# IuvenisSapiens/Qwen3-TTS-Rust

Hardware: AMD Instinct MI355X
Metric: audio-seconds generated per second (aggregate over GPUs) = concurrent real-time streams; RTF and first-chunk latency from the single-utterance leg (higher is better)
Workload: dtype i8

## Files before the change

include/q3tts.h:

```cpp
#ifndef Q3TTS_H
#define Q3TTS_H
#include <stdint.h>
#include <stddef.h>
#ifdef __cplusplus
extern "C" {
#endif

#define Q3TTS_OK 0
#define Q3TTS_ERR -1

const char* q3tts_last_error(void);
int q3tts_version(void);
int q3tts_device_count(void);

typedef struct q3tts_sampler_config {
    float temperature;
    int32_t top_k;
    float top_p;
    int32_t has_seed;
    uint64_t seed;
} q3tts_sampler_config;
void q3tts_sampler_config_default(q3tts_sampler_config* c);

typedef struct q3tts_gen_options {
    float repetition_penalty;
    float predictor_temperature;
    int32_t predictor_top_k;
    float predictor_top_p;
} q3tts_gen_options;
void q3tts_gen_options_default(q3tts_gen_options* o);

typedef struct q3tts_engine q3tts_engine;
typedef struct q3tts_engine_params {
    const char* model_dir;
    const char* quant;
    int32_t device;
    int32_t max_batch;
    int32_t max_prompt;
    int32_t max_steps;
    int32_t load_codec;
    int32_t use_graph;
} q3tts_engine_params;
void q3tts_engine_params_default(q3tts_engine_params* p);
int q3tts_engine_create(const q3tts_engine_params* p, q3tts_engine** out);
void q3tts_engine_destroy(q3tts_engine* e);

typedef struct q3tts_request {
    const float* prompt;
    int32_t n_prompt;
    q3tts_sampler_config sampler;
    int32_t max_steps;
    int32_t mask_eos;
    int32_t* codes_out;
    float* pcm_out;
    int64_t pcm_capacity;
    int32_t n_frames;
    int64_t n_pcm;
    double prefill_ms, first_chunk_ms, total_ms;
} q3tts_request;
int q3tts_generate_batch(q3tts_engine* e, q3tts_request* reqs, int32_t n_reqs, int32_t want_pcm);
int q3tts_generate_batch_ex(q3tts_engine* e, q3tts_request* reqs, int32_t n_reqs, int32_t want_pcm, const q3tts_gen_options* opts);
int q3tts_generate_batch_trailing(q3tts_engine* e, q3tts_request* reqs, int32_t n_reqs, int32_t want_pcm, const q3tts_gen_options* opts,
                                  const int32_t* const* trail_ids, const int32_t* n_trail);

typedef struct q3tts_stats {
    double frame_loop_ms; int64_t frames; double prefill_ms;
    double gemv_ms; int64_t gemv_launches; double gemv_bytes;
    double codec_ms; int64_t codec_calls;
    double talker_weight_bytes, predictor_weight_bytes, kv_bytes_per_token;
    double gu_ms; int64_t gu_launches; double gu_bytes;
    int64_t sched_steps; double slot_frames;
    int64_t graph_frames;
} q3tts_stats;
int q3tts_engine_stats(q3tts_engine* e, q3tts_stats* out);
void q3tts_engine_reset_stats(q3tts_engine* e);
void q3tts_engine_set_instrument(q3tts_engine* e, int32_t on);
double q3tts_engine_bytes_per_step(q3tts_engine* e, int32_t batch, double mean_ctx);

#define Q3TTS_REQ_QUEUED 0
#define Q3TTS_REQ_RUNNING 1
#define Q3TTS_REQ_DRAINING 2
#define Q3TTS_REQ_DONE 3
#define Q3TTS_REQ_CANCELLED 4
#define Q3TTS_REQ_FAILED (-1)
typedef struct q3tts_req_status {
    int32_t state; int32_t n_frames; int64_t n_pcm;
    double queue_ms, prefill_ms, first_chunk_ms, total_ms;
} q3tts_req_status;
int q3tts_submit(q3tts_engine* e, const q3tts_request* r, int32_t want_pcm, int64_t* req_id);
int q3tts_submit_ex(q3tts_engine* e, const q3tts_request* r, int32_t want_pcm, const q3tts_gen_options* opts ,
                    int64_t* req_id);
int q3tts_submit_trailing(q3tts_engine* e, const q3tts_request* r, int32_t want_pcm, const q3tts_gen_options* opts ,
                          const int32_t* trail_ids, int32_t n_trail, int64_t* req_id);
int q3tts_submit_trailing_open(q3tts_engine* e, const q3tts_request* r, int32_t want_pcm, const q3tts_gen_options* opts,
                               const int32_t* trail_ids, int32_t n_trail, int64_t* req_id);
int q3tts_trail_append(q3tts_engine* e, int64_t req_id, const int32_t* ids, int32_t n, int32_t close);
int q3tts_trail_progress(q3tts_engine* e, int64_t req_id, int32_t* n_appended, int32_t* n_consumed, int32_t* closed);
int q3tts_poll(q3tts_engine* e, int64_t req_id, q3tts_req_status* out);
int q3tts_fetch(q3tts_engine* e, int64_t req_id, int32_t* codes_out, int32_t frame_off, int32_t max_frames, float* pcm_out,
                int64_t pcm_off, int64_t pcm_cap, int32_t* got_frames, int64_t* got_pcm);
int q3tts_wait(q3tts_engine* e, int64_t req_id, double timeout_ms );
int q3tts_release(q3tts_engine* e, int64_t req_id);
int q3tts_cancel(q3tts_engine* e, int64_t req_id);
int q3tts_submit_resume(q3tts_engine* e, const q3tts_request* r, int32_t want_pcm, const q3tts_gen_options* opts,
                        const int32_t* trail_ids, int32_t n_trail, int32_t open,
                        const int32_t* prefix_codes, int32_t n_prefix, int64_t* req_id);
#define Q3TTS_LOGPROB_COLS 17
#define Q3TTS_LOGPROB_NONE 1.0f
int q3tts_engine_set_logprobs(q3tts_engine* e, int32_t on);
int q3tts_fetch_logprobs(q3tts_engine* e, int64_t req_id, float* out, int32_t frame_off, int32_t max_frames, int32_t* got_frames);
int32_t q3tts_engine_prefill_width(q3tts_engine* e);
int q3tts_sched_start(q3tts_engine* e);
int q3tts_sched_stop(q3tts_engine* e);
int q3tts_sched_step(q3tts_engine* e, int32_t* busy);
int q3tts_voice_register(q3tts_engine* e, const float* spk_emb2048, const int32_t* ref_codes, int32_t n_ref_codes,
                         const int32_t* ref_text_ids, int32_t n_ref_text, int32_t* voice_id);
int q3tts_submit_text(q3tts_engine* e, int32_t voice_id, const int32_t* text_ids, int32_t n_text, int32_t lang_id,
                      const int32_t* instr_ids, int32_t n_instr, const q3tts_sampler_config* sampler, int32_t max_steps,
                      int32_t mask_eos, int32_t want_pcm, int64_t* req_id);
int q3tts_submit_text_ex(q3tts_engine* e, int32_t voice_id, const int32_t* text_ids, int32_t n_text, int32_t lang_id,
                         const int32_t* instr_ids, int32_t n_instr, const q3tts_sampler_config* sampler, int32_t max_steps,
                         int32_t mask_eos, int32_t want_pcm, const q3tts_gen_options* opts, int64_t* req_id);
int q3tts_submit_text_streaming(q3tts_engine* e, int32_t voice_id, const int32_t* text_ids, int32_t n_text, int32_t lang_id,
                                const int32_t* instr_ids, int32_t n_instr, const q3tts_sampler_config* sampler, int32_t max_steps,
                                int32_t mask_eos, int32_t want_pcm, const q3tts_gen_options* opts, int64_t* req_id);
int q3tts_submit_text_streaming_open(q3tts_engine* e, int32_t voice_id, const int32_t* text_ids, int32_t n_text, int32_t lang_id,
                                     const int32_t* instr_ids, int32_t n_instr, const q3tts_sampler_config* sampler, int32_t max_steps,
                                     int32_t mask_eos, int32_t want_pcm, const q3tts_gen_options* opts, int64_t* req_id);
int q3tts_text_append(q3tts_engine* e, int64_t req_id, const int32_t* text_ids, int32_t n, int32_t is_last);

// ... 173 lines not shown
enum { Q3TTS_GEMM_AUTO = 0, Q3TTS_GEMM_SKINNY4 = 1, Q3TTS_GEMM_SKINNY8 = 2, Q3TTS_GEMM_SKINNY16 = 3,
       Q3TTS_GEMM_F32_1 = 4, Q3TTS_GEMM_F32_2 = 5,
       Q3TTS_GEMM_H1 = 6, Q3TTS_GEMM_H1_EPL = 7, Q3TTS_GEMM_H2 = 8, Q3TTS_GEMM_H2_EPL = 9,
       Q3TTS_GEMM_H3 = 10, Q3TTS_GEMM_H3_EPL = 11 };
enum { Q3TTS_EPI_NONE = 0, Q3TTS_EPI_GELU = 1, Q3TTS_EPI_RES_SCALE = 2 , Q3TTS_EPI_RES = 3 ,
       Q3TTS_EPI_SNAKE = 4  };
typedef struct q3tts_codec_gemm_desc {
    int32_t M, N, cin, taps, dil;
    const float* A; int64_t a_rows; int32_t lda, a_segT, a_skip;
    int32_t a_split, o_split;
    const float* W; const float* bias;
    int32_t epi; const float* res; int64_t res_floats; int32_t ldr, r_segT; int64_t r_skip;
    const float* scale; const float* snake_ea; const float* snake_ib;
    float* out; int64_t out_floats, out_off; int32_t ldo, o_segT; int64_t o_skip;
    int64_t ws_floats;
    int32_t form, ksplit, reducer;
    int32_t form_ran, ksplit_ran, reducer_ran;
} q3tts_codec_gemm_desc;
int q3tts_op_codec_gemm(q3tts_codec_gemm_desc* d);
int q3tts_codec_gemm_plan(q3tts_codec_gemm_desc* d);

enum { Q3TTS_CK_RVQ_SUM = 0, Q3TTS_CK_RMSNORM_ROWS = 1, Q3TTS_CK_LAYERNORM_ROWS = 2, Q3TTS_CK_ROPE_APPEND = 3, Q3TTS_CK_WINDOW_ATTN = 4,
       Q3TTS_CK_SWIGLU_ROWS = 5, Q3TTS_CK_DWCONV7 = 6, Q3TTS_CK_SNAKE = 7, Q3TTS_CK_SNAKE_SPLIT = 8, Q3TTS_CK_CONV_OUT_WAVE = 9,
       Q3TTS_CK_CONV_OUT_WIN = 10, Q3TTS_CK_HIST_LOAD = 11, Q3TTS_CK_HIST_SAVE = 12, Q3TTS_CK_HIST_ZERO = 13 };
typedef struct q3tts_codec_kernel_desc {
    int32_t kernel;
    int32_t G, T, C, H;
    int32_t n_heads, head_dim, window; float rope_base, eps, bias;
    const int64_t* meta;
    const int64_t* codes; int32_t n_q, cb_size;
    int32_t n_streams, stream;
    const float* in[3]; int64_t in_floats[3];
    const float* p0; const float* p1; int64_t p0_floats, p1_floats;
    float* out[3]; int64_t out_floats[3];
} q3tts_codec_kernel_desc;
int q3tts_op_codec_kernel(q3tts_codec_kernel_desc* d);

enum { Q3TTS_ATTN_AUTO = 0, Q3TTS_ATTN_UNFUSED = 1 , Q3TTS_ATTN_FUSED = 2 ,
       Q3TTS_ATTN_SHORT1 = 3, Q3TTS_ATTN_SHORT2 = 4 , Q3TTS_ATTN_GGML = 5  };
typedef struct q3tts_attention_desc {
    int32_t n_head, n_kv, n_layer, layer, ntok;
    const float* qkv; int32_t qkv_stride;
    const float* q_norm; const float* k_norm;
    float eps, rope_base; int32_t n_ctx; int32_t mrope_sec[4];
    const int32_t* seq; const int32_t* slot; const int32_t* pos; int32_t uniform_pos;
    const int32_t* page_table; int32_t n_seq, max_pages;
    uint16_t* k_cache; uint16_t* v_cache; int32_t n_pages;
    int32_t fused, fused_max_tok, same_seq, short_attn_min, hpw1_max, float_mode, ggml_mode;
    int32_t form;
    float* att; int8_t* aq; uint16_t* ad;
    int32_t form_ran;
} q3tts_attention_desc;
int q3tts_op_attention(q3tts_attention_desc* d);
int q3tts_attention_plan(q3tts_attention_desc* d);

enum { Q3TTS_LOP_GEMV = 0, Q3TTS_LOP_GATEUP = 1, Q3TTS_LOP_NORM = 2, Q3TTS_LOP_NORM_GEMV = 3, Q3TTS_LOP_NORM_ARGMAX = 4, Q3TTS_LOP_NORM_GATEUP = 5,
       Q3TTS_LOP_F_GEMV = 6, Q3TTS_LOP_F_GATEUP = 7 };
enum { Q3TTS_LIN_AUTO = 0, Q3TTS_LIN_GEMV_Q8 = 1, Q3TTS_LIN_GEMM_Q8_TOK = 2, Q3TTS_LIN_GEMM_Q8_MFMA = 3, Q3TTS_LIN_GEMM_Q8_TILE1 = 4,
       Q3TTS_LIN_GEMV_KQ = 5, Q3TTS_LIN_GEMM_KQ_MFMA = 6, Q3TTS_LIN_GU_Q8_TILE1 = 7, Q3TTS_LIN_GU_Q8_MFMA = 8, Q3TTS_LIN_GU_KQ_MFMA = 9,
       Q3TTS_LIN_GU_UNFUSED = 10, Q3TTS_LIN_NORM = 11, Q3TTS_LIN_NORM_WG = 12, Q3TTS_LIN_GEMV_NORM = 13, Q3TTS_LIN_GEMV_NORM_ARGMAX = 14,
       Q3TTS_LIN_GU_SWIGLU_NORM = 15, Q3TTS_LIN_F_GEMV = 16, Q3TTS_LIN_F_MFMA16 = 17, Q3TTS_LIN_F_MFMA = 18, Q3TTS_LIN_F_GU_MFMA16 = 19,
       Q3TTS_LIN_F_GU_UNFUSED = 20 };
typedef struct q3tts_linear_desc {
    int32_t op, form;
    int32_t nw; const void* raw[3]; int32_t type[3]; int32_t rows[3]; int32_t kq_layout;
    int32_t K, row0, nrows, nrows_valid, ntok, ff;
    int32_t lpr, mt, ztiles;
    int32_t fused;
    const int8_t* xq; const uint16_t* xd; int32_t a_rows;
    const float* x; int64_t x_floats; int32_t x_off, x_stride;
    const float* h_in; int64_t h_floats; int32_t h_stride;
    const uint64_t* idx_keys; const int32_t* idx; int32_t idx_stride;
    const float* parts; int64_t parts_floats; int32_t nparts, parts_stride; int64_t parts_slab;
    const float* g; float eps;
    float* h_out; float* xn_out;
    int8_t* xq_out; uint16_t* xd_out;
    uint64_t* keys; int64_t n_keys; int32_t key_stride; const int32_t* mask_per_tok; int32_t idx_add;
    float* out; int64_t out_floats, out_off; int32_t out_stride;
    int8_t* aq; uint16_t* ad;
    int32_t form_ran, lpr_ran, mt_ran, z_ran;
} q3tts_linear_desc;
int q3tts_op_linear(q3tts_linear_desc* d);
int q3tts_linear_plan(q3tts_linear_desc* d);
uint64_t q3tts_argmax_key(float v, int32_t idx);

#ifdef __cplusplus
}
#endif
#endif
```

qwen3-tts-rust_amd/csrc/capi.cpp:

```cpp
#include "../../include/q3tts.h"
#include "engine.h"
#include "tfctx.h"
#include <algorithm>

using namespace q3;

struct q3tts_assets { std::unique_ptr<HostAssets> owned; const HostAssets* a = nullptr; };
struct q3tts_engine { std::unique_ptr<Engine> e; q3tts_assets assets_view; };
struct q3tts_sampler { Sampler s; };
struct q3tts_chunker { std::unique_ptr<Chunker> c; };
struct q3tts_decoder { std::unique_ptr<CodecDecoder> d; hipStream_t st = nullptr; float* pinned = nullptr; size_t pinned_cap = 0; };
struct q3tts_tf { std::unique_ptr<TfContext> c; };

#define Q3_API_BEGIN try {
#define Q3_API_END(failval) } catch (const std::exception& ex) { set_last_error(ex.what()); return failval; } catch (...) { set_last_error("unknown error"); return failval; }

static void require_gpu() {
    int n = 0;
    if (hipGetDeviceCount(&n) != hipSuccess || n <= 0) throw Error("no HIP device available: the HIP path is the only compute path (no CPU fallback)");
}

extern "C" {

const char* q3tts_last_error(void) { return last_error(); }
// ... 214 lines not shown
    return submit_text(e, voice_id, text_ids, n_text, lang_id, instr_ids, n_instr, sampler, max_steps, mask_eos, want_pcm, opts, true, req_id);
}
int q3tts_submit_text_streaming_open(q3tts_engine* e, int32_t voice_id, const int32_t* text_ids, int32_t n_text, int32_t lang_id,
                                     const int32_t* instr_ids, int32_t n_instr, const q3tts_sampler_config* sampler, int32_t max_steps,
                                     int32_t mask_eos, int32_t want_pcm, const q3tts_gen_options* opts, int64_t* req_id) {
    return submit_text(e, voice_id, text_ids, n_text, lang_id, instr_ids, n_instr, sampler, max_steps, mask_eos, want_pcm, opts, true, req_id,
                       true);
}
static int submit_text(q3tts_engine* e, int32_t voice_id, const int32_t* text_ids, int32_t n_text, int32_t lang_id, const int32_t* instr_ids,
                       int32_t n_instr, const q3tts_sampler_config* sampler, int32_t max_steps, int32_t mask_eos, int32_t want_pcm,
                       const q3tts_gen_options* opts, bool streaming, int64_t* req_id, bool open) {
    Q3_API_BEGIN
    Q3_CHECK(e && text_ids && n_text >= 0 && req_id, "bad arguments");
    Q3_CHECK(!streaming || n_text >= 1, "the streaming-text layout needs n_text >= 1");
    const Voice& v = e->e->voice(voice_id);
    std::vector<int32_t> t(text_ids, text_ids + n_text), ins;
    if (instr_ids) ins.assign(instr_ids, instr_ids + n_instr);
    int lang = lang_id;
    std::vector<int32_t> trail;
    std::vector<int32_t>* tr = streaming ? &trail : nullptr;
    PromptData pd = !v.ref_codes.empty()
        ? PromptBuilder::build_clone_prompt(e->e->assets(), t, v.ref_codes, v.ref_text_ids, v.spk_emb.data(), lang_id, instr_ids ? &ins : nullptr, tr)
        : PromptBuilder::build_core(e->e->assets(), t, lang_id >= 0 ? &lang : nullptr, nullptr, v.spk_emb.data(), instr_ids ? &ins : nullptr, nullptr, tr);
    GenRequest g;
    g.prompt = pd.embd.data(); g.n_prompt = pd.n_rows; g.max_steps = max_steps; g.mask_eos = mask_eos != 0;
    if (sampler) {
        g.sampler.temperature = sampler->temperature; g.sampler.top_k = sampler->top_k; g.sampler.top_p = sampler->top_p;
        g.sampler.has_seed = sampler->has_seed != 0; g.sampler.seed = sampler->seed;
    }
    g.opts = to_opts(opts);
    if (open) trail.pop_back();
    g.trail = trail.data(); g.n_trail = (int)trail.size(); g.open = open;
    *req_id = e->e->submit(g, want_pcm != 0, true);
    return Q3TTS_OK;
    Q3_API_END(Q3TTS_ERR)
}

int q3tts_engine_stats(q3tts_engine* e, q3tts_stats* o) {
    Q3_API_BEGIN
    const EngineStats& s = e->e->stats;
    o->frame_loop_ms = s.frame_loop_ms; o->frames = s.frames; o->prefill_ms = s.prefill_ms; o->gemv_ms = s.gemv_ms;
    o->gemv_launches = s.gemv_launches; o->gemv_bytes = s.gemv_bytes; o->codec_ms = s.codec_ms; o->codec_calls = s.codec_calls;
    o->gu_ms = s.gu_ms; o->gu_launches = s.gu_launches; o->gu_bytes = s.gu_bytes;
    o->sched_steps = s.steps; o->slot_frames = s.slot_frames; o->graph_frames = s.graph_frames;
    o->talker_weight_bytes = (double)e->e->talker().weight_bytes(); o->predictor_weight_bytes = (double)e->e->predictor().weight_bytes();
    const auto& hp = e->e->talker().hp();
    o->kv_bytes_per_token = (double)hp.n_layer * 2 * hp.n_kv * 128 * 2;
    return Q3TTS_OK;
    Q3_API_END(Q3TTS_ERR)
}
void q3tts_engine_reset_stats(q3tts_engine* e) { if (e) e->e->reset_stats(); }
void q3tts_engine_set_instrument(q3tts_engine* e, int32_t on) { if (e) e->e->set_instrument(on != 0); }
double q3tts_engine_bytes_per_step(q3tts_engine* e, int32_t batch, double mean_ctx) { return e ? (double)e->e->bytes_per_frame_step(batch, mean_ctx) : 0.0; }

int q3tts_assets_open(const char* path, q3tts_assets** out) {
    Q3_API_BEGIN
    Q3_CHECK(path && out, "null argument");
    auto* h = new q3tts_assets();
    try { h->owned.reset(new HostAssets(path)); } catch (...) { delete h; throw; }
    h->a = h->owned.get();
    *out = h;
    return Q3TTS_OK;
    Q3_API_END(Q3TTS_ERR)
}
void q3tts_assets_close(q3tts_assets* a) { delete a; }
const q3tts_assets* q3tts_engine_assets(q3tts_engine* e) { return e ? &e->assets_view : nullptr; }
int q3tts_assets_codec_embedding(const q3tts_assets* a, int32_t q, int32_t code, float* out) { Q3_API_BEGIN a->a->codec_embedding(q, code, out); return Q3TTS_OK; Q3_API_END(Q3TTS_ERR) }
int q3tts_assets_text_embedding(const q3tts_assets* a, int64_t tok, float* out) { Q3_API_BEGIN a->a->text_embedding(tok, out); return Q3TTS_OK; Q3_API_END(Q3TTS_ERR) }
int q3tts_assets_tts_pad(const q3tts_assets* a, float* out) { Q3_API_BEGIN std::copy(a->a->tts_pad(), a->a->tts_pad() + 2048, out); return Q3TTS_OK; Q3_API_END(Q3TTS_ERR) }

int q3tts_op_feedback_rows(const q3tts_assets* a, const int32_t* codes, int32_t n, const int32_t* trail_ids, int32_t n_trail, float* rows) {
    Q3_API_BEGIN
    Q3_CHECK(a && a->a && codes && rows && n >= 1, "bad arguments");
    Q3_CHECK(n_trail >= 0 && (n_trail == 0 || trail_ids), "trailing ids missing");
    require_gpu();
    const HostAssets& h = *a->a;
    Q3_CHECK(h.n_codec == 16, "need 16 codec embedding tables");
    std::vector<DevBuf<float>> tab(16);
    std::vector<const float*> ptrs(16); std::vector<int64_t> nrows(16);
    for (int q = 0; q < 16; q++) {
        const size_t sz = (size_t)h.codec_rows[q] * Q3_EMBD;
        tab[q].alloc(sz); tab[q].upload(h.codec[q], sz);
        ptrs[q] = tab[q].p; nrows[q] = h.codec_rows[q];
    }
    DevBuf<const float*> d_ptrs(16); DevBuf<int64_t> d_nrows(16); DevBuf<float> d_pad(Q3_EMBD), d_text, d_rows((size_t)(n + 2) * Q3_EMBD);
    DevBuf<int32_t> d_codes((size_t)n * 16), d_ids;
    d_ptrs.upload(ptrs.data(), 16); d_nrows.upload(nrows.data(), 16); d_pad.upload(h.tts_pad(), Q3_EMBD); d_codes.upload(codes, (size_t)n * 16);
    FeedbackIds fi;
    const int nt = std::min(n_trail, n);
    if (nt > 0) {
        const int64_t tr = h.text_table ? h.text_rows : 0;
        d_text.alloc((size_t)std::max<int64_t>(tr, 1) * Q3_EMBD);
        if (tr > 0) d_text.upload(h.text_table, (size_t)tr * Q3_EMBD);
        d_ids.alloc(nt); d_ids.upload(trail_ids, nt);
        fi.ids = d_ids.p; fi.n_ids = nt; fi.table = d_text.p; fi.rows = tr;
    }
    std::vector<float> all((size_t)(n + 2) * Q3_EMBD, -12345.0f);
    d_rows.upload(all.data(), all.size());
    launch_feedback_codes(0, d_ptrs.p, d_nrows.p, d_codes.p, d_pad.p, d_rows.p + Q3_EMBD, n, &fi);
    Q3_HIP(hipDeviceSynchronize());
    d_rows.download(all.data(), all.size());
    for (int i = 0; i < Q3_EMBD; i++)
        Q3_CHECK(all[i] == -12345.0f && all[(size_t)(n + 1) * Q3_EMBD + i] == -12345.0f, "k_feedback_codes wrote outside its rows");
    std::copy(all.begin() + Q3_EMBD, all.begin() + (size_t)(n + 1) * Q3_EMBD, rows);
    return Q3TTS_OK;
    Q3_API_END(Q3TTS_ERR)
// ... 166 lines not shown
```

qwen3-tts-rust_amd/csrc/capi_ops.cpp:

```cpp
#include "../../include/q3tts.h"
#include "transformer.h"
#include "host_logic.h"
#include "kdev.h"
#include "codec.h"

using namespace q3;
#define Q3_API_BEGIN try {
#define Q3_API_END(failval) } catch (const std::exception& ex) { set_last_error(ex.what()); return failval; } catch (...) { set_last_error("unknown error"); return failval; }
static void require_gpu() {
    int n = 0;
    if (hipGetDeviceCount(&n) != hipSuccess || n <= 0) throw Error("no HIP device available: the HIP path is the only compute path (no CPU fallback)");
}

static int attention_op_plan(const q3tts_attention_desc& d) {
    AttnPlanIn a;
    a.ntok = d.ntok; a.fused = d.fused != 0; a.fused_max_tok = d.fused_max_tok; a.same_seq = d.same_seq != 0; a.short_attn_min = d.short_attn_min;
    a.n_head = d.n_head; a.n_kv = d.n_kv; a.hpw1_max = d.hpw1_max > 0 ? d.hpw1_max : short_attn_hpw1_max();
    a.float_mode = d.float_mode != 0; a.ggml_mode = d.ggml_mode != 0;
    return plan_attention(a);
}

static void attention_op_check(const q3tts_attention_desc& d, int form) {
    Q3_CHECK(form >= ATTN_UNFUSED && form <= ATTN_GGML, "unknown attention form");
    Q3_CHECK(d.n_head >= 1 && d.n_kv >= 1 && d.n_head % d.n_kv == 0, "n_head must be a multiple of n_kv");
    Q3_CHECK(d.n_layer >= 1 && d.layer >= 0 && d.layer < d.n_layer && d.ntok >= 1 && d.ntok <= 65535, "bad layer / token count");
    Q3_CHECK(d.qkv && d.q_norm && d.k_norm && d.k_cache && d.v_cache && d.qkv_stride >= (d.n_head + 2 * d.n_kv) * 128, "bad qkv / norm / cache buffers");
    Q3_CHECK(d.n_ctx >= 1 && d.n_pages >= 1, "bad n_ctx / n_pages");
    if (form != ATTN_GGML) Q3_CHECK(d.aq && d.ad, "aq / ad are required");
    else Q3_CHECK(d.att, "the ggml form produces att only");
    if (d.uniform_pos < 0) Q3_CHECK(d.seq && d.slot && d.pos, "per-token seq / slot / pos are required without uniform_pos");
    if (d.page_table) {
        Q3_CHECK(d.n_seq >= 1 && d.max_pages >= 1, "bad page table shape");
        for (int64_t i = 0; i < (int64_t)d.n_seq * d.max_pages; i++)
            Q3_CHECK(d.page_table[i] >= 0 && d.page_table[i] < d.n_pages, "page table entry out of range");
    }
    const bool short_form = form == ATTN_SHORT1 || form == ATTN_SHORT2;
    if (short_form) Q3_CHECK(d.n_head == 2 * d.n_kv, "the short forms need n_head == 2 * n_kv");
    std::map<std::pair<int, int>, int> seen;
    std::map<int, int> per_seq;
    for (int t = 0; t < d.ntok; t++) {
        const int seq = d.uniform_pos >= 0 ? t : d.seq[t], slot = d.uniform_pos >= 0 ? d.uniform_pos : d.slot[t];
        Q3_CHECK(slot >= 0 && slot < d.n_ctx, "slot out of [0, n_ctx)");
        if (d.page_table) Q3_CHECK(seq >= 0 && seq < d.n_seq && slot < d.max_pages * 64, "sequence or slot beyond the page table");
        else Q3_CHECK(seq >= 0 && seq < d.n_pages && slot < 64, "identity paging: sequence beyond the cache or slot beyond its one page");
        if (short_form) Q3_CHECK(slot < 64, "the short forms read page 0 only: slot must be < 64");
        Q3_CHECK(seen[std::make_pair(seq, slot)]++ == 0, "two tokens write the same (sequence, slot)");
        if (++per_seq[seq] > 1) Q3_CHECK(form == ATTN_UNFUSED || form == ATTN_GGML, "the fused and short forms need one token per sequence");
    }
}

static void attention_op_run(q3tts_attention_desc* dp) {
    Q3_CHECK(dp, "null attention descriptor");
    q3tts_attention_desc& d = *dp;
    Q3_CHECK(d.ntok >= 1 && d.n_head >= 1 && d.n_kv >= 1, "bad attention shape");
    const int form = d.form == Q3TTS_ATTN_AUTO ? attention_op_plan(d) : d.form;
    attention_op_check(d, form);
    const int nt = d.ntok, dq = d.n_head * 128, qs = d.qkv_stride;
    DevBuf<float> qkv((size_t)nt * qs); qkv.upload(d.qkv, qkv.n);
    DevBuf<float> qn(128), kn(128); qn.upload(d.q_norm, 128); kn.upload(d.k_norm, 128);
    std::vector<float> hc, hs;
    build_rope_tables(d.rope_base, d.n_ctx, hc, hs);
    DevBuf<float> rc(hc.size()), rs(hs.size()); rc.upload(hc.data(), hc.size()); rs.upload(hs.data(), hs.size());
    DevBuf<int32_t> sec(4); sec.upload(d.mrope_sec, 4);
    DevBuf<int32_t> dseq, dslot, dpos, dtab;
    TokMeta tm{nullptr, nullptr, nullptr};
    if (d.uniform_pos >= 0) tm.uniform_pos = d.uniform_pos;
    else {
        dseq.alloc(nt); dseq.upload(d.seq, nt); dslot.alloc(nt); dslot.upload(d.slot, nt); dpos.alloc((size_t)nt * 4); dpos.upload(d.pos, (size_t)nt * 4);
        tm.seq = dseq.p; tm.slot = dslot.p; tm.pos = dpos.p;
    }
    const size_t cache_halfs = (size_t)d.n_pages * d.n_layer * d.n_kv * 8192;
    DevBuf<uint16_t> kc(cache_halfs), vc(cache_halfs);
    kc.upload(d.k_cache, cache_halfs); vc.upload(d.v_cache, cache_halfs);
    KvCache kv;
    kv.k = kc.p; kv.v = vc.p; kv.page_table = nullptr; kv.max_pages = d.page_table ? d.max_pages : 1; kv.n_layer = d.n_layer; kv.n_kv = d.n_kv;
    if (d.page_table) { dtab.alloc((size_t)d.n_seq * d.max_pages); dtab.upload(d.page_table, dtab.n); kv.page_table = dtab.p; }
    DevBuf<float> att((size_t)nt * dq), qrot, scores;
    DevBuf<int8_t> aq((size_t)nt * dq); DevBuf<uint16_t> ad((size_t)nt * (dq / 32));
    switch (form) {
    case ATTN_UNFUSED:
        qrot.alloc((size_t)nt * dq);
        launch_qk_rope_append(0, qkv.p, qs, nullptr, d.n_head, d.n_kv, qn.p, kn.p, d.eps, rc.p, rs.p, d.n_ctx, sec.p, tm, kv, d.layer, qrot.p, nt);
        launch_attention(0, qrot.p, d.n_head, d.n_kv, tm, kv, d.layer, att.p, aq.p, ad.p, nt);
        break;
    case ATTN_FUSED:
        launch_attention_fused(0, qkv.p, qs, d.n_head, d.n_kv, qn.p, kn.p, d.eps, rc.p, rs.p, d.n_ctx, sec.p, tm, kv, d.layer, aq.p, ad.p, nt);
        break;
    case ATTN_SHORT1: case ATTN_SHORT2:
        launch_attention_short(0, form == ATTN_SHORT1 ? 1 : 2, qkv.p, qs, d.n_head, d.n_kv, qn.p, kn.p, d.eps, rc.p, rs.p, d.n_ctx, sec.p, tm, kv,
                               d.layer, aq.p, ad.p, nt, att.p);
        break;
    default:
        scores.alloc((size_t)nt * d.n_head * d.n_ctx);
        gg_qk_rope_append(0, qkv.p, qs, d.n_head, d.n_kv, qn.p, kn.p, d.eps, rc.p, rs.p, d.n_ctx, sec.p, tm, kv, d.layer, nt);
        gg_attention(0, qkv.p, qs, d.n_head, d.n_kv, tm, kv, d.layer, att.p, scores.p, d.n_ctx, nt);
        break;
    }
    Q3_LAUNCH_CHECK();
    Q3_HIP(hipDeviceSynchronize());
    kc.download(d.k_cache, cache_halfs); vc.download(d.v_cache, cache_halfs);
    if (d.att && form != ATTN_FUSED) att.download(d.att, att.n);
    if (form != ATTN_GGML) { aq.download(d.aq, aq.n); ad.download(d.ad, ad.n); }
    d.form_ran = form;
}

static bool lin_quant(const q3tts_linear_desc& d) { return d.op <= LOP_NORM_GATEUP && d.op != LOP_NORM; }
static bool lin_kq(const q3tts_linear_desc& d) {
    if (d.kq_layout || d.nw > 1) return true;
    return d.type[0] != Q3_T_Q8_0;
}
static int lin_rows(const q3tts_linear_desc& d) { int n = 0; for (int i = 0; i < d.nw; i++) n += d.rows[i]; return n; }
static int lin_wts(const q3tts_linear_desc& d) {
    if (d.op >= LOP_F_GEMV) return d.type[0];
    if (!lin_kq(d)) return 0;
    int n = 0, last = -1;
    for (int i = 0; i < d.nw; i++) if (d.type[i] != last) { n++; last = d.type[i]; }
    return n == 1 ? d.type[0] : -1;
}
static LinearPlanIn lin_plan_in(const q3tts_linear_desc& d) {
    LinearPlanIn in;
    in.op = d.op; in.K = d.K; in.row0 = d.row0; in.nrows = d.nrows; in.ntok = d.ntok; in.ff = d.ff;
    in.kq = lin_quant(d) && lin_kq(d); in.wts = lin_wts(d); in.has_wt = true;
    if (in.kq) { int n = 0, last = -1; for (int i = 0; i < d.nw; i++) if (d.type[i] != last) { n++; last = d.type[i]; } in.kq_parts = n; }
    in.out_stride = d.out_stride; in.out_addr = (uintptr_t)d.out_off * 4 + (d.out ? (uintptr_t)d.out : 0);
    in.x_stride = d.x_stride; in.x_addr = (uintptr_t)d.x_off * 4 + (d.x ? (uintptr_t)d.x : 0);
    in.aq_addr = 0; in.fused = d.fused != 0;
    return in;
}
static LinearPlan lin_plan(const q3tts_linear_desc& d) {
    Q3_CHECK(d.op >= LOP_GEMV && d.op <= LOP_F_GATEUP, "unknown linear op");
    Q3_CHECK(d.K >= 256 && d.K % 256 == 0 && d.ntok >= 1 && d.ntok <= 65535 && d.nrows >= 1 && d.row0 >= 0, "bad linear shape");
    return plan_linear(lin_plan_in(d));
}
static bool in_set(int v, std::initializer_list<int> s) { for (int x : s) if (v == x) return true; return false; }
static int op_of_form(int f) {
    if (f <= LIN_GEMM_KQ_MFMA) return LOP_GEMV;
    if (f <= LIN_GU_UNFUSED) return LOP_GATEUP;
    if (f <= LIN_NORM_WG) return LOP_NORM;
    if (f == LIN_GEMV_NORM) return LOP_NORM_GEMV;
    if (f == LIN_GEMV_NORM_ARGMAX) return LOP_NORM_ARGMAX;
    if (f == LIN_GU_SWIGLU_NORM) return LOP_NORM_GATEUP;
    if (f <= LIN_F_MFMA) return LOP_F_GEMV;
    return LOP_F_GATEUP;
}
static void lin_check(const q3tts_linear_desc& d, const LinearPlan& p) {
    const int f = p.form, K = d.K, nt = d.ntok, ntiles = (nt + 31) / 32;
    Q3_CHECK(f >= LIN_GEMV_Q8 && f <= LIN_F_GU_UNFUSED && op_of_form(f) == d.op, "the form does not compute this op");
    const bool quant = lin_quant(d), kq = quant && lin_kq(d), norm = d.op >= LOP_NORM && d.op <= LOP_NORM_GATEUP;
    if (d.op != LOP_NORM) {
        Q3_CHECK(d.nw >= 1 && d.nw <= 3, "1 to 3 weight tensors");
        for (int i = 0; i < d.nw; i++) Q3_CHECK(d.raw[i] && d.rows[i] >= 1, "missing weight tensor");
        if (d.op >= LOP_F_GEMV) Q3_CHECK(d.nw == 1 && (d.type[0] == Q3_T_F32 || d.type[0] == Q3_T_F16 || d.type[0] == Q3_T_BF16), "float ops take one f32 / f16 / bf16 tensor");
        else if (kq) for (int i = 0; i < d.nw; i++) Q3_CHECK(in_set(d.type[i], {Q3_T_Q8_0, Q3_T_Q5_K, Q3_T_Q6_K}) && d.rows[i] % 32 == 0, "K-quant layout: Q8_0 / Q5_K / Q6_K tensors of 32-row multiples");
        Q3_CHECK(d.row0 + d.nrows <= lin_rows(d), "rows past the matrix");
    }
// ... 134 lines not shown
        dxq_out.alloc((size_t)nt * K); dxq_out.upload(d.xq_out, dxq_out.n); dxd_out.alloc((size_t)nt * (K / 32)); dxd_out.upload(d.xd_out, dxd_out.n);
        launch_rmsnorm_quant_wg(0, a, K, dxq_out.p, dxd_out.p, nt);
        break;
    case LIN_GEMV_NORM: case LIN_GEMV_NORM_ARGMAX: {
        ArgmaxEpi am{};
        if (p.form == LIN_GEMV_NORM_ARGMAX) {
            dkeys.alloc((size_t)d.n_keys); dkeys.upload((const q3_u64*)d.keys, dkeys.n);
            if (d.mask_per_tok) { dmask.alloc(nt); dmask.upload(d.mask_per_tok, nt); }
            am.keys = dkeys.p; am.key_stride = d.key_stride; am.mask_per_tok = dmask.p; am.idx_add = d.idx_add;
            run_gemv_q8_norm(0, p, m, d.row0, d.nrows_valid, a, nullptr, 0, nt, &am);
        } else run_gemv_q8_norm(0, p, m, d.row0, d.nrows, a, out, d.out_stride, nt, nullptr);
        break;
    }
    case LIN_GU_SWIGLU_NORM: run_gateup_swiglu(0, p, m, ff, a, daq.p, dad.p, nt); break;
    case LIN_F_GEMV: case LIN_F_MFMA16: case LIN_F_MFMA:
        run_gemv_float(0, p, fm, d.row0, d.nrows, dx.p + d.x_off, d.x_stride, out, d.out_stride, nt);
        break;
    case LIN_F_GU_MFMA16:
        dgu.alloc((size_t)nt * ff);
        run_gateup_float(0, p, fm, ff, dx.p + d.x_off, d.x_stride, dgu.p, nt);
        break;
    case LIN_F_GU_UNFUSED: {
        dgu.alloc((size_t)nt * 2 * ff);
        LinearPlanIn gi = lin_plan_in(d); gi.op = LOP_F_GEMV;
        const LinearPlan gp = plan_linear(gi);
        run_gemv_float(0, gp, fm, 0, 2 * ff, dx.p + d.x_off, d.x_stride, dgu.p, 2 * ff, nt);
        DevBuf<float> act((size_t)nt * ff);
        launch_swiglu_f32(0, dgu.p, ff, act.p, nt);
        Q3_HIP(hipMemcpy2D(out, (size_t)d.out_stride * 4, act.p, (size_t)ff * 4, (size_t)ff * 4, nt, hipMemcpyDeviceToDevice));
        Q3_HIP(hipDeviceSynchronize());
        p.lpr = gp.lpr; p.mt = gp.mt; p.z = gp.z;
        break;
    }
    default: throw Error("unhandled linear form");
    }
    Q3_LAUNCH_CHECK();
    if (p.form == LIN_F_GU_MFMA16) Q3_HIP(hipMemcpy2D(out, (size_t)d.out_stride * 4, dgu.p, (size_t)ff * 4, (size_t)ff * 4, nt, hipMemcpyDeviceToDevice));
    Q3_HIP(hipDeviceSynchronize());
    if (d.out) dout.download(d.out, dout.n);
    if (d.aq) { daq.download(d.aq, daq.n); dad.download(d.ad, dad.n); }
    if (d.h_out) dhout.download(d.h_out, dhout.n);
    if (d.xn_out) dxn.download(d.xn_out, dxn.n);
    if (dxq_out.p) { dxq_out.download(d.xq_out, dxq_out.n); dxd_out.download(d.xd_out, dxd_out.n); }
    if (dkeys.p) dkeys.download((q3_u64*)d.keys, dkeys.n);
    d.form_ran = p.form; d.lpr_ran = p.lpr; d.mt_ran = p.mt; d.z_ran = p.z;
}

extern "C" {

int q3tts_op_attention(q3tts_attention_desc* d) {
    Q3_API_BEGIN
    require_gpu();
    attention_op_run(d);
    return Q3TTS_OK;
    Q3_API_END(Q3TTS_ERR)
}

int q3tts_attention_plan(q3tts_attention_desc* d) {
    Q3_API_BEGIN
    Q3_CHECK(d && d->ntok >= 1 && d->n_kv >= 1 && d->n_head >= 1, "bad attention shape");
    d->form_ran = attention_op_plan(*d);
    return Q3TTS_OK;
    Q3_API_END(Q3TTS_ERR)
}

int q3tts_op_linear(q3tts_linear_desc* d) {
    Q3_API_BEGIN
    require_gpu();
    lin_run(d);
    return Q3TTS_OK;
    Q3_API_END(Q3TTS_ERR)
}

int q3tts_linear_plan(q3tts_linear_desc* d) {
    Q3_API_BEGIN
    Q3_CHECK(d, "null linear descriptor");
    const LinearPlan p = lin_plan(*d);
    d->form_ran = p.form; d->lpr_ran = p.lpr; d->mt_ran = p.mt; d->z_ran = p.z;
    return Q3TTS_OK;
    Q3_API_END(Q3TTS_ERR)
}

uint64_t q3tts_argmax_key(float v, int32_t idx) { return pack_key(v, idx); }

int q3tts_op_gemv_q8(const void* w, int32_t n, int32_t k, const int8_t* xq, const uint16_t* xd, int32_t ntok, float* y, int32_t lpr) {
    Q3_API_BEGIN
    require_gpu();
    DevBuf<uint8_t> storage;
    Q8Mat m = q8mat_from_host(w, n, k, storage);
    DevBuf<int8_t> dxq((size_t)ntok * k); dxq.upload(xq, dxq.n);
    DevBuf<uint16_t> dxd((size_t)ntok * (k / 32)); dxd.upload(xd, dxd.n);
    const int nsseg = ((k >> 8) + 7) / 8;
    DevBuf<float> parts((size_t)nsseg * ntok * n);
    launch_gemv_q8(0, m, 0, n, dxq.p, dxd.p, parts.p, n, ntok, lpr);
    Q3_HIP(hipDeviceSynchronize());
    std::vector<float> hp(parts.n);
    parts.download(hp.data(), hp.size());
    for (int t = 0; t < ntok; t++)
        for (int r = 0; r < n; r++) {
            float v = hp[((size_t)0 * ntok + t) * n + r];
            for (int s = 1; s < nsseg; s++) v = v + hp[((size_t)s * ntok + t) * n + r];
            y[(size_t)t * n + r] = v;
        }
    return Q3TTS_OK;
    Q3_API_END(Q3TTS_ERR)
}
// ... 483 lines not shown
```

qwen3-tts-rust_amd/csrc/engine.cpp:

```cpp
#include "engine.h"
#include "../../include/q3tts.h"
#include <algorithm>
#include <cmath>
#include <chrono>
#include "kdev.h"
#include <functional>

namespace q3 {

static std::string quant_dir(const std::string& q) {
    if (q == "q5_k_m") return "gguf_q5_k_m";
    if (q == "q8_0") return "gguf_q8_0";
    if (q == "bf16") return "gguf_bf16";
    if (q == "f16") return "gguf_f16";
    return "gguf";
}
static double now_ms() {
    return std::chrono::duration<double, std::milli>(std::chrono::steady_clock::now().time_since_epoch()).count();
}

Engine::Engine(const EngineParams& p) : p_(p) {
    Q3_CHECK(p.max_batch >= 1 && p.max_batch <= 512, "max_batch out of range");
    Q3_HIP(hipGetDevice(&dev_));
    Q3_HIP(hipStreamCreateWithFlags(&st_, hipStreamNonBlocking));
    const std::string dir = p.model_dir + "/" + quant_dir(p.quant);
    assets_.reset(new HostAssets(dir + "/qwen3_assets.gguf"));
    const int B = p.max_batch;
    B_ = B;
    talker_.reset(new Transformer(dir + "/qwen3_tts_talker.gguf", Q3_TALKER_NCTX, std::max(256, B)));
    predictor_.reset(new Transformer(dir + "/qwen3_tts_predictor.gguf", Q3_PRED_NCTX, 2 * B));
    if (const char* e = std::getenv("Q3_PRED_FUSED_MAX")) predictor_->set_fused_max_tokens(atoi(e));
    {
        int min_tok = 8;
        if (const char* e = std::getenv("Q3_SHORT_ATTN_MIN")) min_tok = atoi(e);
        predictor_->set_short_attention(min_tok, 17);
    }
    Q3_CHECK(talker_->hp().n_embd == Q3_EMBD, "talker n_embd must be 2048 (reference hard-codes 2048-wide rows)");
    dP_ = predictor_->hp().n_embd;
    Q3_CHECK(assets_->proj_out == dP_ && assets_->proj_in == Q3_EMBD, "proj shape does not match predictor n_embd");
    Q3_CHECK(assets_->n_codec == 16, "need 16 codec embedding tables");
    Q3_CHECK(predictor_->hp().n_vocab >= 15 * Q3_CODEBOOK_SIZE, "predictor vocab < 15*2048");
    std::vector<float> wt((size_t)Q3_EMBD * dP_);
    for (int o = 0; o < dP_; o++)
        for (int i = 0; i < Q3_EMBD; i++) wt[(size_t)i * dP_ + o] = assets_->proj_w[(size_t)o * Q3_EMBD + i];
    d_proj_wt_.alloc(wt.size()); d_proj_wt_.upload(wt.data(), wt.size());
    Q3_CHECK(dP_ % 16 == 0, "projection width must be a multiple of 16");
    {
        std::vector<float> wb((size_t)Q3_EMBD * dP_);
        for (int o = 0; o < dP_; o++)
            for (int i = 0; i < Q3_EMBD; i++) wb[((size_t)(o / 16) * Q3_EMBD + i) * 16 + (o % 16)] = assets_->proj_w[(size_t)o * Q3_EMBD + i];
        d_proj_wblk_.alloc(wb.size()); d_proj_wblk_.upload(wb.data(), wb.size());
    }
    d_proj_b_.alloc(dP_); d_proj_b_.upload(assets_->proj_b, dP_);
    d_tts_pad_.alloc(Q3_EMBD); d_tts_pad_.upload(assets_->tts_pad(), Q3_EMBD);
    std::vector<const float*> ptrs(16);
    std::vector<int64_t> rows(16);
    for (int q = 0; q < 16; q++) {
        const size_t n = (size_t)assets_->codec_rows[q] * Q3_EMBD;
        d_codec_tab_[q].alloc(n); d_codec_tab_[q].upload(assets_->codec[q], n);
        d_proj_tab_[q].alloc((size_t)assets_->codec_rows[q] * dP_);
        launch_project_table(st_, d_codec_tab_[q].p, assets_->codec_rows[q], d_proj_wt_.p, d_proj_b_.p, Q3_EMBD, dP_, d_proj_tab_[q].p);
        ptrs[q] = d_codec_tab_[q].p; rows[q] = assets_->codec_rows[q];
    }
    d_tab_ptrs_.alloc(16); d_tab_ptrs_.upload(ptrs.data(), 16);
    d_tab_rows_.alloc(16); d_tab_rows_.upload(rows.data(), 16);
    const int pages_per_seq = (p.max_prompt + p.max_steps + 1 + 63) / 64;
    kv_rows_ = (int64_t)pages_per_seq * 64;
    kv_t_.reset(new KvPool(talker_->hp().n_layer, talker_->hp().n_kv, B * pages_per_seq + 1, B + 1, pages_per_seq));
    kv_p_.reset(new KvPool(predictor_->hp().n_layer, predictor_->hp().n_kv, B, B, 1));
    for (int b = 0; b < B; b++) kv_p_->ensure(b, 16);
    pred_identity_pages_ = true;
    for (int b = 0; b < B; b++) if (kv_p_->page(b, 0) != b) pred_identity_pages_ = false;
    if (const char* e = std::getenv("Q3_UNIFORM_META")) if (e[0] == '0') pred_identity_pages_ = false;
    kv_t_->ensure(B, 1);
    {
        const char* e = std::getenv("Q3_ASYNC_PREFILL");
        async_pf_ = B > 1 && !(e && e[0] == '0');
    }
    if (async_pf_) {
        talker_pf_.reset(new Transformer(*talker_, 256));
        Q3_HIP(hipStreamCreateWithFlags(&st_pf_, hipStreamNonBlocking));
        Q3_HIP(hipEventCreate(&pf_done_)); Q3_HIP(hipEventCreate(&pf_e0_));
        arena_pf_cap_ = (size_t)4096 * (Q3_EMBD * 4 + 24 + 68) + ((size_t)1 << 16);
        Q3_HIP(hipHostMalloc((void**)&arena_pf_, arena_pf_cap_));
        d_prompt_pf_.alloc((size_t)256 * Q3_EMBD); d_pfa_seq_.alloc(256); d_pfa_slot_.alloc(256); d_pfa_pos_.alloc(4 * 256);
        d_pfa_codes_.alloc((size_t)256 * 16); d_pfa_ids_.alloc(256);
    }
    hist_stride_ = p.max_steps * 16;
    tl_stride_ = (Q3_SAMPLE_END + 31) & ~31;
    slots_ = SlotTable(B); d_slots_.alloc(slots_.host.size()); slots_.dev = d_slots_.p;
    d_keys_.alloc(16 * B); d_next_key0_.alloc(B); d_hist_.alloc((size_t)B * hist_stride_);
    d_rngkey_.alloc((size_t)8 * B); d_draws_.alloc(B); d_prngkey_.alloc((size_t)8 * B); d_pdraws_.alloc(B);
    d_rngkey_.zero(); d_draws_.zero(); d_prngkey_.zero(); d_pdraws_.zero(); d_plogits_.alloc((size_t)B * Q3_CODEBOOK_SIZE);
    d_tlogits_.alloc((size_t)B * tl_stride_); d_thidden_.alloc((size_t)B * Q3_EMBD); d_pin_.alloc((size_t)2 * B * dP_);
    d_fb_.alloc((size_t)B * Q3_EMBD);
    d_prompt_.alloc((size_t)talker_->max_tok() * Q3_EMBD);
    d_pf_seq_.alloc(talker_->max_tok()); d_pf_slot_.alloc(talker_->max_tok()); d_pf_pos_.alloc(4 * (size_t)talker_->max_tok());
    d_pf_codes_.alloc((size_t)talker_->max_tok() * 16); d_pf_ids_.alloc(talker_->max_tok());
    d_hist_.zero(); d_tlogits_.zero(); d_thidden_.zero();
    std::vector<int32_t> seq(B), slot((size_t)16 * B), pos((size_t)16 * B * 4);
    for (int b = 0; b < B; b++) {
        seq[b] = b;
        for (int i = 0; i < 16; i++) { slot[(size_t)i * B + b] = i; for (int s = 0; s < 4; s++) pos[((size_t)i * B + b) * 4 + s] = i; }
    }
    d_pseq_.alloc(B); d_pseq_.upload(seq.data(), B);
    d_pslot_.alloc(slot.size()); d_pslot_.upload(slot.data(), slot.size());
    d_ppos_.alloc(pos.size()); d_ppos_.upload(pos.data(), pos.size());
    h_pend_.assign(B, std::vector<int32_t>()); h_pend_off_.assign(B, 0);
    slot_req_.assign(B, nullptr);
    if (async_pf_) { d_pf_logits_.alloc((size_t)B * tl_stride_); d_pf_hidden_.alloc((size_t)B * Q3_EMBD); }
    {
        std::vector<q3_u64> k0((size_t)16 * B, pack_key(-INFINITY, 0)), n0(B, pack_key(-INFINITY, 0));
        d_keys_.upload(k0.data(), k0.size()); d_next_key0_.upload(n0.data(), n0.size());
    }
    arena_cap_ = (size_t)talker_->max_tok() * Q3_EMBD * 4 + (size_t)B * 4096 + ((size_t)1 << 20);
    Q3_HIP(hipHostMalloc((void**)&arena_, arena_cap_));
    Q3_HIP(hipDeviceSynchronize());
    upload_slot_state();
// ... 32 lines not shown
void* Engine::d2h_begin(const void* src, size_t bytes) {
    void* p = stage_alloc(bytes);
    Q3_HIP(hipMemcpyAsync(p, src, bytes, hipMemcpyDeviceToHost, st_));
    return p;
}

struct Engine::Req {
    int64_t id = 0;
    GenRequest r; std::vector<float> prompt_own; std::vector<int32_t> trail_own; bool want_pcm = false;
    std::vector<int32_t> prefix_own;
    bool closed = false;
    bool cancel = false;
    int state = REQ_QUEUED; int slot = -1, cs = -1; int fed = 0;
    std::vector<int32_t> codes; std::vector<float> pcm;
    std::vector<float> lp;
    size_t pcm_enq = 0;
    size_t pcm_ready = 0;
    std::unique_ptr<Chunker> chunker;
    uint64_t seed = 0;
    hipEvent_t ev_admit = nullptr; bool first_seen = false;
    double t_submit = 0, t_admit = 0, t_done = 0, prefill_ms = 0, first_chunk_ms = 0;
    std::string error;
};

Engine::~Engine() {
    (void)hipSetDevice(dev_);
    try { stop_driver(); } catch (...) {}
    if (dec_started_) {
        { std::lock_guard<std::mutex> lk(dmu_); dec_stop_ = true; }
        dcv_.notify_all();
        dec_thread_.join();
    }
    for (auto& c : comp_) (void)hipEventDestroy(c.ev);
    for (auto& kv : reqs_) if (kv.second->ev_admit) (void)hipEventDestroy(kv.second->ev_admit);
    for (auto& g : graphs_) {
        if (g.second->exec) (void)hipGraphExecDestroy(g.second->exec);
        if (g.second->graph) (void)hipGraphDestroy(g.second->graph);
    }
    if (pcm_pinned_) (void)hipHostFree(pcm_pinned_);
    if (arena_) (void)hipHostFree(arena_);
    if (arena_pf_) (void)hipHostFree(arena_pf_);
    if (pf_done_) (void)hipEventDestroy(pf_done_);
    if (pf_e0_) (void)hipEventDestroy(pf_e0_);
    if (st_pf_) (void)hipStreamDestroy(st_pf_);
    for (auto s2 : st2_) (void)hipStreamDestroy(s2);
    if (st_) (void)hipStreamDestroy(st_);
}

size_t Engine::bytes_per_frame_step(int batch, double mean_ctx) const {
    const auto& t = talker_->hp();
    const size_t head_t = (size_t)tl_stride_ * talker_->head_bytes_per_row();
    const size_t head_p = (size_t)15 * Q3_CODEBOOK_SIZE * predictor_->head_bytes_per_row();
    const size_t kv_per_tok = (size_t)t.n_layer * 2 * t.n_kv * 128 * 2;
    return talker_->weight_bytes() + head_t + predictor_->weight_bytes() + head_p +
           (size_t)((double)batch * mean_ctx * (double)kv_per_tok) + (size_t)batch * 17 * 8192;
}

void Engine::record_frame(FrameGraph& fg, FrameVariant v) {
    const int B = fg.width;
    const KvCache kvt = kv_t_->view(), kvp = kv_p_->view();
    AdvanceKeysArgs a{B, di(SF_FINISHED), di(SF_NFRAMES), di(SF_MAXFRAMES), d_keys_.p, d_next_key0_.p, d_hist_.p, hist_stride_, di(SF_TSLOT), di(SF_TPOS)};
    StallArgs sg;
    if (v.gate) {
        sg.open = di(SF_OPEN); sg.n_trail = di(SF_NTRAIL); sg.hidden = d_thidden_.p; sg.draws = d_draws_.p; sg.pdraws = d_pdraws_.p;
        sg.save_hidden = d_stall_hidden_.p; sg.save_draws = d_stall_draws_.p;
        launch_stall_save(st_, a, sg);
    }
    launch_project_blk(st_, d_thidden_.p, Q3_EMBD, d_proj_wblk_.p, d_proj_b_.p, Q3_EMBD, dP_, d_pin_.p, dP_, B);
    launch_gather_rows_keys(st_, d_proj_tab_[0].p, assets_->codec_rows[0], d_keys_.p, 16, dP_, d_pin_.p + (size_t)B * dP_, B);
    {
        TokMeta tm{fg.seqA.p, fg.slotA.p, fg.posA.p};
        Transformer::Input in; in.x = d_pin_.p; in.x_stride = dP_;
        predictor_->set_same_seq_tokens(true);
        predictor_->forward(st_, in, 2 * B, tm, kvp, nullptr);
        if (v.pred || v.lp) {
            float* pl = v.lp ? d_plp_.p : d_plogits_.p;
            predictor_->head(st_, B, B, 0, Q3_CODEBOOK_SIZE, pl, Q3_CODEBOOK_SIZE);
            SampleArgs sa{pl, Q3_CODEBOOK_SIZE, Q3_CODEBOOK_SIZE, df(SF_PTEMP), di(SF_PTOPK), df(SF_PTOPP), nullptr, d_prngkey_.p, d_pdraws_.p, d_keys_.p + 1, 16};
            launch_sample_pred(st_, sa, B);
        } else {
            ArgmaxEpi am{d_keys_.p + 1, 16, nullptr, 0};
            predictor_->head(st_, B, B, 0, Q3_CODEBOOK_SIZE, nullptr, 0, &am);
        }
    }
    predictor_->set_same_seq_tokens(false);
    for (int q = 1; q < 15; q++) {
        TokMeta tm{d_pseq_.p, d_pslot_.p + (size_t)(q + 1) * B_, d_ppos_.p + (size_t)(q + 1) * B_ * 4};
        KvCache kvq = kvp;
        if (pred_identity_pages_) { tm.uniform_pos = q + 1; kvq.page_table = nullptr; }
        Transformer::Input in; in.x = d_proj_tab_[q].p; in.x_stride = dP_; in.idx_keys = d_keys_.p + q; in.idx_stride = 16;
        predictor_->forward(st_, in, B, tm, kvq, nullptr);
        if (v.pred || v.lp) {
            float* pl = v.lp ? d_plp_.p + (size_t)q * B_ * Q3_CODEBOOK_SIZE : d_plogits_.p;
            predictor_->head(st_, 0, B, q * Q3_CODEBOOK_SIZE, Q3_CODEBOOK_SIZE, pl, Q3_CODEBOOK_SIZE);
            SampleArgs sa{pl, Q3_CODEBOOK_SIZE, Q3_CODEBOOK_SIZE, df(SF_PTEMP), di(SF_PTOPK), df(SF_PTOPP), nullptr, d_prngkey_.p, d_pdraws_.p, d_keys_.p + q + 1, 16};
            launch_sample_pred(st_, sa, B);
        } else {
            ArgmaxEpi am{d_keys_.p + q + 1, 16, nullptr, 0};
            predictor_->head(st_, 0, B, q * Q3_CODEBOOK_SIZE, Q3_CODEBOOK_SIZE, nullptr, 0, &am);
        }
    }
    if (v.trail) {
        TextTrail tt; tt.n_frames = di(SF_NFRAMES); tt.n_trail = di(SF_NTRAIL); tt.ids = d_trail_.p; tt.ids_stride = p_.max_prompt;
        tt.table = d_text_.p; tt.rows = text_rows_;
        launch_feedback_keys(st_, d_tab_ptrs_.p, d_tab_rows_.p, d_keys_.p, 16, d_tts_pad_.p, d_fb_.p, B, &tt);
    } else {
        launch_feedback_keys(st_, d_tab_ptrs_.p, d_tab_rows_.p, d_keys_.p, 16, d_tts_pad_.p, d_fb_.p, B);
    }
    {
        TokMeta tm{di(SF_TSEQ), di(SF_TSLOT), di(SF_TPOS)};
        Transformer::Input in; in.x = d_fb_.p; in.x_stride = Q3_EMBD;
        talker_->set_same_seq_tokens(false);
        talker_->forward(st_, in, B, tm, kvt, nullptr);
        if (v.sampled || v.pen || v.lp) {
            talker_->head(st_, 0, B, 0, tl_stride_, d_tlogits_.p, tl_stride_, nullptr, -1, d_thidden_.p);
            SampleArgs sa{d_tlogits_.p, tl_stride_, Q3_SAMPLE_END, df(SF_TEMP), di(SF_TOPK), df(SF_TOPP), di(SF_MASKEOS), d_rngkey_.p, d_draws_.p, d_next_key0_.p, 1};
            if (v.pen) { sa.penalty = df(SF_PEN); sa.hist = d_hist_.p; sa.hist_stride = hist_stride_; sa.hist_len = di(SF_NFRAMES); sa.cur_key = d_keys_.p; sa.cur_stride = 16; }
            launch_sample(st_, sa, B);
            if (v.lp) {
                LogprobArgs la;
                la.p.logits = d_plp_.p; la.p.stride = Q3_CODEBOOK_SIZE; la.p.head_stride = (size_t)B_ * Q3_CODEBOOK_SIZE; la.p.n = Q3_CODEBOOK_SIZE;
                la.p.key = d_keys_.p + 1; la.p.key_stride = 16; la.p.col = 1; la.n_first = 15;
                la.t.logits = d_tlogits_.p; la.t.stride = tl_stride_; la.t.n = Q3_SAMPLE_END; la.t.key = d_next_key0_.p; la.t.key_stride = 1;
                la.t.extra_idx = Q3_CODEC_EOS; la.t.col = 0; la.t.col_extra = Q3_LOGPROB_COLS - 1; la.t.row_ahead = 1;
                la.out = d_lp_.p; la.out_stride = Q3_LOGPROB_COLS; la.out_rows = lp_rows_;
                la.n_frames = di(SF_NFRAMES); la.finished = di(SF_FINISHED); la.max_frames = di(SF_MAXFRAMES); la.open = di(SF_OPEN);
                la.n_trail = di(SF_NTRAIL); la.record = d_lp_rec_.p;
                launch_logprob_rows(st_, la, B);
            }
        } else {
            ArgmaxEpi am{d_next_key0_.p, 1, di(SF_MASKEOS), 0};
            talker_->head(st_, 0, B, 0, tl_stride_, nullptr, 0, &am, Q3_SAMPLE_END, d_thidden_.p);
        }
    }
    if (v.gate) launch_advance_keys_gated(st_, a, sg);
    else launch_advance_keys(st_, a);
    Q3_LAUNCH_CHECK();
}

std::mutex& capture_mutex() { static std::mutex mu; return mu; }

Engine::FrameGraph& Engine::frame_graph(int width, FrameVariant v, bool capture) {
    std::unique_ptr<FrameGraph>& slot = graphs_[v.key(width)];
// ... 879 lines not shown
```

qwen3-tts-rust_amd/csrc/engine.h:

```cpp
#pragma once
#include "transformer.h"
#include "host_logic.h"
#include "sched_logic.h"
#include "codec.h"
#include <atomic>
#include <condition_variable>
#include <deque>
#include <map>
#include <memory>
#include <mutex>
#include <thread>

namespace q3 {

struct EngineParams {
    std::string model_dir;
    std::string quant = "q8_0";
    int max_batch = 1;
    int max_prompt = 1024;
    int max_steps = Q3_DEFAULT_MAX_STEPS;
    bool load_codec = true;
    bool use_graph = true;
};

// ... 4 lines not shown
};

struct EngineStats {
    double frame_loop_ms = 0; long frames = 0;
    double gemv_ms = 0; long gemv_launches = 0; double gemv_bytes = 0;
    double gu_ms = 0; long gu_launches = 0; double gu_bytes = 0;
    double codec_ms = 0; long codec_calls = 0;
    double prefill_ms = 0;
    long steps = 0; double slot_frames = 0;
    long graph_frames = 0;
};

struct ReqStatus {
    int state = REQ_QUEUED; int n_frames = 0; int64_t n_pcm = 0;
    double queue_ms = 0, prefill_ms = 0, first_chunk_ms = 0, total_ms = 0;
    std::string error;
};

struct Voice {
    std::vector<float> spk_emb; std::vector<int32_t> ref_codes, ref_text_ids;
};


class Engine {
public:
    explicit Engine(const EngineParams& p);
    ~Engine();
    void generate_batch(const std::vector<GenRequest>& reqs, std::vector<GenResult>& out, bool want_pcm);

    int64_t submit(const GenRequest& r, bool want_pcm, bool copy_prompt = true, bool may_record = true);
    void set_logprobs(bool on);
    void fetch_logprobs(int64_t id, float* out, int frame_off, int max_frames, int* got_frames);
    int append_trail(int64_t id, const int32_t* ids, int n, bool close);
    void trail_progress(int64_t id, int* n_appended, int* n_consumed, bool* closed);
    int cancel(int64_t id);
    bool step();
    ReqStatus poll(int64_t id);
    void fetch(int64_t id, int32_t* codes, int frame_off, int max_frames, float* pcm, int64_t pcm_off, int64_t pcm_cap,
               int* got_frames, int64_t* got_pcm);
    bool wait(int64_t id, double timeout_ms);
    void release(int64_t id);
    void start_driver();
    void stop_driver();
    int register_voice(const Voice& v);
    const Voice& voice(int id) const;

    const HostAssets& assets() const { return *assets_; }
    Transformer& talker() { return *talker_; }
    Transformer& predictor() { return *predictor_; }
    CodecDecoder* codec() { return codec_.get(); }
    EngineStats stats; void reset_stats() { stats = EngineStats(); }
    void set_instrument(bool on) { instrument_ = on; }
    size_t bytes_per_frame_step(int batch, double mean_ctx) const;
    hipStream_t stream() const { return st_; }
    int max_batch() const { return B_; }
    int device() const { return dev_; }

private:
    struct Req;
    struct FrameGraph {
        int width = 0; hipGraph_t graph = nullptr; hipGraphExec_t exec = nullptr;
        DevBuf<int32_t> seqA, slotA, posA;
    };
    void record_frame(FrameGraph& fg, FrameVariant v);
    FrameGraph& frame_graph(int width, FrameVariant v, bool capture);
    void validate(const GenRequest& g) const;
    void ensure_text_stream();
    void prefill(const std::vector<Req*>& batch, bool sampled);
    void feedback_rows(hipStream_t st, const std::vector<Req*>& batch, const std::vector<FbRun>& fb, int32_t* hc, int32_t* d_codes, int32_t* d_ids, float* d_rows);
    void head_history(SampleArgs& sa, int b) const;
    static bool resumed_penalised(const GenRequest& g) { return g.n_prefix > 0 && g.opts.penalised(); }
    void first_head_logprobs(hipStream_t st, const float* logits_row, int b, int row);
    void prefill_async(const std::vector<Req*>& batch);
    void activate();
    void admit(bool stalled);
    void run_group();
    void collect_appends();
    void collect_cancels();
    void harvest(bool block);
    void purge_chunks(Req* r);
    void retire(Req* r, bool flush_tail);
    void decoder_main();
    void upload_slot_state();
    void* stage_alloc(size_t bytes);
    void h2d(void* dst, const void* src, size_t bytes);
    void* d2h_begin(const void* src, size_t bytes);
    unsigned char* arena_ = nullptr; size_t arena_cap_ = 0, arena_used_ = 0;

    EngineParams p_;
    hipStream_t st_ = nullptr; int dev_ = 0;
    std::vector<hipStream_t> st2_;
    float* pcm_pinned_ = nullptr; size_t slot_cap_ = 0;
    std::unique_ptr<HostAssets> assets_;
    std::unique_ptr<Transformer> talker_, predictor_, talker_pf_;
    hipStream_t st_pf_ = nullptr; unsigned char* arena_pf_ = nullptr; size_t arena_pf_cap_ = 0;
    DevBuf<float> d_prompt_pf_, d_pf_logits_, d_pf_hidden_; DevBuf<int32_t> d_pfa_seq_, d_pfa_slot_, d_pfa_pos_;
    std::vector<Req*> pf_batch_; hipEvent_t pf_done_ = nullptr, pf_e0_ = nullptr; bool async_pf_ = false; int n_prefilling_ = 0;
    std::unique_ptr<KvPool> kv_t_, kv_p_;
    std::unique_ptr<CodecDecoder> codec_;
    DevBuf<float> d_codec_tab_[16]; DevBuf<float> d_proj_tab_[16];
    DevBuf<float> d_proj_wt_, d_proj_wblk_, d_proj_b_, d_tts_pad_;
    DevBuf<const float*> d_tab_ptrs_; DevBuf<int64_t> d_tab_rows_;
    int dP_ = 0;
    int B_ = 0; SlotTable slots_; DevBuf<uint32_t> d_slots_; bool slot_dirty_ = false;
    int32_t* di(SlotField f) const { return slots_.di(f); } float* df(SlotField f) const { return slots_.df(f); }
    DevBuf<int32_t> d_hist_; DevBuf<q3_u64> d_keys_, d_next_key0_;
    DevBuf<uint32_t> d_rngkey_, d_draws_, d_prngkey_, d_pdraws_; DevBuf<float> d_plogits_;
    DevBuf<int32_t> d_pseq_, d_pslot_, d_ppos_;
    DevBuf<float> d_tlogits_, d_thidden_, d_pin_, d_fb_, d_prompt_;
    DevBuf<int32_t> d_pf_seq_, d_pf_slot_, d_pf_pos_;
    DevBuf<int32_t> d_pf_codes_, d_pf_ids_, d_pfa_codes_, d_pfa_ids_;
    int64_t kv_rows_ = 0;
    int hist_stride_ = 0, tl_stride_ = 0;
    DevBuf<float> d_text_; DevBuf<int32_t> d_trail_; int64_t text_rows_ = 0;
    std::mutex text_mu_; bool text_ready_ = false;
    DevBuf<float> d_stall_hidden_; DevBuf<uint32_t> d_stall_draws_;
    DevBuf<float> d_lp_, d_plp_; DevBuf<int32_t> d_lp_rec_; int lp_rows_ = 0;
    std::mutex lp_mu_; std::atomic<bool> lp_on_{false}, lp_ready_{false};
    std::map<int, std::unique_ptr<FrameGraph>> graphs_;
    bool instrument_ = false; bool pred_identity_pages_ = false;
    std::vector<std::vector<int32_t>> h_pend_; std::vector<int> h_pend_off_;
    std::mutex mu_; std::condition_variable cv_;
    std::mutex step_mu_;
    std::map<int64_t, std::unique_ptr<Req>> reqs_;
    std::deque<Req*> pending_;
    std::vector<Req*> slot_req_;
    std::vector<int> cs_free_;
    int64_t next_id_ = 1;
    int n_active_ = 0, n_draining_ = 0;
    bool trail_dirty_ = false;
    std::vector<int64_t> cancel_ids_;
    uint64_t wake_ = 0;
    bool stalled_idle_ = false;
    std::vector<Voice> voices_;
    std::thread driver_; bool driver_on_ = false, driver_stop_ = false;
    struct DecTask { Req* r; std::vector<int64_t> codes; bool is_final; bool fence; bool reset; };
    struct Completion { Req* r; hipEvent_t ev; size_t pcm_after; bool fence; };
    std::thread dec_thread_; bool dec_started_ = false, dec_stop_ = false;
    std::mutex dmu_; std::condition_variable dcv_;
    std::deque<DecTask> dq_; std::deque<Completion> comp_;
    int dec_pending_ = 0;
    std::string derr_;
    LaunchTimer timer_, timer_gu_;
};

}
```

qwen3-tts-rust_amd/csrc/kernels.h:

```cpp
#pragma once
#include <hip/hip_runtime.h>
#include <cstdint>
#include "wlayout.h"

namespace q3 {

struct Q8Mat {
    const uint8_t* qs = nullptr;
    const uint16_t* sc = nullptr;
    int N = 0;
    int Npad = 0;
    int K = 0;
    const uint8_t* rg_type = nullptr;
    const uint32_t* rg_off = nullptr;
    const uint8_t* meta = nullptr;
    size_t qbytes = 0;
    int nparts = 0; int p1_rg0 = 0x7fffffff, p2_rg0 = 0x7fffffff; int p0_type = 0, p1_type = 0, p2_type = 0; uint32_t p0_off = 0, p1_off = 0, p2_off = 0;
    size_t bytes() const { return (qbytes ? qbytes : (size_t)Npad * K) + (size_t)Npad * (K / 32) * 2 + (meta ? (size_t)Npad * (K / 256) * 16 : 0); }
};

struct TokMeta {
    const int32_t* seq;
    const int32_t* slot;
    const int32_t* pos;
    int uniform_pos = -1;
    __device__ __forceinline__ int seq_of(int tok) const { return uniform_pos >= 0 ? tok : seq[tok]; }
    __device__ __forceinline__ int slot_of(int tok) const { return uniform_pos >= 0 ? uniform_pos : slot[tok]; }
    __device__ __forceinline__ int pos_of(int tok, int stream) const { return uniform_pos >= 0 ? uniform_pos : pos[(size_t)tok * 4 + stream]; }
};

struct KvCache {
    uint16_t* k;
    uint16_t* v;
    const int32_t* page_table;
    int max_pages;
    int n_layer, n_kv;
    __host__ __device__ size_t page_stride() const { return (size_t)n_layer * n_kv * 8192; }
    __host__ __device__ size_t layer_stride() const { return (size_t)n_kv * 8192; }
    __device__ __forceinline__ int page_of(int seq, int logical) const { return page_table ? page_table[(size_t)seq * max_pages + logical] : seq; }
};

bool launch_gateup_mfma(hipStream_t st, const Q8Mat& wgu, int ff, const int8_t* xq, const uint16_t* xd, int8_t* aq, uint16_t* ad, int ntok);
void launch_gemv_q8(hipStream_t st, const Q8Mat& w, int row0, int nrows, const int8_t* xq, const uint16_t* xd,
                    float* out, int out_stride, int ntok, int lpr_hint = 0);

struct NormArgs {
    const float* h_in; int h_stride;
    const int32_t* idx; int idx_stride;
    const unsigned long long* idx_keys;
    const float* parts; int nparts; int parts_stride;
    float* h_out;
    const float* g; float eps; int d;
    int8_t* xq; uint16_t* xd;
    float* xn_out;
};
void launch_rmsnorm_quant(hipStream_t st, const NormArgs& a, int ntok);

void launch_qk_rope_append(hipStream_t st, const float* qkv, int qkv_stride, const float* parts_unused, int n_head, int n_kv,
                           const float* q_norm_w, const float* k_norm_w, float eps, const float* rope_cos,
                           const float* rope_sin, int n_ctx, const int32_t* mrope_sec , const TokMeta& tm,
                           const KvCache& kv, int layer, float* qrot, int ntok);

void launch_attention(hipStream_t st, const float* qrot, int n_head, int n_kv, const TokMeta& tm, const KvCache& kv,
                      int layer, float* att , int8_t* aq, uint16_t* ad, int ntok);

void launch_swiglu_quant(hipStream_t st, const float* gu, int ff, int8_t* aq, uint16_t* ad, int ntok);

void launch_argmax(hipStream_t st, const float* logits, int stride, int start, int end, const int32_t* mask_per_tok,
                   int32_t* out, int out_stride, int add, int ntok);

void launch_project(hipStream_t st, const float* x, int x_stride, const float* Wt, const float* b, int n_in, int n_out,
                    float* out, int out_stride, int ntok);
void launch_project_table(hipStream_t st, const float* table, int64_t rows, const float* Wt, const float* b, int n_in,
                          int n_out, float* out);

void launch_argmax_keys(hipStream_t st, const float* logits, int stride, int n, const int32_t* mask_per_tok, unsigned long long* keys,
                        int key_stride, int ntok);


void launch_copy_f32(hipStream_t st, const float* src, float* dst, size_t n);
void init_kernel_attributes();

struct FMat { const void* w = nullptr; const void* wt = nullptr; int type = 0; int N = 0, K = 0; size_t bytes() const { return (size_t)N * K * (type == 0 ? 4 : 2); } };
void launch_gemv_float(hipStream_t st, const FMat& w, int row0, int nrows, const float* x, int x_stride, float* out, int out_stride, int ntok);
bool launch_gateup_float(hipStream_t st, const FMat& wgu, int ff, const float* x, int x_stride, float* act, int ntok);
void launch_tile_float(hipStream_t st, const void* w, void* wt, int type, int N, int K);
void launch_swiglu_f32(hipStream_t st, const float* gu, int ff, float* out, int ntok);

typedef unsigned long long q3_u64;
struct NormPro {
    const float* h_in; int h_stride;
    const q3_u64* idx_keys; int idx_stride;
    const float* parts; int nparts; int parts_stride; size_t parts_slab;
    float* h_out;
    const float* g; float eps;
    float* xn_out;
};
struct ArgmaxEpi {
    q3_u64* keys; int key_stride;
    const int32_t* mask_per_tok;
    int idx_add;
};
void launch_gemv_q8_norm(hipStream_t st, const Q8Mat& w, int row0, int nrows, const NormPro& a, float* out, int out_stride,
                         int ntok, const ArgmaxEpi* am);
void launch_rmsnorm_quant_wg(hipStream_t st, const NormPro& a, int d, int8_t* xq, uint16_t* xd, int ntok);
inline NormArgs norm_args(const NormPro& p, int d, int8_t* xq, uint16_t* xd, const int32_t* idx = nullptr) {
    return NormArgs{p.h_in, p.h_stride, idx, p.idx_stride, p.idx_keys, p.parts, p.nparts, p.parts_stride, p.h_out, p.g, p.eps, d, xq, xd, p.xn_out};
}
void launch_gateup_swiglu(hipStream_t st, const Q8Mat& wgu, int ff, const NormPro& a, int8_t* aq, uint16_t* ad, int ntok);
void launch_attention_fused(hipStream_t st, const float* qkv, int qkv_stride, int n_head, int n_kv, const float* q_norm_w,
                            const float* k_norm_w, float eps, const float* rope_cos, const float* rope_sin, int n_ctx,
                            const int32_t* mrope_sec, const TokMeta& tm, const KvCache& kv, int layer, int8_t* aq, uint16_t* ad,
                            int ntok);
void launch_attention_short(hipStream_t st, int hpw, const float* qkv, int qkv_stride, int n_head, int n_kv, const float* q_norm_w,
                            const float* k_norm_w, float eps, const float* rope_cos, const float* rope_sin, int n_ctx,
                            const int32_t* mrope_sec, const TokMeta& tm, const KvCache& kv, int layer, int8_t* aq, uint16_t* ad, int ntok,
                            float* att = nullptr );
int short_attn_hpw1_max();
void launch_project_blk(hipStream_t st, const float* x, int x_stride, const float* Wblk , const float* b,
                        int n_in, int n_out, float* out, int out_stride, int ntok);
enum LinearOp { LOP_GEMV = 0, LOP_GATEUP = 1, LOP_NORM = 2, LOP_NORM_GEMV = 3, LOP_NORM_ARGMAX = 4, LOP_NORM_GATEUP = 5, LOP_F_GEMV = 6,
                LOP_F_GATEUP = 7 };
enum LinearForm { LIN_AUTO = 0, LIN_GEMV_Q8 = 1, LIN_GEMM_Q8_TOK = 2, LIN_GEMM_Q8_MFMA = 3, LIN_GEMM_Q8_TILE1 = 4, LIN_GEMV_KQ = 5,
                  LIN_GEMM_KQ_MFMA = 6, LIN_GU_Q8_TILE1 = 7, LIN_GU_Q8_MFMA = 8, LIN_GU_KQ_MFMA = 9, LIN_GU_UNFUSED = 10, LIN_NORM = 11,
                  LIN_NORM_WG = 12, LIN_GEMV_NORM = 13, LIN_GEMV_NORM_ARGMAX = 14, LIN_GU_SWIGLU_NORM = 15, LIN_F_GEMV = 16, LIN_F_MFMA16 = 17,
                  LIN_F_MFMA = 18, LIN_F_GU_MFMA16 = 19, LIN_F_GU_UNFUSED = 20 };
struct LinearPlanIn {
    int op = LOP_GEMV;
    int K = 0, row0 = 0, nrows = 0, ntok = 0, ff = 0;
    int wts = 0;
    bool kq = false;
    int kq_parts = 0;
    bool has_wt = false;
    int out_stride = 0; uintptr_t out_addr = 0;
    int x_stride = 0; uintptr_t x_addr = 0;
    uintptr_t aq_addr = 0;
    int lpr_hint = 0;
    bool fused = true;
};
struct LinearPlan { int form = LIN_AUTO, lpr = 0, mt = 0, z = 0, nseg = 0; };
LinearPlan plan_linear(const LinearPlanIn& in);
void run_gemv_q8(hipStream_t st, const LinearPlan& p, const Q8Mat& w, int row0, int nrows, const int8_t* xq, const uint16_t* xd, float* out,
                 int out_stride, int ntok);
void run_gateup_q8(hipStream_t st, const LinearPlan& p, const Q8Mat& wgu, int ff, const int8_t* xq, const uint16_t* xd, int8_t* aq, uint16_t* ad,
                   int ntok);
void run_gemv_q8_norm(hipStream_t st, const LinearPlan& p, const Q8Mat& w, int row0, int nrows, const NormPro& a, float* out, int out_stride,
                      int ntok, const ArgmaxEpi* am);
void run_gateup_swiglu(hipStream_t st, const LinearPlan& p, const Q8Mat& wgu, int ff, const NormPro& a, int8_t* aq, uint16_t* ad, int ntok);
void run_gemv_float(hipStream_t st, const LinearPlan& p, const FMat& w, int row0, int nrows, const float* x, int x_stride, float* out,
                    int out_stride, int ntok);
void run_gateup_float(hipStream_t st, const LinearPlan& p, const FMat& wgu, int ff, const float* x, int x_stride, float* act, int ntok);
LinearPlanIn linear_plan_in(int op, const Q8Mat& w, int row0, int nrows, int ntok);
struct TextTrail {
    const int32_t* n_frames = nullptr; const int32_t* n_trail = nullptr; const int32_t* ids = nullptr; int ids_stride = 0;
    const float* table = nullptr; int64_t rows = 0;
};
void launch_feedback_keys(hipStream_t st, const float* const* tables, const int64_t* table_rows, const q3_u64* keys, int key_stride,
                          const float* tts_pad, float* out, int ntok, const TextTrail* trail = nullptr);
struct FeedbackIds { const int32_t* ids = nullptr; int n_ids = 0; const float* table = nullptr; int64_t rows = 0; };
void launch_feedback_codes(hipStream_t st, const float* const* tables, const int64_t* table_rows, const int32_t* codes, const float* tts_pad,
                           float* out, int n, const FeedbackIds* ids = nullptr);
void launch_gather_rows_keys(hipStream_t st, const float* table, int64_t rows, const q3_u64* keys, int key_stride, int row_len,
                             float* dst, int ntok);
struct AdvanceKeysArgs {
    int B; int32_t *finished, *n_frames; const int32_t* max_frames; q3_u64* keys; q3_u64* next_key0; int32_t* hist; int hist_stride;
    int32_t *t_slot, *t_pos;
};
// ... 37 lines not shown
```

qwen3-tts-rust_amd/csrc/kernels.hip:

```cpp
#include "kernels.h"
#include <cstdlib>
#include "q3_common.h"
#include "../../include/q3tts_spec.h"
#include "kdev.h"
#include "wslice.h"

namespace q3 {

Q3_STAMP_SETTER(set_stamp_buffer)

template <int LPR, int MT>
__global__ void __launch_bounds__(512) k_gemv_q8(Q8Mat w, int row0, int nrows, const int8_t* __restrict__ xq,
                                                 const uint16_t* __restrict__ xd, float* __restrict__ out,
                                                 int out_stride, int ntok) {
    constexpr int R = 64 / LPR, BPL = LPR / 2, NLD = 8 / BPL;
    __shared__ float red[8][R * MT];
    const int lane = threadIdx.x & 63, wave = threadIdx.x >> 6;
    const int r = lane % R, q = lane / R, half = q & 1, bil = q >> 1;
    const int nseg = w.K >> 8, nb = w.K >> 5;
    const int sseg = blockIdx.y, seg = sseg * 8 + wave;
    const int tok0 = blockIdx.z * MT;
    const bool active = seg < nseg;
    float acc[MT];
#pragma unroll
// ... 758 lines not shown
__global__ void __launch_bounds__(64) k_rmsnorm_quant(NormArgs a) {
    const int tok = blockIdx.x, lane = threadIdx.x;
    const int nch = a.d >> 8;
    const float* hin = a.h_in;
    if (a.idx_keys) hin += (size_t)key_code(a.idx_keys[(size_t)tok * a.idx_stride]) * a.h_stride;
    else if (a.idx) hin += (size_t)a.idx[(size_t)tok * a.idx_stride] * a.h_stride;
    else hin += (size_t)tok * a.h_stride;
    float4 x[8];
    float p = 0.0f;
#pragma unroll
    for (int c = 0; c < 8; c++) {
        if (c < nch) {
            float4 v = *reinterpret_cast<const float4*>(hin + 256 * c + 4 * lane);
            if (a.nparts > 0) {
                const float* pp = a.parts + (size_t)tok * a.parts_stride + 256 * c + 4 * lane;
                float4 y = *reinterpret_cast<const float4*>(pp);
                for (int s = 1; s < a.nparts; s++) {
                    const float4 z = *reinterpret_cast<const float4*>(pp + (size_t)s * gridDim.x * a.parts_stride);
                    y.x = y.x + z.x; y.y = y.y + z.y; y.z = y.z + z.z; y.w = y.w + z.w;
                }
                v.x = v.x + y.x; v.y = v.y + y.y; v.z = v.z + y.z; v.w = v.w + y.w;
            }
            if (a.h_out) *reinterpret_cast<float4*>(a.h_out + (size_t)tok * a.d + 256 * c + 4 * lane) = v;
            x[c] = v;
            p = q3_fmaf(v.x, v.x, p); p = q3_fmaf(v.y, v.y, p); p = q3_fmaf(v.z, v.z, p); p = q3_fmaf(v.w, v.w, p);
        }
    }
    const float ss = wave_sum_bfly(p);
    const float mean = ss / (float)a.d;
    const float scale = 1.0f / q3_sqrtf(mean + a.eps);
#pragma unroll
    for (int c = 0; c < 8; c++) {
        if (c < nch) {
            const float4 g = *reinterpret_cast<const float4*>(a.g + 256 * c + 4 * lane);
            float4 y;
            y.x = (x[c].x * scale) * g.x; y.y = (x[c].y * scale) * g.y;
            y.z = (x[c].z * scale) * g.z; y.w = (x[c].w * scale) * g.w;
            if (a.xn_out) *reinterpret_cast<float4*>(a.xn_out + (size_t)tok * a.d + 256 * c + 4 * lane) = y;
            float amax = fmaxf(fmaxf(q3_fabsf(y.x), q3_fabsf(y.y)), fmaxf(q3_fabsf(y.z), q3_fabsf(y.w)));
            amax = fmaxf(amax, xor_lane<1>(amax)); amax = fmaxf(amax, xor_lane<2>(amax)); amax = fmaxf(amax, xor_lane<4>(amax));
            const float dd = amax / 127.0f;
            const float id = (dd != 0.0f) ? (1.0f / dd) : 0.0f;
            const int q0 = (int)q3_rintf(y.x * id), q1 = (int)q3_rintf(y.y * id), q2 = (int)q3_rintf(y.z * id), q3v = (int)q3_rintf(y.w * id);
            const uint32_t pk = (uint32_t)(q0 & 0xFF) | ((uint32_t)(q1 & 0xFF) << 8) | ((uint32_t)(q2 & 0xFF) << 16) | ((uint32_t)(q3v & 0xFF) << 24);
            *reinterpret_cast<uint32_t*>(a.xq + (size_t)tok * a.d + 256 * c + 4 * lane) = pk;
            if ((lane & 7) == 0) a.xd[(size_t)tok * (a.d >> 5) + 8 * c + (lane >> 3)] = f2h(dd);
        }
    }
}
void launch_rmsnorm_quant(hipStream_t st, const NormArgs& a, int ntok) {
    hipLaunchKernelGGL(k_rmsnorm_quant, dim3(ntok), dim3(64), 0, st, a);
}

__global__ void __launch_bounds__(64) k_qk_rope_append(const float* __restrict__ qkv, int qkv_stride, int n_head, int n_kv,
                                                       const float* __restrict__ q_norm_w, const float* __restrict__ k_norm_w,
                                                       float eps, const float* __restrict__ rope_cos,
                                                       const float* __restrict__ rope_sin, int n_ctx,
                                                       const int32_t* __restrict__ mrope_sec, TokMeta tm, KvCache kv,
                                                       int layer, float* __restrict__ qrot) {
    const int hv = blockIdx.x, tok = blockIdx.y, lane = threadIdx.x;
    const float* vec = qkv + (size_t)tok * qkv_stride + (size_t)hv * 128;
    float x1 = vec[lane], x2 = vec[lane + 64];
    const int seq = tm.seq_of(tok), slot = tm.slot_of(tok);
    const int page = kv.page_of(seq, slot >> 6);
    const int ps = slot & 63;
    if (hv < n_head + n_kv) {
        const float* w = hv < n_head ? q_norm_w : k_norm_w;
        float p = x1 * x1;
        p = q3_fmaf(x2, x2, p);
        const float ss = wave_sum_bfly(p);
        const float mean = ss / 128.0f;
        const float scale = 1.0f / q3_sqrtf(mean + eps);
        const float y1 = (x1 * scale) * w[lane], y2 = (x2 * scale) * w[lane + 64];
        int32_t sec[4] = { mrope_sec[0], mrope_sec[1], mrope_sec[2], mrope_sec[3] };
        int pp = tm.pos_of(tok, q3_mrope_stream(lane, sec));
        if (pp < 0) pp = 0;
        if (pp > n_ctx - 1) pp = n_ctx - 1;
        float o1, o2;
        q3_rope_pair(y1, y2, rope_cos[(size_t)pp * 64 + lane], rope_sin[(size_t)pp * 64 + lane], &o1, &o2);
        if (hv < n_head) {
            float* dst = qrot + ((size_t)tok * n_head + hv) * 128;
            dst[lane] = o1; dst[lane + 64] = o2;
        } else {
            const int kh = hv - n_head;
            uint16_t* Kb = kv.k + (size_t)page * kv.page_stride() + (size_t)layer * kv.layer_stride() + (size_t)kh * 8192;
            Kb[((lane >> 3) * 64 + ps) * 8 + (lane & 7)] = f2h(o1);
            Kb[(((lane + 64) >> 3) * 64 + ps) * 8 + (lane & 7)] = f2h(o2);
        }
    } else {
        const int vh = hv - n_head - n_kv;
        uint16_t* Vb = kv.v + (size_t)page * kv.page_stride() + (size_t)layer * kv.layer_stride() + (size_t)vh * 8192;
        Vb[ps * 128 + lane] = f2h(x1);
        Vb[ps * 128 + lane + 64] = f2h(x2);
    }
}
void launch_qk_rope_append(hipStream_t st, const float* qkv, int qkv_stride, const float*, int n_head, int n_kv,
                           const float* q_norm_w, const float* k_norm_w, float eps, const float* rope_cos,
                           const float* rope_sin, int n_ctx, const int32_t* mrope_sec, const TokMeta& tm,
                           const KvCache& kv, int layer, float* qrot, int ntok) {
    hipLaunchKernelGGL(k_qk_rope_append, dim3(n_head + 2 * n_kv, ntok), dim3(64), 0, st, qkv, qkv_stride, n_head, n_kv,
                       q_norm_w, k_norm_w, eps, rope_cos, rope_sin, n_ctx, mrope_sec, tm, kv, layer, qrot);
}

__global__ void __launch_bounds__(256) k_attention(const float* __restrict__ qrot, int n_head, int n_kv, TokMeta tm,
                                                   KvCache kv, int layer, float* __restrict__ att,
                                                   int8_t* __restrict__ aq, uint16_t* __restrict__ ad) {
    __shared__ float q_s[128];
    __shared__ float p_s[256];
    __shared__ float red_s[4][128];
    __shared__ float wmax_s[4];
    const int h = blockIdx.x, tok = blockIdx.y, tid = threadIdx.x, lane = tid & 63, wave = tid >> 6;
    const int seq = tm.seq_of(tok), n = tm.slot_of(tok) + 1;
    const int kvh = h / (n_head / n_kv);
    const size_t head_off = (size_t)layer * kv.layer_stride() + (size_t)kvh * 8192;
    if (tid < 128) q_s[tid] = qrot[((size_t)tok * n_head + h) * 128 + tid];
    __syncthreads();
    const float scale = 0.08838834764831845f;
    const int jj = lane >> 4, dc = lane & 15;
    float M = 0.0f, L = 0.0f, O[8];
#pragma unroll
    for (int i = 0; i < 8; i++) O[i] = 0.0f;
    for (int c0 = 0; c0 < n; c0 += 256) {
        const int jbase = c0 + wave * 64;
        const bool valid = (jbase + lane) < n;
        float s = -INFINITY;
        if (jbase < n) {
            const int page = kv.page_of(seq, jbase >> 6);
            const uint16_t* Kb = kv.k + (size_t)page * kv.page_stride() + head_off;
            float acc = 0.0f;
#pragma unroll
            for (int d8 = 0; d8 < 16; d8++) {
                const uint4 kk = *reinterpret_cast<const uint4*>(Kb + (d8 * 64 + lane) * 8);
                const float4 qa = *reinterpret_cast<const float4*>(&q_s[8 * d8]);
                const float4 qb = *reinterpret_cast<const float4*>(&q_s[8 * d8 + 4]);
                acc = q3_fmaf(qa.x, h2f(kk.x & 0xFFFFu), acc); acc = q3_fmaf(qa.y, h2f(kk.x >> 16), acc);
                acc = q3_fmaf(qa.z, h2f(kk.y & 0xFFFFu), acc); acc = q3_fmaf(qa.w, h2f(kk.y >> 16), acc);
                acc = q3_fmaf(qb.x, h2f(kk.z & 0xFFFFu), acc); acc = q3_fmaf(qb.y, h2f(kk.z >> 16), acc);
                acc = q3_fmaf(qb.z, h2f(kk.w & 0xFFFFu), acc); acc = q3_fmaf(qb.w, h2f(kk.w >> 16), acc);
            }
            if (valid) s = acc * scale;
        }
        const float wm = wave_max_bfly(s);
        if (lane == 0) wmax_s[wave] = wm;
        __syncthreads();
        const float mc = fmaxf(fmaxf(wmax_s[0], wmax_s[1]), fmaxf(wmax_s[2], wmax_s[3]));
        const float p = valid ? q3_expf(s - mc) : 0.0f;
        p_s[wave * 64 + lane] = p;
        __syncthreads();
        float S[8];
#pragma unroll
        for (int i = 0; i < 8; i++) S[i] = 0.0f;
        const int cn = (n - c0) < 256 ? (n - c0) : 256;
#pragma unroll 4
// ... 631 lines not shown
```

qwen3-tts-rust_amd/csrc/kernels_fused.hip:

```cpp
#include "kernels.h"
#include "kdev.h"
#include "wslice.h"
#include <cstdlib>
#include "q3_common.h"

namespace q3 {
Q3_STAMP_SETTER(set_stamp_buffer_fused)

__device__ __forceinline__ void norm_quant_token(const NormPro& a, int d, int tok, int ntok, int lane, int8_t* xq_dst,
                                                 uint16_t* xd_dst, bool write_global) {
    const int nch = d >> 8;
    const float* hin = a.h_in;
    if (a.idx_keys) hin += (size_t)key_code(a.idx_keys[(size_t)tok * a.idx_stride]) * a.h_stride;
    else hin += (size_t)tok * a.h_stride;
    float4 x[8];
    float p = 0.0f;
#pragma unroll
    for (int c = 0; c < 8; c++) {
        if (c < nch) {
            float4 v = *reinterpret_cast<const float4*>(hin + 256 * c + 4 * lane);
            if (a.nparts > 0) {
                const float* pp = a.parts + (size_t)tok * a.parts_stride + 256 * c + 4 * lane;
                float4 y = *reinterpret_cast<const float4*>(pp);
                for (int s = 1; s < a.nparts; s++) {
// ... 252 lines not shown
                    const float dx = h2f(half_of(dxv, i));
                    ag = q3_fmaf((float)ig, h2f(half_of(wsg.dwv, i)) * dx, ag);
                    au = q3_fmaf((float)iu, h2f(half_of(wsu.dwv, i)) * dx, au);
                }
            } else {
                ag = wsg.chain(0.0f, &xq_s[mm][seg * 256], dxv, r, half, 0);
                au = wsu.chain(0.0f, &xq_s[mm][seg * 256], dxv, r, half, 0);
            }
            if (half == 0) { red[wave][0][m * 32 + r] = ag; red[wave][1][m * 32 + r] = au; }
        }
    });
    wg_barrier_lds();
    for (int t = threadIdx.x; t < 32 * MT; t += blockDim.x) {
        const int m = t >> 5, rr = t & 31, tok = tok0 + m;
        float vg[8], vu[8];
#pragma unroll
        for (int s = 0; s < 8; s++) { vg[s] = red[s][0][t]; vu[s] = red[s][1][t]; }
        float G = vg[0], U = vu[0];
#pragma unroll
        for (int s = 1; s < 8; s++) { G = (s < nseg) ? G + vg[s] : G; U = (s < nseg) ? U + vu[s] : U; }
        const float y = q3_swiglu(G, U);
        float amax = q3_fabsf(y);
        amax = fmaxf(amax, xor_lane<16>(amax)); amax = fmaxf(amax, xor_lane<8>(amax)); amax = fmaxf(amax, xor_lane<4>(amax));
        amax = fmaxf(amax, xor_lane<2>(amax)); amax = fmaxf(amax, xor_lane<1>(amax));
        const float dd = amax / 127.0f;
        const float id = (dd != 0.0f) ? (1.0f / dd) : 0.0f;
        if (tok < ntok) {
            aq[(size_t)tok * ff + blockIdx.x * 32 + rr] = (int8_t)(int)q3_rintf(y * id);
            if (rr == 0) ad[(size_t)tok * (ff >> 5) + blockIdx.x] = f2h(dd);
        }
    }
}
void run_gateup_swiglu(hipStream_t st, const LinearPlan& p, const Q8Mat& w, int ff, const NormPro& a, int8_t* aq, uint16_t* ad, int ntok) {
    if (p.form != LIN_GU_SWIGLU_NORM) throw Error("run_gateup_swiglu: not the fused norm gate/up form");
    const int nseg = w.K >> 8;
    const int mt = p.mt;
    dim3 grid(ff / 32, 1, (ntok + mt - 1) / mt);
#define Q3_GU(MTV, NS) Q3_TS_SWITCH(w, hipLaunchKernelGGL((k_gateup_swiglu<MTV, NS, TS>), grid, dim3(64 * NS), 0, st, w, ff, a, aq, ad, ntok))
#define Q3_GU_NS(NS) do { if (mt == 1) Q3_GU(1, NS); else if (mt == 2) Q3_GU(2, NS); else Q3_GU(4, NS); } while (0)
    switch (nseg) {
        case 1: Q3_GU_NS(1); break; case 2: Q3_GU_NS(2); break; case 3: Q3_GU_NS(3); break; case 4: Q3_GU_NS(4); break;
        case 5: Q3_GU_NS(5); break; case 6: Q3_GU_NS(6); break; case 7: Q3_GU_NS(7); break; case 8: Q3_GU_NS(8); break;
        default: throw Error("k_gateup_swiglu: K must be at most 2048");
    }
#undef Q3_GU_NS
#undef Q3_GU
}
void launch_gateup_swiglu(hipStream_t st, const Q8Mat& w, int ff, const NormPro& a, int8_t* aq, uint16_t* ad, int ntok) {
    LinearPlanIn in = linear_plan_in(LOP_NORM_GATEUP, w, 0, 2 * ff, ntok);
    in.ff = ff;
    run_gateup_swiglu(st, plan_linear(in), w, ff, a, aq, ad, ntok);
}

__global__ void __launch_bounds__(256) k_attention_fused(const float* __restrict__ qkv, int qkv_stride, int n_head, int n_kv,
                                                         const float* __restrict__ q_norm_w, const float* __restrict__ k_norm_w,
                                                         float eps, const float* __restrict__ rope_cos,
                                                         const float* __restrict__ rope_sin, int n_ctx,
                                                         const int32_t* __restrict__ mrope_sec, TokMeta tm, KvCache kv, int layer,
                                                         int8_t* __restrict__ aq, uint16_t* __restrict__ ad) {
    __shared__ __attribute__((aligned(16))) float q_s[128];
    __shared__ __attribute__((aligned(16))) uint16_t kcur_s[128];
    __shared__ __attribute__((aligned(16))) uint16_t vcur_s[128];
    __shared__ float p_s[256];
    __shared__ float red_s[4][128];
    __shared__ float wmax_s[4];
    const int h = blockIdx.x, tok = blockIdx.y, tid = threadIdx.x, lane = tid & 63, wave = tid >> 6;
    const int seq = tm.seq_of(tok), slot = tm.slot_of(tok), n = slot + 1;
    const int grp = n_head / n_kv, kvh = h / grp;
    const size_t head_off = (size_t)layer * kv.layer_stride() + (size_t)kvh * 8192;
    const int jj = lane >> 4, dc = lane & 15;
    uint4 kreg[16], vreg[16];
    {
        const int jbase = wave * 64;
        if (jbase < n) {
            const int page = kv.page_of(seq, jbase >> 6);
            const uint16_t* Kb = kv.k + (size_t)page * kv.page_stride() + head_off;
#pragma unroll
            for (int d8 = 0; d8 < 16; d8++) kreg[d8] = *reinterpret_cast<const uint4*>(Kb + (d8 * 64 + lane) * 8);
        }
#pragma unroll
        for (int u = 0; u < 16; u++) {
            const int jg = 16 * u + 4 * wave + jj;
            vreg[u] = make_uint4(0, 0, 0, 0);
            if (jg < n && jg != slot) {
                const int page = kv.page_of(seq, jg >> 6);
                vreg[u] = *reinterpret_cast<const uint4*>(kv.v + (size_t)page * kv.page_stride() + head_off + (jg & 63) * 128 + dc * 8);
            }
        }
    }
    if (wave < 3) {
        const float* vec = qkv + (size_t)tok * qkv_stride + (wave == 0 ? (size_t)h * 128 : wave == 1 ? (size_t)(n_head + kvh) * 128 : (size_t)(n_head + n_kv + kvh) * 128);
        const float x1 = vec[lane], x2 = vec[lane + 64];
        const int page = kv.page_of(seq, slot >> 6), ps = slot & 63;
        if (wave < 2) {
            const float* wn = wave == 0 ? q_norm_w : k_norm_w;
            const float w1 = wn[lane], w2 = wn[lane + 64];
            int32_t sec[4] = { mrope_sec[0], mrope_sec[1], mrope_sec[2], mrope_sec[3] };
            int pp = tm.pos_of(tok, q3_mrope_stream(lane, sec));
            if (pp < 0) pp = 0;
            if (pp > n_ctx - 1) pp = n_ctx - 1;
            const float cs = rope_cos[(size_t)pp * 64 + lane], sn = rope_sin[(size_t)pp * 64 + lane];
            float p = x1 * x1;
            p = q3_fmaf(x2, x2, p);
            const float ss = wave_sum_bfly(p);
            const float mean = ss / 128.0f;
            const float scale = 1.0f / q3_sqrtf(mean + eps);
            const float y1 = (x1 * scale) * w1, y2 = (x2 * scale) * w2;
            float o1, o2;
            q3_rope_pair(y1, y2, cs, sn, &o1, &o2);
            if (wave == 0) { q_s[lane] = o1; q_s[lane + 64] = o2; }
            else {
                const uint16_t k1 = f2h(o1), k2 = f2h(o2);
                kcur_s[lane] = k1; kcur_s[lane + 64] = k2;
                if (h % grp == 0) {
                    uint16_t* Kb = kv.k + (size_t)page * kv.page_stride() + head_off;
                    Kb[((lane >> 3) * 64 + ps) * 8 + (lane & 7)] = k1;
                    Kb[(((lane + 64) >> 3) * 64 + ps) * 8 + (lane & 7)] = k2;
                }
            }
        } else {
            const uint16_t v1 = f2h(x1), v2 = f2h(x2);
            vcur_s[lane] = v1; vcur_s[lane + 64] = v2;
            if (h % grp == 0) {
                uint16_t* Vb = kv.v + (size_t)page * kv.page_stride() + head_off;
                Vb[ps * 128 + lane] = v1; Vb[ps * 128 + lane + 64] = v2;
            }
        }
    }
    wg_barrier_lds();
    const float scale = 0.08838834764831845f;
    float M = 0.0f, L = 0.0f, O[8];
#pragma unroll
    for (int i = 0; i < 8; i++) O[i] = 0.0f;
    for (int c0 = 0; c0 < n; c0 += 256) {
        const int jbase = c0 + wave * 64;
        const int jme = jbase + lane;
        const bool valid = jme < n;
        if (c0 > 0) {
            if (jbase < n) {
                const int page = kv.page_of(seq, jbase >> 6);
                const uint16_t* Kb = kv.k + (size_t)page * kv.page_stride() + head_off;
#pragma unroll
                for (int d8 = 0; d8 < 16; d8++) kreg[d8] = *reinterpret_cast<const uint4*>(Kb + (d8 * 64 + lane) * 8);
            }
// ... 51 lines not shown
        }
#pragma unroll
        for (int i = 0; i < 8; i++) {
            const float a2 = S[i] + xor_lane<16>(S[i]);
            const float T = a2 + xor_lane<32>(a2);
            if (jj == 0) red_s[wave][dc * 8 + i] = T;
        }
        wg_barrier_lds();
        if (wave == 0) {
            float a2 = p_s[lane];
            a2 = a2 + p_s[lane + 64]; a2 = a2 + p_s[lane + 128]; a2 = a2 + p_s[lane + 192];
            const float lc = wave_sum_bfly(a2);
            float oc[8];
#pragma unroll
            for (int i = 0; i < 8; i++) oc[i] = (red_s[0][dc * 8 + i] + red_s[1][dc * 8 + i]) + (red_s[2][dc * 8 + i] + red_s[3][dc * 8 + i]);
            if (c0 == 0) {
                M = mc; L = lc;
#pragma unroll
                for (int i = 0; i < 8; i++) O[i] = oc[i];
            } else {
                const float mn = fmaxf(M, mc);
                const float ea = q3_expf(M - mn), eb = q3_expf(mc - mn);
                const float t2 = lc * eb;
                L = q3_fmaf(L, ea, t2);
#pragma unroll
                for (int i = 0; i < 8; i++) { const float u2 = oc[i] * eb; O[i] = q3_fmaf(O[i], ea, u2); }
                M = mn;
            }
        }
        wg_barrier_lds();
    }
    if (wave == 0) {
        float y[8];
        float amax = 0.0f;
#pragma unroll
        for (int i = 0; i < 8; i++) { y[i] = O[i] / L; amax = fmaxf(amax, q3_fabsf(y[i])); }
        amax = fmaxf(amax, xor_lane<1>(amax));
        amax = fmaxf(amax, xor_lane<2>(amax));
        const float dd = amax / 127.0f;
        const float id = (dd != 0.0f) ? (1.0f / dd) : 0.0f;
        if (jj == 0) {
            const size_t o = ((size_t)tok * n_head + h) * 128 + dc * 8;
            uint32_t lo = 0, hi = 0;
#pragma unroll
            for (int i = 0; i < 4; i++) {
                lo |= (uint32_t)((int)q3_rintf(y[i] * id) & 0xFF) << (8 * i);
                hi |= (uint32_t)((int)q3_rintf(y[i + 4] * id) & 0xFF) << (8 * i);
            }
            *reinterpret_cast<uint2*>(aq + o) = make_uint2(lo, hi);
            if ((dc & 3) == 0) ad[o >> 5] = f2h(dd);
        }
    }
}
void launch_attention_fused(hipStream_t st, const float* qkv, int qkv_stride, int n_head, int n_kv, const float* q_norm_w,
                            const float* k_norm_w, float eps, const float* rope_cos, const float* rope_sin, int n_ctx,
                            const int32_t* mrope_sec, const TokMeta& tm, const KvCache& kv, int layer, int8_t* aq, uint16_t* ad,
                            int ntok) {
    hipLaunchKernelGGL(k_attention_fused, dim3(n_head, ntok), dim3(256), 0, st, qkv, qkv_stride, n_head, n_kv, q_norm_w, k_norm_w,
                       eps, rope_cos, rope_sin, n_ctx, mrope_sec, tm, kv, layer, aq, ad);
}

template <int HPW>
__global__ void __launch_bounds__(64) k_attention_short(const float* __restrict__ qkv, int qkv_stride, int n_head, int n_kv,
                                                        const float* __restrict__ q_norm_w, const float* __restrict__ k_norm_w, float eps,
                                                        const float* __restrict__ rope_cos, const float* __restrict__ rope_sin, int n_ctx,
                                                        const int32_t* __restrict__ mrope_sec, TokMeta tm, KvCache kv, int layer,
                                                        int8_t* __restrict__ aq, uint16_t* __restrict__ ad, float* __restrict__ att) {
    __shared__ __attribute__((aligned(16))) float q_s[HPW][128];
    __shared__ __attribute__((aligned(16))) uint16_t kcur_s[128];
    __shared__ __attribute__((aligned(16))) uint16_t vcur_s[128];
    __shared__ float p_s[HPW][64];
    const int kvh = HPW == 2 ? blockIdx.x : blockIdx.x >> 1, h0 = HPW == 2 ? 2 * blockIdx.x : blockIdx.x;
    Q3_STAMP_DECL;
    Q3_STAMP(0);
    const bool writer = HPW == 2 || (blockIdx.x & 1) == 0;
    const int tok = blockIdx.y, lane = threadIdx.x;
    const float scale = 0.08838834764831845f;
    const int jj = lane >> 4, dc = lane & 15;
    const int seq = tm.seq_of(tok), slot = tm.slot_of(tok), n = slot + 1;
    const size_t head_off = (size_t)layer * kv.layer_stride() + (size_t)kvh * 8192;
    const int page = kv.page_of(seq, 0);
    const uint16_t* Kb = kv.k + (size_t)page * kv.page_stride() + head_off;
    const uint16_t* Vb = kv.v + (size_t)page * kv.page_stride() + head_off;
    uint4 kreg[16], vreg[4][4];
#pragma unroll
    for (int d8 = 0; d8 < 16; d8++) kreg[d8] = (lane < slot) ? *reinterpret_cast<const uint4*>(Kb + (d8 * 64 + lane) * 8) : make_uint4(0, 0, 0, 0);
#pragma unroll
    for (int ww = 0; ww < 4; ww++)
#pragma unroll
        for (int u = 0; u < 4; u++) {
            const int jl = 16 * u + 4 * ww + jj;
            vreg[ww][u] = (jl < slot) ? *reinterpret_cast<const uint4*>(Vb + jl * 128 + dc * 8) : make_uint4(0, 0, 0, 0);
        }
    int32_t sec[4] = { mrope_sec[0], mrope_sec[1], mrope_sec[2], mrope_sec[3] };
    int pp = tm.pos_of(tok, q3_mrope_stream(lane, sec));
    if (pp < 0) pp = 0;
    if (pp > n_ctx - 1) pp = n_ctx - 1;
    const float cs = rope_cos[(size_t)pp * 64 + lane], sn = rope_sin[(size_t)pp * 64 + lane];
    const float* tv = qkv + (size_t)tok * qkv_stride;
#pragma unroll
    for (int which = 0; which < HPW + 1; which++) {
        const float* vec = tv + (which < HPW ? (size_t)(h0 + which) * 128 : (size_t)(n_head + kvh) * 128);
        const float* wn = which < HPW ? q_norm_w : k_norm_w;
        const float x1 = vec[lane], x2 = vec[lane + 64];
        float p = x1 * x1;
        p = q3_fmaf(x2, x2, p);
        const float ss = wave_sum_bfly(p);
        const float mean = ss / 128.0f;
        const float sc2 = 1.0f / q3_sqrtf(mean + eps);
        const float y1 = (x1 * sc2) * wn[lane], y2 = (x2 * sc2) * wn[lane + 64];
        float o1, o2;
        q3_rope_pair(y1, y2, cs, sn, &o1, &o2);
        if (which < HPW) { q_s[which][lane] = o1; q_s[which][lane + 64] = o2; }
        else {
            const uint16_t k1 = f2h(o1), k2 = f2h(o2);
            kcur_s[lane] = k1; kcur_s[lane + 64] = k2;
            if (writer) {
                uint16_t* Kw = kv.k + (size_t)page * kv.page_stride() + head_off;
                Kw[((lane >> 3) * 64 + slot) * 8 + (lane & 7)] = k1;
                Kw[(((lane + 64) >> 3) * 64 + slot) * 8 + (lane & 7)] = k2;
            }
        }
    }
    {
        const float* vec = tv + (size_t)(n_head + n_kv + kvh) * 128;
        const uint16_t v1 = f2h(vec[lane]), v2 = f2h(vec[lane + 64]);
        vcur_s[lane] = v1; vcur_s[lane + 64] = v2;
        if (writer) {
            uint16_t* Vw = kv.v + (size_t)page * kv.page_stride() + head_off;
            Vw[slot * 128 + lane] = v1; Vw[slot * 128 + lane + 64] = v2;
        }
    }
    wg_barrier_lds();
    Q3_STAMP(1);
    const bool valid = lane < n, cur = lane == slot;
    float a[HPW];
#pragma unroll
    for (int hh = 0; hh < HPW; hh++) a[hh] = 0.0f;
#pragma unroll
    for (int d8 = 0; d8 < 16; d8++) {
        uint4 kk = kreg[d8];
        if (cur) kk = *reinterpret_cast<const uint4*>(&kcur_s[8 * d8]);
        const float kf[8] = { h2f(kk.x & 0xFFFFu), h2f(kk.x >> 16), h2f(kk.y & 0xFFFFu), h2f(kk.y >> 16),
                              h2f(kk.z & 0xFFFFu), h2f(kk.z >> 16), h2f(kk.w & 0xFFFFu), h2f(kk.w >> 16) };
#pragma unroll
        for (int e = 0; e < 8; e++)
#pragma unroll
            for (int hh = 0; hh < HPW; hh++) a[hh] = q3_fmaf(q_s[hh][8 * d8 + e], kf[e], a[hh]);
    }
    Q3_STAMP_AFTER(2, a[0]);
    float L[HPW];
#pragma unroll
// ... 18 lines not shown
#pragma unroll
            for (int u = 0; u < 4; u++) {
                if (16 * u < n) {
                    const int jl = 16 * u + 4 * ww + jj;
                    const float pj = p_s[hh][jl];
                    uint4 vv = vreg[ww][u];
                    if (jl == slot) vv = *reinterpret_cast<const uint4*>(&vcur_s[dc * 8]);
                    S[0] = q3_fmaf(pj, h2f(vv.x & 0xFFFFu), S[0]); S[1] = q3_fmaf(pj, h2f(vv.x >> 16), S[1]);
                    S[2] = q3_fmaf(pj, h2f(vv.y & 0xFFFFu), S[2]); S[3] = q3_fmaf(pj, h2f(vv.y >> 16), S[3]);
                    S[4] = q3_fmaf(pj, h2f(vv.z & 0xFFFFu), S[4]); S[5] = q3_fmaf(pj, h2f(vv.z >> 16), S[5]);
                    S[6] = q3_fmaf(pj, h2f(vv.w & 0xFFFFu), S[6]); S[7] = q3_fmaf(pj, h2f(vv.w >> 16), S[7]);
                }
            }
#pragma unroll
            for (int i = 0; i < 8; i++) {
                const float a2 = S[i] + xor_lane<16>(S[i]);
                const float T = a2 + xor_lane<32>(a2);
                if (ww == 0) s01[i] = T; else if (ww == 1) s01[i] = s01[i] + T; else if (ww == 2) s23[i] = T; else s23[i] = s23[i] + T;
            }
        }
#pragma unroll
        for (int i = 0; i < 8; i++) y[i] = (s01[i] + s23[i]) / L[hh];
        const int hq = h0 + hh;
        if (att && jj == 0) {
            float* o = att + (size_t)tok * dq + (size_t)hq * 128 + dc * 8;
            *reinterpret_cast<float4*>(o) = make_float4(y[0], y[1], y[2], y[3]);
            *reinterpret_cast<float4*>(o + 4) = make_float4(y[4], y[5], y[6], y[7]);
        }
        float amax = 0.0f;
#pragma unroll
        for (int i = 0; i < 8; i++) amax = fmaxf(amax, q3_fabsf(y[i]));
        amax = fmaxf(amax, xor_lane<1>(amax));
        amax = fmaxf(amax, xor_lane<2>(amax));
        const float dd = amax / 127.0f;
        const float id = (dd != 0.0f) ? (1.0f / dd) : 0.0f;
        if (jj == 0) {
            uint32_t lo = 0, hi = 0;
#pragma unroll
            for (int i = 0; i < 4; i++) {
                lo |= (uint32_t)((int)q3_rintf(y[i] * id) & 0xFF) << (8 * i);
                hi |= (uint32_t)((int)q3_rintf(y[i + 4] * id) & 0xFF) << (8 * i);
            }
            *reinterpret_cast<uint2*>(aq + (size_t)tok * dq + (size_t)hq * 128 + dc * 8) = make_uint2(lo, hi);
            if ((dc & 3) == 0) ad[(size_t)tok * (dq >> 5) + hq * 4 + (dc >> 2)] = f2h(dd);
        }
    }
    Q3_STAMP(6);
    Q3_STAMP_FLUSH();
}
int short_attn_hpw1_max() {
    static const int v = [] { const char* e = std::getenv("Q3_SHORT_ATTN_HPW1_MAX"); return e ? atoi(e) : 128; }();
    return v;
}
void launch_attention_short(hipStream_t st, int hpw, const float* qkv, int qkv_stride, int n_head, int n_kv, const float* q_norm_w,
                            const float* k_norm_w, float eps, const float* rope_cos, const float* rope_sin, int n_ctx,
                            const int32_t* mrope_sec, const TokMeta& tm, const KvCache& kv, int layer, int8_t* aq, uint16_t* ad, int ntok, float* att) {
    if (hpw == 1)
        hipLaunchKernelGGL(k_attention_short<1>, dim3(n_head, ntok), dim3(64), 0, st, qkv, qkv_stride, n_head, n_kv, q_norm_w, k_norm_w, eps, rope_cos,
                           rope_sin, n_ctx, mrope_sec, tm, kv, layer, aq, ad, att);
    else
        hipLaunchKernelGGL(k_attention_short<2>, dim3(n_kv, ntok), dim3(64), 0, st, qkv, qkv_stride, n_head, n_kv, q_norm_w, k_norm_w, eps, rope_cos,
                           rope_sin, n_ctx, mrope_sec, tm, kv, layer, aq, ad, att);
}

__global__ void __launch_bounds__(256) k_project_mt(const float* __restrict__ x, int x_stride, const float* __restrict__ Wblk,
                                                    const float* __restrict__ b, int n_in, int n_out, float* __restrict__ out,
                                                    int out_stride, int ntok) {
    constexpr int KC = 512, LDP = KC + 4;
    __shared__ __attribute__((aligned(16))) float xs[16][LDP];
    __shared__ __attribute__((aligned(16))) float ws[16][LDP];
    const int ob = blockIdx.x, t0 = blockIdx.y * 16, tid = threadIdx.x;
    const int o16 = tid & 15, tl = tid >> 4;
    const float* wslab = Wblk + (size_t)ob * n_in * 16;
    float4 rx[8], rw[8];
    auto fetch = [&](int k0) {
#pragma unroll
        for (int j = 0; j < 8; j++) {
            const int e = tid + 256 * j;
            const int t = e >> 7, i4 = e & 127;
            rx[j] = (t0 + t < ntok) ? *reinterpret_cast<const float4*>(x + (size_t)(t0 + t) * x_stride + k0 + 4 * i4) : make_float4(0.f, 0.f, 0.f, 0.f);
            rw[j] = *reinterpret_cast<const float4*>(wslab + (size_t)k0 * 16 + 4 * (size_t)e);
        }
    };
    auto stash = [&]() {
#pragma unroll
        for (int j = 0; j < 8; j++) {
            const int e = tid + 256 * j;
            *reinterpret_cast<float4*>(&xs[e >> 7][4 * (e & 127)]) = rx[j];
            const int i = e >> 2, q = (e & 3) * 4;
            ws[q + 0][i] = rw[j].x; ws[q + 1][i] = rw[j].y; ws[q + 2][i] = rw[j].z; ws[q + 3][i] = rw[j].w;
        }
    };
    const int o = ob * 16 + o16;
    float sum = b[o];
    fetch(0);
    for (int k0 = 0; k0 < n_in; k0 += KC) {
        stash();
        __syncthreads();
        if (k0 + KC < n_in) fetch(k0 + KC);
#pragma unroll 8
        for (int i = 0; i < KC; i += 4) {
            const float4 xv = *reinterpret_cast<const float4*>(&xs[tl][i]), wv = *reinterpret_cast<const float4*>(&ws[o16][i]);
            float t = xv.x * wv.x; sum = sum + t;
            t = xv.y * wv.y; sum = sum + t;
            t = xv.z * wv.z; sum = sum + t;
            t = xv.w * wv.w; sum = sum + t;
        }
        __syncthreads();
    }
    if (t0 + tl < ntok) out[(size_t)(t0 + tl) * out_stride + o] = sum;
}
void init_fused_kernel_attributes() {}
void launch_project_blk(hipStream_t st, const float* x, int x_stride, const float* Wblk, const float* b, int n_in, int n_out,
                        float* out, int out_stride, int ntok) {
// ... 164 lines not shown
```

qwen3-tts-rust_amd/csrc/transformer.cpp:

```cpp
#include "transformer.h"
#include <cstdlib>
#include <cmath>

namespace q3 {

__global__ void k_repack_q8(const uint8_t* __restrict__ raw, int n, int K, int row_off, uint8_t* __restrict__ qs,
                            uint16_t* __restrict__ sc, int sc_row_extra) {
    const int nb = K >> 5, nseg = K >> 8;
    const size_t id = (size_t)blockIdx.x * 256 + threadIdx.x;
    if (id >= (size_t)n * nb) return;
    const int r = (int)(id / nb), b = (int)(id % nb);
    const uint8_t* src = raw + id * 34;
    const int row = row_off + r, rg = row >> 5, r32 = row & 31;
    uint16_t d;
    memcpy(&d, src, 2);
    const int srow = row + sc_row_extra;
    sc[(((size_t)(srow >> 5) * nseg + (b >> 3)) * 32 + (srow & 31)) * 8 + (b & 7)] = d;
    uint8_t* dst = qs + ((size_t)rg * nb + b) * 1024 + r32 * 16;
    for (int i = 0; i < 16; i++) { dst[i] = src[2 + i]; dst[512 + i] = src[18 + i]; }
}

__global__ void k_repack_q5k(const uint8_t* __restrict__ raw, int n, int K, int row_off, uint8_t* __restrict__ qs, const uint32_t* __restrict__ rg_off,
                             uint16_t* __restrict__ sc, uint8_t* __restrict__ meta) {
    const int nseg = K >> 8;
    const size_t id = (size_t)blockIdx.x * 256 + threadIdx.x;
    if (id >= (size_t)n * nseg) return;
    const int r = (int)(id / nseg), s = (int)(id % nseg);
    const uint8_t* blk = raw + id * 176;
    const int row = row_off + r, rg = row >> 5, r32 = row & 31;
    const size_t vidx = ((size_t)rg * nseg + s) * 32 + r32;
    uint16_t d, dm;
    memcpy(&d, blk, 2); memcpy(&dm, blk + 2, 2);
    for (int i = 0; i < 8; i++) sc[vidx * 8 + i] = i == 0 ? d : i == 1 ? dm : 0;
    const uint8_t *scales = blk + 4, *qh = blk + 16, *ql = blk + 48;
    uint8_t* base = qs + (size_t)rg_off[rg] * 16 + (size_t)s * 5120;
    for (int j = 0; j < 8; j++) {
        int scv, mv;
        if (j < 4) { scv = scales[j] & 63; mv = scales[j + 4] & 63; }
        else { scv = (scales[j + 4] & 0xF) | ((scales[j - 4] >> 6) << 4); mv = (scales[j + 4] >> 4) | ((scales[j] >> 6) << 4); }
        meta[vidx * 16 + j] = (uint8_t)scv; meta[vidx * 16 + 8 + j] = (uint8_t)mv;
        const int jj = j >> 1, hi = j & 1;
        uint8_t q[32];
        uint32_t H = 0;
        for (int l = 0; l < 32; l++) {
            q[l] = (uint8_t)(hi ? (ql[32 * jj + l] >> 4) : (ql[32 * jj + l] & 0xF));
            H |= (uint32_t)((qh[l] >> (2 * jj + hi)) & 1) << (8 * (l & 3) + (l >> 2));
        }
        for (int h = 0; h < 2; h++)
            for (int w = 0; w < 2; w++)
                for (int bb = 0; bb < 4; bb++) base[j * 512 + h * 256 + r32 * 8 + w * 4 + bb] = (uint8_t)(q[16 * h + 8 * w + bb] | (q[16 * h + 8 * w + 4 + bb] << 4));
        memcpy(base + 4096 + r32 * 32 + j * 4, &H, 4);
    }
}
__global__ void k_repack_q6k(const uint8_t* __restrict__ raw, int n, int K, int row_off, uint8_t* __restrict__ qs, const uint32_t* __restrict__ rg_off,
                             uint16_t* __restrict__ sc, uint8_t* __restrict__ meta) {
// ... 271 lines not shown
    gg_load_rows(st, in.x, in.x_stride, nullptr, in.idx_stride, in.idx_keys, d, h_.p, ntok);
    for (int l = 0; l < hp_.n_layer; l++) {
        const Layer& L = layers_[l];
        const GgLayer& G = gg_layers_[l];
        gg_rmsnorm(st, h_.p, L.attn_norm, d, hp_.eps, gg_xn_.p, ntok);
        gg_quant(st, gg_xn_.p, d, gg_act_, ntok);
        gg_matvec(st, G.wq, 0, dq, gg_act_, qkv_.p, qs, ntok);
        gg_matvec(st, G.wk, 0, dkv, gg_act_, qkv_.p + dq, qs, ntok);
        gg_matvec(st, G.wv, 0, dkv, gg_act_, qkv_.p + dq + dkv, qs, ntok);
        gg_qk_rope_append(st, qkv_.p, qs, hp_.n_head, hp_.n_kv, L.q_norm, L.k_norm, hp_.eps, rope_cos_.p, rope_sin_.p, n_ctx_, d_mrope_.p, tm, kv, l, ntok);
        gg_attention(st, qkv_.p, qs, hp_.n_head, hp_.n_kv, tm, kv, l, gg_att_.p, gg_scores_.p, n_ctx_, ntok);
        gg_linear(st, G.wo, 0, d, gg_att_.p, parts_o_.p, d, ntok);
        gg_add(st, h_.p, parts_o_.p, (size_t)ntok * d);
        gg_rmsnorm(st, h_.p, L.ffn_norm, d, hp_.eps, gg_xn_.p, ntok);
        gg_quant(st, gg_xn_.p, d, gg_act_, ntok);
        gg_matvec(st, G.gate, 0, ff, gg_act_, gu_.p, ff, ntok);
        gg_matvec(st, G.up, 0, ff, gg_act_, gu_.p + (size_t)ntok * ff, ff, ntok);
        gg_swiglu(st, gu_.p, gu_.p + (size_t)ntok * ff, gg_act_f_.p, (size_t)ntok * ff);
        gg_linear(st, G.down, 0, d, gg_act_f_.p, parts_o_.p, d, ntok);
        gg_add(st, h_.p, parts_o_.p, (size_t)ntok * d);
    }
    gg_rmsnorm(st, h_.p, output_norm_, d, hp_.eps, hid_.p, ntok);
    if (hidden_out) launch_copy_f32(st, hid_.p, hidden_out, (size_t)ntok * d);
    Q3_LAUNCH_CHECK();
}


template <class F> static void timed(LaunchTimer* t, hipStream_t st, double bytes, F&& launch) {
    if (t) t->begin(st);
    launch();
    if (t) t->end(st, bytes);
}

void Transformer::gemv(hipStream_t st, const Q8Mat& w, int row0, int nrows, const int8_t* xq, const uint16_t* xd, float* out,
                       int out_stride, int ntok) {
    timed(timer, st, (double)nrows * ((double)w.K + (double)(w.K / 32) * 2.0), [&] { launch_gemv_q8(st, w, row0, nrows, xq, xd, out, out_stride, ntok); });
}

void Transformer::norm(const Pass& s, const NormPro& a) {
    if (s.wgnorm) launch_rmsnorm_quant_wg(s.st, a, hp_.n_embd, xq_.p, xd_.p, s.ntok);
    else launch_rmsnorm_quant(s.st, norm_args(a, hp_.n_embd, xq_.p, xd_.p), s.ntok);
}

void Transformer::linear(const Pass& s, const Q8Mat& w, const FMat& fw, const float* xf, const int8_t* xq, const uint16_t* xd, float* out) {
    if (float_mode_) timed(timer, s.st, (double)fw.bytes(), [&] { launch_gemv_float(s.st, fw, 0, fw.N, xf, fw.K, out, fw.N, s.ntok); });
    else gemv(s.st, w, 0, w.N, xq, xd, out, w.N, s.ntok);
}

void Transformer::qkv(const Pass& s, const Layer& L, const NormPro& a) {
    if (!s.fused) { norm(s, a); linear(s, L.wqkv, L.fqkv, xnf_.p, xq_.p, xd_.p, qkv_.p); return; }
    timed(timer, s.st, (double)L.wqkv.bytes(), [&] { launch_gemv_q8_norm(s.st, L.wqkv, 0, L.wqkv.N, a, qkv_.p, L.wqkv.N, s.ntok, nullptr); });
}

void Transformer::attention(const Pass& s, const Layer& L, int l) {
    const int qs = (hp_.n_head + 2 * hp_.n_kv) * 128;
    float* att = float_mode_ ? attf_.p : nullptr;
    if (s.af == ATTN_SHORT1 || s.af == ATTN_SHORT2)
        launch_attention_short(s.st, s.af == ATTN_SHORT1 ? 1 : 2, qkv_.p, qs, hp_.n_head, hp_.n_kv, L.q_norm, L.k_norm, hp_.eps, rope_cos_.p, rope_sin_.p,
                               n_ctx_, d_mrope_.p, s.tm, s.kv, l, aq_.p, ad_.p, s.ntok, att);
    else if (s.af == ATTN_FUSED)
        launch_attention_fused(s.st, qkv_.p, qs, hp_.n_head, hp_.n_kv, L.q_norm, L.k_norm, hp_.eps, rope_cos_.p, rope_sin_.p, n_ctx_, d_mrope_.p, s.tm,
                               s.kv, l, aq_.p, ad_.p, s.ntok);
    else {
        launch_qk_rope_append(s.st, qkv_.p, qs, nullptr, hp_.n_head, hp_.n_kv, L.q_norm, L.k_norm, hp_.eps, rope_cos_.p, rope_sin_.p, n_ctx_, d_mrope_.p,
                              s.tm, s.kv, l, qrot_.p, s.ntok);
        launch_attention(s.st, qrot_.p, hp_.n_head, hp_.n_kv, s.tm, s.kv, l, att, aq_.p, ad_.p, s.ntok);
    }
}

void Transformer::gate_up(const Pass& s, const Layer& L, const NormPro& b) {
    const int d = hp_.n_embd, ff = hp_.n_ff;
    LaunchTimer* tg = timer_gu ? timer_gu : timer;
    const double bytes = float_mode_ ? (double)L.fgu.bytes() : (double)L.wgu.bytes();
    if (s.fused) { timed(tg, s.st, bytes, [&] { launch_gateup_swiglu(s.st, L.wgu, ff, b, fq_.p, fd_.p, s.ntok); }); return; }
    norm(s, b);
    LinearPlanIn in;
    if (float_mode_) {
        in.op = LOP_F_GATEUP; in.K = d; in.nrows = 2 * ff; in.ntok = s.ntok; in.wts = L.fgu.type; in.has_wt = L.fgu.wt != nullptr;
        in.x_stride = d; in.x_addr = (uintptr_t)xnf_.p;
    } else { in = linear_plan_in(LOP_GATEUP, L.wgu, 0, 2 * ff, s.ntok); in.aq_addr = (uintptr_t)fq_.p; in.fused = fused; }
    in.ff = ff;
    const LinearPlan p = plan_linear(in);
    timed(tg, s.st, bytes, [&] {
        if (p.form == LIN_F_GU_MFMA16) run_gateup_float(s.st, p, L.fgu, ff, xnf_.p, d, actf_.p, s.ntok);
        else if (p.form == LIN_F_GU_UNFUSED) launch_gemv_float(s.st, L.fgu, 0, 2 * ff, xnf_.p, d, gu_.p, 2 * ff, s.ntok);
        else if (p.form == LIN_GU_UNFUSED) launch_gemv_q8(s.st, L.wgu, 0, 2 * ff, xq_.p, xd_.p, gu_.p, 2 * ff, s.ntok);
        else run_gateup_q8(s.st, p, L.wgu, ff, xq_.p, xd_.p, fq_.p, fd_.p, s.ntok);
    });
    if (p.form == LIN_F_GU_UNFUSED) launch_swiglu_f32(s.st, gu_.p, ff, actf_.p, s.ntok);
    else if (p.form == LIN_GU_UNFUSED) launch_swiglu_quant(s.st, gu_.p, ff, fq_.p, fd_.p, s.ntok);
}

void Transformer::forward(hipStream_t st, const Input& in, int ntok, const TokMeta& tm, const KvCache& kv, float* hidden_out) {
    Q3_CHECK(ntok >= 1 && ntok <= max_tok_, "ntok out of range");
    const int d = hp_.n_embd;
    Pass s{st, ntok, tm, kv, attention_form(ntok), false, false};
    last_fused_ = false; last_ntok_ = ntok;
    if (s.af == ATTN_GGML) { forward_ggml(st, in, ntok, tm, kv, hidden_out); return; }
    Q3_CHECK(!float_mode_ || s.af != ATTN_FUSED, "float mode has no fused attention form");
    last_fused_ = s.fused = !float_mode_ && fused && ntok <= fused_max_tok_;
    LinearPlanIn npi; npi.op = LOP_NORM; npi.ntok = ntok;
    s.wgnorm = plan_linear(npi).form == LIN_NORM_WG;
    float* hb = s.fused ? h2_.p : h_.p;
    const int npd = float_mode_ ? 1 : nparts_d_;
    float* xn = float_mode_ ? xnf_.p : nullptr;
    auto pro = [&](const float* h_in, const float* parts, int nparts, float* h_out, const float* g, float* xn_out) {
        NormPro a{};
        a.h_in = h_in; a.h_stride = d; a.parts = parts; a.nparts = nparts; a.parts_stride = d; a.parts_slab = (size_t)ntok * d;
        a.h_out = h_out; a.g = g; a.eps = hp_.eps; a.xn_out = xn_out;
        return a;
    };
    for (int l = 0; l < hp_.n_layer; l++) {
        const Layer& L = layers_[l];
        NormPro a = pro(hb, parts_d_.p, npd, h_.p, L.attn_norm, xn);
        if (l == 0) { a.h_in = in.x; a.h_stride = in.x_stride; a.idx_keys = in.idx_keys; a.idx_stride = in.idx_stride; a.parts = nullptr; a.nparts = 0; }
        qkv(s, L, a);
        attention(s, L, l);
        linear(s, L.wo, L.fo, attf_.p, aq_.p, ad_.p, parts_o_.p);
        gate_up(s, L, pro(h_.p, parts_o_.p, 1, hb, L.ffn_norm, xn));
        linear(s, L.wdown, L.fdown, actf_.p, fq_.p, fd_.p, parts_d_.p);
    }
    if (s.fused) { if (hidden_out) head(st, 0, ntok, 0, 0, nullptr, 0, nullptr, -1, hidden_out); }
    else {
        norm(s, pro(h_.p, parts_d_.p, npd, nullptr, output_norm_, hidden_out ? hidden_out : hid_.p));
        if (float_mode_ && hidden_out) launch_copy_f32(st, hidden_out, hid_.p, (size_t)ntok * d);
    }
    Q3_LAUNCH_CHECK();
}

void Transformer::head(hipStream_t st, int tok0, int tok_count, int row0, int nrows, float* logits, int logits_stride,
                       const ArgmaxEpi* am, int nrows_valid, float* hidden_out) {
    head_impl(st, tok0, tok_count, row0, nrows, logits, logits_stride, am, nrows_valid, hidden_out);
    Q3_LAUNCH_CHECK();
}
void Transformer::head_impl(hipStream_t st, int tok0, int tok_count, int row0, int nrows, float* logits, int logits_stride,
                            const ArgmaxEpi* am, int nrows_valid, float* hidden_out) {
    const int d = hp_.n_embd, nv = nrows_valid > 0 ? nrows_valid : nrows;
    Q3_CHECK(row0 % 32 == 0 && (float_mode_ || row0 + nrows <= output_.Npad), "head row range");
    if (last_fused_) {
        NormPro f{};
        f.h_in = h2_.p + (size_t)tok0 * d; f.h_stride = d;
        f.parts = parts_d_.p + (size_t)tok0 * d; f.nparts = nparts_d_; f.parts_stride = d;
        f.parts_slab = (size_t)last_ntok_ * d;
        f.g = output_norm_; f.eps = hp_.eps; f.xn_out = hidden_out;
        if (nrows <= 0)
            timed(timer, st, 32.0 * ((double)d * 1.0625), [&] { launch_gemv_q8_norm(st, output_, 0, 32, f, scratch_logits(tok_count), 32, tok_count, nullptr); });
        else
            timed(timer, st, (double)nrows * ((double)d * 1.0625),
                  [&] { launch_gemv_q8_norm(st, output_, row0, am ? nv : nrows, f, am ? nullptr : logits, am ? 0 : logits_stride, tok_count, am); });
        return;
    }
    if (hidden_out) launch_copy_f32(st, hid_.p + (size_t)tok0 * d, hidden_out, (size_t)tok_count * d);
    if (nrows <= 0) return;
    float* dst = am ? big_logits_.p : logits;
    const int ls = am ? nrows : logits_stride;
    if (am && big_logits_.n < (size_t)tok_count * nrows) throw Error("head scratch too small");
    int nr = nrows;
    if (ggml_mode_) {
        nr = std::min(nrows, gg_output_.n - row0);
        gg_linear(st, gg_output_, row0, nr, hid_.p + (size_t)tok0 * d, dst, ls, tok_count);
    } else if (float_mode_)
        timed(timer, st, (double)nrows * d * (foutput_.type == Q3_T_F32 ? 4 : 2),
              [&] { launch_gemv_float(st, foutput_, row0, nrows, hid_.p + (size_t)tok0 * d, d, dst, ls, tok_count); });
    else gemv(st, output_, row0, nrows, xq_.p + (size_t)tok0 * d, xd_.p + (size_t)tok0 * (d / 32), dst, ls, tok_count);
    if (am) launch_argmax_keys(st, big_logits_.p, nrows, std::min(nv, nr), am->mask_per_tok, am->keys, am->key_stride, tok_count);
}

KvPool::KvPool(int n_layer, int n_kv, int n_pages, int n_seq, int max_pages_per_seq)
    : n_layer_(n_layer), n_kv_(n_kv), n_pages_(n_pages), n_seq_(n_seq), max_pages_(max_pages_per_seq) {
    const size_t per_page = (size_t)n_layer * n_kv * 8192;
    k_.alloc(per_page * n_pages); v_.alloc(per_page * n_pages);
    k_.zero(); v_.zero();
    const size_t nt = (size_t)n_seq * max_pages_per_seq;
    Q3_HIP(hipHostMalloc((void**)&table_, nt * sizeof(int32_t)));
    std::fill(table_, table_ + nt, 0);
    d_table_.alloc(nt);
    d_table_.upload(table_, nt);
    for (int p = n_pages - 1; p >= 0; p--) free_.push_back(p);
// ... 41 lines not shown
```

qwen3-tts-rust_amd/csrc/transformer.h:

```cpp
#pragma once
#include "q3_common.h"
#include "gguf.h"
#include "kernels.h"
#include "ggml_mode.h"
#include <memory>

namespace q3 {

struct TfHparams {
    std::string arch;
    int n_embd = 0, n_layer = 0, n_head = 0, n_kv = 0, n_ff = 0, n_vocab = 0;
    float eps = 1e-6f, rope_base = 1e6f;
    int32_t mrope_sec[4] = {0, 0, 0, 0};
};

enum AttnForm { ATTN_UNFUSED = 1, ATTN_FUSED = 2, ATTN_SHORT1 = 3, ATTN_SHORT2 = 4, ATTN_GGML = 5 };
struct AttnPlanIn {
    int ntok = 1;
    bool fused = true; int fused_max_tok = 8;
    bool same_seq = false;
    int short_attn_min = 0;
    int n_head = 1, n_kv = 1;
    int hpw1_max = 128;
    bool float_mode = false, ggml_mode = false;
};
int plan_attention(const AttnPlanIn& in);
void build_rope_tables(float rope_base, int n_ctx, std::vector<float>& cos_out, std::vector<float>& sin_out);

class Transformer {
public:
    Transformer(const std::string& gguf_path, int n_ctx, int max_tok);
    Transformer(const Transformer& weights_of, int max_tok);
    const TfHparams& hp() const { return hp_; }
    int n_ctx() const { return n_ctx_; }
    int max_tok() const { return max_tok_; }
    size_t weight_bytes() const { return weight_bytes_; }
    size_t layer_weight_bytes() const { return layer_weight_bytes_; }
    size_t head_bytes_per_row() const { return (size_t)hp_.n_embd + (size_t)(hp_.n_embd / 32) * 2; }

    struct Input {
        const float* x = nullptr; int x_stride = 0;
        const q3_u64* idx_keys = nullptr; int idx_stride = 0;
    };
    bool fused = true;
    void forward(hipStream_t st, const Input& in, int ntok, const TokMeta& tm, const KvCache& kv, float* hidden_out);
    void head(hipStream_t st, int tok0, int tok_count, int row0, int nrows, float* logits, int logits_stride,
              const ArgmaxEpi* am = nullptr, int nrows_valid = -1, float* hidden_out = nullptr);
    void set_same_seq_tokens(bool v) { same_seq_ = v; }
    void set_short_attention(int min_tok, int max_positions) {
        Q3_CHECK(min_tok <= 0 || (max_positions >= 1 && max_positions <= 64), "the short attention form serves at most 64 positions per sequence");
        short_attn_min_ = min_tok;
    }
    void set_fused_max_tokens(int n) { fused_max_tok_ = n; }

    bool ggml_mode() const { return ggml_mode_; }
    int attention_form(int ntok) const;

    LaunchTimer* timer = nullptr;
    LaunchTimer* timer_gu = nullptr;
    const Q8Mat& mat_qkv(int l) const { return layers_[l].wqkv; }
    const Q8Mat& mat_out() const { return output_; }

private:
    void head_impl(hipStream_t st, int tok0, int tok_count, int row0, int nrows, float* logits, int logits_stride, const ArgmaxEpi* am,
                   int nrows_valid, float* hidden_out);
    struct Layer { Q8Mat wqkv, wo, wgu, wdown; FMat fqkv, fo, fgu, fdown; float *attn_norm, *q_norm, *k_norm, *ffn_norm; };
    FMat make_fmat(const Gguf& g, const std::vector<std::string>& names, int K_expect);
    struct Pass { hipStream_t st; int ntok; const TokMeta& tm; const KvCache& kv; int af ; bool fused , wgnorm ; };
    void norm(const Pass& s, const NormPro& a);
    void linear(const Pass& s, const Q8Mat& w, const FMat& fw, const float* xf, const int8_t* xq, const uint16_t* xd, float* out);
    void qkv(const Pass& s, const Layer& L, const NormPro& a);
    void attention(const Pass& s, const Layer& L, int l);
    void gate_up(const Pass& s, const Layer& L, const NormPro& b);
    bool float_mode_ = false; FMat foutput_; DevBuf<float> xnf_, attf_, actf_;
    float* scratch_logits(int) { return scratch_.p; }
    DevBuf<float> scratch_, hid_, big_logits_;
    void gemv(hipStream_t st, const Q8Mat& w, int row0, int nrows, const int8_t* xq, const uint16_t* xd, float* out,
              int out_stride, int ntok);
    Q8Mat make_mat(const Gguf& g, const std::vector<std::pair<std::string, int>>& rows , int N, int K);
    float* load_f32(const Gguf& g, const std::string& name, int64_t n_expect);
    TfHparams hp_;
    int n_ctx_ = 0, max_tok_ = 0;
    std::vector<Layer> layers_;
    Q8Mat output_;
    float* output_norm_ = nullptr;
    struct WeightStore {
        std::vector<DevBuf<uint8_t>> blobs; DevBuf<float> rope_cos, rope_sin; DevBuf<int32_t> d_mrope;
    };
    std::shared_ptr<WeightStore> ws_;
    std::vector<DevBuf<uint8_t>>& blobs_ = ws_init()->blobs;
    size_t weight_bytes_ = 0, layer_weight_bytes_ = 0;
    DevBuf<float>& rope_cos_ = ws_->rope_cos; DevBuf<float>& rope_sin_ = ws_->rope_sin;
    DevBuf<int32_t>& d_mrope_ = ws_->d_mrope;
    WeightStore* ws_init() { if (!ws_) ws_ = std::make_shared<WeightStore>(); return ws_.get(); }
    void alloc_workspace();
    DevBuf<float> h_, h2_, parts_o_, parts_d_, qkv_, qrot_, gu_;
    bool same_seq_ = false; int short_attn_min_ = 0; int fused_max_tok_ = 8; bool last_fused_ = false; int last_ntok_ = 0;
    DevBuf<int8_t> xq_, aq_, fq_;
    DevBuf<uint16_t> xd_, ad_, fd_;
    int nparts_d_ = 1;
    struct GgLayer { GgMat wq, wk, wv, wo, gate, up, down; };
    bool ggml_mode_ = false;
    std::vector<GgLayer> gg_layers_;
    GgMat gg_output_;
    GgMat gg_load(const Gguf& g, const std::string& name, int n_expect, int k_expect);
    void forward_ggml(hipStream_t st, const Input& in, int ntok, const TokMeta& tm, const KvCache& kv, float* hidden_out);
    void gg_linear(hipStream_t st, const GgMat& w, int row0, int nrows, const float* x, float* out, int out_stride, int ntok);
    GgAct gg_act_{};
    DevBuf<int8_t> gg_q8_, gg_qk_; DevBuf<uint16_t> gg_d8_; DevBuf<float> gg_dk_, gg_xn_, gg_att_, gg_scores_, gg_act_f_; DevBuf<int16_t> gg_bs_;
};

Q8Mat build_q8mat(const WLayout& L, const void* const* raw, DevBuf<uint8_t>& blob);
Q8Mat q8mat_from_host(const void* raw_q8_0, int n, int k, DevBuf<uint8_t>& storage);
Q8Mat kqmat_from_host(const void* const* raw, const int32_t* types, const int32_t* rows, int nw, int k, DevBuf<uint8_t>& storage);

class KvPool {
public:
    KvPool(int n_layer, int n_kv, int n_pages, int n_seq, int max_pages_per_seq);
    ~KvPool();
    KvPool(const KvPool&) = delete; KvPool& operator=(const KvPool&) = delete;
    KvCache view() const;
    int alloc_page();
    void free_page(int p);
    void assign(int seq, int logical_page, int physical_page);
    void ensure(int seq, int n_positions);
// ... 17 lines not shown
```

qwen3-tts-rust_amd/python/q3tts/__init__.py:

```python
import ctypes as C
import os
import numpy as np

_HERE = os.path.dirname(os.path.abspath(__file__))
PKG_ROOT = os.path.dirname(os.path.dirname(_HERE))
LIB_PATH = os.path.join(PKG_ROOT, "libq3tts.so")
_lib = None


class Q3Error(RuntimeError):
    pass


class SamplerConfig(C.Structure):
    _fields_ = [("temperature", C.c_float), ("top_k", C.c_int32), ("top_p", C.c_float), ("has_seed", C.c_int32),
                ("seed", C.c_uint64)]


class GenOptions(C.Structure):
    _fields_ = [("repetition_penalty", C.c_float), ("predictor_temperature", C.c_float), ("predictor_top_k", C.c_int32),
                ("predictor_top_p", C.c_float)]


GEN_DEFAULTS = {"repetition_penalty": 1.0, "predictor_temperature": 0.0, "predictor_top_k": 0, "predictor_top_p": 1.0}
# ... 11 lines not shown
                ("total_ms", C.c_double)]


class Stats(C.Structure):
    _fields_ = [("frame_loop_ms", C.c_double), ("frames", C.c_int64), ("prefill_ms", C.c_double), ("gemv_ms", C.c_double),
                ("gemv_launches", C.c_int64), ("gemv_bytes", C.c_double), ("codec_ms", C.c_double), ("codec_calls", C.c_int64),
                ("talker_weight_bytes", C.c_double), ("predictor_weight_bytes", C.c_double), ("kv_bytes_per_token", C.c_double),
                ("gu_ms", C.c_double), ("gu_launches", C.c_int64), ("gu_bytes", C.c_double),
                ("sched_steps", C.c_int64), ("slot_frames", C.c_double), ("graph_frames", C.c_int64)]


class ReqStatus(C.Structure):
    _fields_ = [("state", C.c_int32), ("n_frames", C.c_int32), ("n_pcm", C.c_int64), ("queue_ms", C.c_double),
                ("prefill_ms", C.c_double), ("first_chunk_ms", C.c_double), ("total_ms", C.c_double)]


REQ_QUEUED, REQ_RUNNING, REQ_DRAINING, REQ_DONE, REQ_CANCELLED, REQ_FAILED = 0, 1, 2, 3, 4, -1


DECODE_CB = C.CFUNCTYPE(None, C.c_void_p, C.POINTER(C.c_int64), C.c_int32, C.c_int32)

SYMBOLS = [
    "q3tts_last_error", "q3tts_version", "q3tts_device_count", "q3tts_sampler_config_default", "q3tts_engine_params_default",
    "q3tts_engine_create", "q3tts_engine_destroy", "q3tts_generate_batch", "q3tts_engine_stats", "q3tts_engine_reset_stats",
    "q3tts_engine_set_instrument", "q3tts_engine_bytes_per_step", "q3tts_assets_open", "q3tts_assets_close", "q3tts_engine_assets",
    "q3tts_assets_codec_embedding", "q3tts_assets_text_embedding", "q3tts_assets_tts_pad", "q3tts_prompt_build_core",
    "q3tts_prompt_build_clone", "q3tts_sampler_new", "q3tts_sampler_free", "q3tts_sampler_sample", "q3tts_chunker_new",
    "q3tts_chunker_free", "q3tts_chunker_push", "q3tts_decoder_create", "q3tts_decoder_destroy", "q3tts_decoder_samples_per_frame",
    "q3tts_decoder_reset", "q3tts_decoder_decode", "q3tts_mel_frames", "q3tts_mel", "q3tts_tf_open", "q3tts_tf_close",
    "q3tts_tf_dims", "q3tts_tf_clear", "q3tts_tf_eval", "q3tts_op_gemv_q8", "q3tts_op_gateup_q8", "q3tts_op_matmul_float", "q3tts_op_rmsnorm_quant", "q3tts_op_swiglu_quant",
    "q3tts_op_argmax", "q3tts_op_project", "q3tts_op_sample", "q3tts_submit", "q3tts_poll", "q3tts_fetch", "q3tts_wait",
    "q3tts_release", "q3tts_decoder_create_ex", "q3tts_decoder_decode_group", "q3tts_sched_start", "q3tts_sched_stop", "q3tts_sched_step", "q3tts_voice_register", "q3tts_submit_text",
    "q3tts_group_create", "q3tts_group_destroy", "q3tts_group_size", "q3tts_group_engine", "q3tts_group_uses_rccl", "q3tts_group_voice_register",
    "q3tts_group_submit", "q3tts_group_submit_text", "q3tts_group_device_of", "q3tts_group_poll", "q3tts_group_fetch", "q3tts_group_wait",
    "q3tts_group_release", "q3tts_group_start", "q3tts_group_stop", "q3tts_comm_available", "q3tts_comm_unique_id", "q3tts_comm_create",
    "q3tts_comm_destroy", "q3tts_comm_voice_register", "q3tts_engine_device",
    "q3tts_onnx_open", "q3tts_onnx_close", "q3tts_onnx_counts", "q3tts_onnx_summary", "q3tts_onnx_node", "q3tts_onnx_node_input", "q3tts_onnx_node_output",
    "q3tts_onnx_node_attr_ints", "q3tts_onnx_node_attr_float", "q3tts_onnx_initializer", "q3tts_onnx_op_kernel", "q3tts_onnx_decoder_contract",
    "q3tts_onnx_session_open", "q3tts_onnx_session_close", "q3tts_onnx_session_unsupported", "q3tts_onnx_session_set_input", "q3tts_onnx_session_run",
    "q3tts_onnx_session_output_info", "q3tts_onnx_session_output", "q3tts_onnx_session_launches", "q3tts_onnx_op_executable",
    "q3tts_text_nfc", "q3tts_op_gemv_kq", "q3tts_op_gateup_kq", "q3tts_onnx_decoder_open", "q3tts_onnx_decoder_close", "q3tts_onnx_decoder_reset", "q3tts_onnx_decoder_fetch", "q3tts_group_info", "q3tts_onnx_decoder_decode",
    "q3tts_decoder_state_floats", "q3tts_decoder_state_export", "q3tts_decoder_state_import", "q3tts_decoder_state_entry",
    "q3tts_tokenizer_open", "q3tts_tokenizer_close", "q3tts_tokenizer_encode", "q3tts_tokenizer_decode", "q3tts_tokenizer_vocab_size",
    "q3tts_gen_options_default", "q3tts_submit_ex", "q3tts_submit_text_ex", "q3tts_generate_batch_ex", "q3tts_group_submit_ex",
    "q3tts_group_submit_text_ex", "q3tts_op_sample_rows",
    "q3tts_prompt_build_streaming", "q3tts_submit_trailing", "q3tts_submit_text_streaming", "q3tts_generate_batch_trailing",
    "q3tts_group_submit_text_streaming", "q3tts_op_codec_gemm", "q3tts_codec_gemm_plan", "q3tts_op_codec_kernel", "q3tts_op_attention", "q3tts_attention_plan",
    "q3tts_op_linear", "q3tts_linear_plan", "q3tts_argmax_key",
    "q3tts_submit_trailing_open", "q3tts_trail_append", "q3tts_trail_progress", "q3tts_submit_text_streaming_open", "q3tts_text_append",
    "q3tts_group_submit_text_streaming_open", "q3tts_group_text_append", "q3tts_group_trail_append", "q3tts_group_trail_progress",
    "q3tts_cancel", "q3tts_group_cancel",
    "q3tts_submit_resume", "q3tts_group_submit_resume", "q3tts_op_feedback_rows", "q3tts_engine_prefill_width",
    "q3tts_engine_set_logprobs", "q3tts_fetch_logprobs", "q3tts_group_set_logprobs", "q3tts_group_fetch_logprobs", "q3tts_op_logprob_rows",
]

LOGPROB_COLS = 17
LOGPROB_NONE = 1.0


def lib():
    global _lib
    if _lib is None:
        if not os.path.exists(LIB_PATH):
            raise Q3Error("libq3tts.so not built (run qwen3-tts-rust_amd/build.sh); there is no CPU fallback")
        L = C.CDLL(LIB_PATH)
        L.q3tts_last_error.restype = C.c_char_p
        L.q3tts_engine_create.argtypes = [C.POINTER(EngineParams), C.POINTER(C.c_void_p)]
        L.q3tts_engine_destroy.argtypes = [C.c_void_p]
        L.q3tts_generate_batch.argtypes = [C.c_void_p, C.POINTER(Request), C.c_int32, C.c_int32]
        L.q3tts_engine_stats.argtypes = [C.c_void_p, C.POINTER(Stats)]
        L.q3tts_submit.argtypes = [C.c_void_p, C.POINTER(Request), C.c_int32, C.POINTER(C.c_int64)]
        L.q3tts_poll.argtypes = [C.c_void_p, C.c_int64, C.POINTER(ReqStatus)]
        L.q3tts_fetch.argtypes = [C.c_void_p, C.c_int64, C.c_void_p, C.c_int32, C.c_int32, C.c_void_p, C.c_int64, C.c_int64,
                                  C.POINTER(C.c_int32), C.POINTER(C.c_int64)]
        L.q3tts_wait.argtypes = [C.c_void_p, C.c_int64, C.c_double]
        L.q3tts_release.argtypes = [C.c_void_p, C.c_int64]
        L.q3tts_sched_start.argtypes = [C.c_void_p]
        L.q3tts_sched_stop.argtypes = [C.c_void_p]
        L.q3tts_sched_step.argtypes = [C.c_void_p, C.POINTER(C.c_int32)]
        L.q3tts_voice_register.argtypes = [C.c_void_p, C.c_void_p, C.c_void_p, C.c_int32, C.c_void_p, C.c_int32, C.POINTER(C.c_int32)]
        L.q3tts_submit_text.argtypes = [C.c_void_p, C.c_int32, C.c_void_p, C.c_int32, C.c_int32, C.c_void_p, C.c_int32,
                                        C.POINTER(SamplerConfig), C.c_int32, C.c_int32, C.c_int32, C.POINTER(C.c_int64)]
        L.q3tts_engine_reset_stats.argtypes = [C.c_void_p]
        L.q3tts_engine_set_instrument.argtypes = [C.c_void_p, C.c_int32]
        L.q3tts_engine_bytes_per_step.restype = C.c_double
        L.q3tts_engine_bytes_per_step.argtypes = [C.c_void_p, C.c_int32, C.c_double]
        L.q3tts_assets_open.argtypes = [C.c_char_p, C.POINTER(C.c_void_p)]
        L.q3tts_assets_close.argtypes = [C.c_void_p]
        L.q3tts_engine_assets.restype = C.c_void_p
        L.q3tts_engine_assets.argtypes = [C.c_void_p]
        L.q3tts_assets_codec_embedding.argtypes = [C.c_void_p, C.c_int32, C.c_int32, C.c_void_p]
        L.q3tts_assets_text_embedding.argtypes = [C.c_void_p, C.c_int64, C.c_void_p]
        L.q3tts_assets_tts_pad.argtypes = [C.c_void_p, C.c_void_p]
        L.q3tts_prompt_build_core.argtypes = [C.c_void_p, C.c_void_p, C.c_int32, C.c_int32, C.c_int32, C.c_void_p, C.c_void_p,
                                              C.c_int32, C.c_void_p, C.c_int32, C.c_void_p, C.c_int32]
        L.q3tts_prompt_build_clone.argtypes = [C.c_void_p, C.c_void_p, C.c_int32, C.c_void_p, C.c_int32, C.c_void_p, C.c_int32,
                                               C.c_void_p, C.c_int32, C.c_void_p, C.c_int32, C.c_void_p, C.c_int32]
        L.q3tts_sampler_new.restype = C.c_void_p
        L.q3tts_sampler_new.argtypes = [C.c_float, C.c_int32, C.c_float, C.c_uint64]
        L.q3tts_sampler_free.argtypes = [C.c_void_p]
        L.q3tts_sampler_sample.restype = C.c_int32
        L.q3tts_sampler_sample.argtypes = [C.c_void_p, C.c_void_p, C.c_int32, C.c_int32, C.c_int32]
        L.q3tts_chunker_new.restype = C.c_void_p
        L.q3tts_chunker_new.argtypes = [DECODE_CB, C.c_void_p]
        L.q3tts_chunker_free.argtypes = [C.c_void_p]
        L.q3tts_chunker_push.argtypes = [C.c_void_p, C.c_void_p, C.c_int32, C.c_int32]
# ... 399 lines not shown
    def generate_batch(self, prompts, max_steps=8, temperature=0.0, top_k=40, top_p=0.9, seed=42, mask_eos=True, want_pcm=False,
                       pcm_per_frame=1920, repetition_penalty=1.0, predictor_temperature=0.0, predictor_top_k=0, predictor_top_p=1.0,
                       trailing_ids=None):
        n = len(prompts)
        reqs = (Request * n)()
        opts = [self._opts(i, repetition_penalty, predictor_temperature, predictor_top_k, predictor_top_p) for i in range(n)]
        keep = []
        for i, pr in enumerate(prompts):
            pr = np.ascontiguousarray(pr, np.float32)
            ms = self._per(max_steps, i)
            codes = np.zeros(max(ms, 1) * 16, np.int32)
            pcm = np.zeros(max(ms * pcm_per_frame, 1), np.float32) if want_pcm else None
            keep.append((pr, codes, pcm))
            r = reqs[i]
            self._fill(r, pr, i, max_steps, temperature, top_k, top_p, seed, mask_eos)
            r.codes_out = codes.ctypes.data
            r.pcm_out = pcm.ctypes.data if pcm is not None else None
            r.pcm_capacity = pcm.size if pcm is not None else 0
        if trailing_ids is not None:
            if len(trailing_ids) != n:
                raise Q3Error("trailing_ids needs one entry per request")
            trs = [np.ascontiguousarray(t if t is not None else [], np.int32) for t in trailing_ids]
            ptrs = (C.c_void_p * n)(*[t.ctypes.data if t.size else None for t in trs])
            cnt = np.array([t.size for t in trs], np.int32)
            arr = (GenOptions * n)(*[o if o is not None else GenOptions(**GEN_DEFAULTS) for o in opts])
            _chk(lib().q3tts_generate_batch_trailing(self.h, reqs, n, 1 if want_pcm else 0, arr, ptrs, _p(cnt)))
        elif all(o is None for o in opts):
            _chk(lib().q3tts_generate_batch(self.h, reqs, n, 1 if want_pcm else 0))
        else:
            arr = (GenOptions * n)(*[o if o is not None else GenOptions(**GEN_DEFAULTS) for o in opts])
            _chk(lib().q3tts_generate_batch_ex(self.h, reqs, n, 1 if want_pcm else 0, arr))
        out = []
        for i in range(n):
            nf = reqs[i].n_frames
            out.append({"codes": keep[i][1][: nf * 16].reshape(nf, 16).copy(),
                        "pcm": keep[i][2][: reqs[i].n_pcm].copy() if want_pcm else None,
                        "prefill_ms": reqs[i].prefill_ms, "first_chunk_ms": reqs[i].first_chunk_ms, "total_ms": reqs[i].total_ms})
        return out

    def stats(self):
        s = Stats()
        _chk(lib().q3tts_engine_stats(self.h, C.byref(s)))
        return {k: getattr(s, k) for k, _ in Stats._fields_}

    def reset_stats(self):
        lib().q3tts_engine_reset_stats(self.h)

    def set_instrument(self, on):
        lib().q3tts_engine_set_instrument(self.h, 1 if on else 0)

    def bytes_per_step(self, batch, mean_ctx):
        return lib().q3tts_engine_bytes_per_step(self.h, batch, mean_ctx)


class TfContext:
    def __init__(self, path, n_ctx=4096, max_tok=64):
        h = C.c_void_p()
        _chk(lib().q3tts_tf_open(path.encode(), n_ctx, max_tok, C.byref(h)))
        self.h = h.value
        d = [C.c_int32() for _ in range(4)]
        lib().q3tts_tf_dims(self.h, *[C.byref(x) for x in d])
        self.n_embd, self.n_layer, self.n_head, self.n_vocab = [x.value for x in d]

    def close(self):
        if self.h:
            lib().q3tts_tf_close(self.h)
        self.h = None

    def clear(self):
        lib().q3tts_tf_clear(self.h)

    def eval(self, x, pos4, row0=0, row1=0):
        x = np.ascontiguousarray(x, np.float32).reshape(-1, self.n_embd)
        pos4 = np.ascontiguousarray(pos4, np.int32).reshape(-1, 4)
        n = x.shape[0]
        hid = np.zeros((n, self.n_embd), np.float32)
        logits = np.zeros((n, max(row1 - row0, 1)), np.float32)
        _chk(lib().q3tts_tf_eval(self.h, _p(x), _p(pos4), n, _p(hid), _p(logits) if row1 > row0 else None, row0, row1))
        return hid, logits[:, : max(row1 - row0, 0)]


class Decoder:
    def __init__(self, path, n_streams=1, max_frames=64, max_group=1):
        h = C.c_void_p()
        if max_group > 1 or max_frames != 64:
            _chk(lib().q3tts_decoder_create_ex(path.encode(), n_streams, max_frames, max_group, C.byref(h)))
        else:
            _chk(lib().q3tts_decoder_create(path.encode(), n_streams, C.byref(h)))
        self.h = h.value
        self.spf = lib().q3tts_decoder_samples_per_frame(self.h)

    def close(self):
        if self.h:
            lib().q3tts_decoder_destroy(self.h)
        self.h = None

    def reset(self, stream=0):
        _chk(lib().q3tts_decoder_reset(self.h, stream))

    def decode(self, codes, is_last=False, stream=0):
        codes = np.ascontiguousarray(codes, np.int64).reshape(-1, 16)
        wav = np.zeros(codes.shape[0] * self.spf, np.float32)
        valid = C.c_int64(0)
        _chk(lib().q3tts_decoder_decode(self.h, stream, _p(codes), codes.shape[0], 1 if is_last else 0, _p(wav), C.byref(valid)))
        return wav[: valid.value]

# ... 315 lines not shown
        if self.h:
            lib().q3tts_onnx_decoder_close(self.h)
        self.h = None

    def reset(self):
        _chk(lib().q3tts_onnx_decoder_reset(self.h))

    def decode(self, codes, is_final=False, max_samples_per_frame=1920):
        codes = np.ascontiguousarray(codes, np.int64).reshape(-1, 16)
        out = np.zeros(max(codes.shape[0], 1) * max_samples_per_frame, np.float32)
        n = C.c_int64()
        rc = lib().q3tts_onnx_decoder_decode(self.h, codes.ctypes.data, codes.shape[0], 1 if is_final else 0, out.ctypes.data, out.size, C.byref(n))
        if rc == 2:
            out = np.zeros(n.value, np.float32)
            lib().q3tts_onnx_decoder_fetch.argtypes = [C.c_void_p, C.c_void_p, C.c_int64, C.POINTER(C.c_int64)]
            rc = lib().q3tts_onnx_decoder_fetch(self.h, out.ctypes.data, out.size, C.byref(n))
        _chk(rc)
        return out[: n.value].copy()


ATTN_FORMS = {"AUTO": 0, "UNFUSED": 1, "FUSED": 2, "SHORT1": 3, "SHORT2": 4, "GGML": 5}
ATTN_FORM_NAMES = {v: k for k, v in ATTN_FORMS.items()}


class AttentionDesc(C.Structure):
    _fields_ = [("n_head", C.c_int32), ("n_kv", C.c_int32), ("n_layer", C.c_int32), ("layer", C.c_int32), ("ntok", C.c_int32),
                ("qkv", C.c_void_p), ("qkv_stride", C.c_int32), ("q_norm", C.c_void_p), ("k_norm", C.c_void_p),
                ("eps", C.c_float), ("rope_base", C.c_float), ("n_ctx", C.c_int32), ("mrope_sec", C.c_int32 * 4),
                ("seq", C.c_void_p), ("slot", C.c_void_p), ("pos", C.c_void_p), ("uniform_pos", C.c_int32),
                ("page_table", C.c_void_p), ("n_seq", C.c_int32), ("max_pages", C.c_int32),
                ("k_cache", C.c_void_p), ("v_cache", C.c_void_p), ("n_pages", C.c_int32),
                ("fused", C.c_int32), ("fused_max_tok", C.c_int32), ("same_seq", C.c_int32), ("short_attn_min", C.c_int32),
                ("hpw1_max", C.c_int32), ("float_mode", C.c_int32), ("ggml_mode", C.c_int32),
                ("form", C.c_int32), ("att", C.c_void_p), ("aq", C.c_void_p), ("ad", C.c_void_p), ("form_ran", C.c_int32)]


def _attn_flags(d, fused, fused_max_tok, same_seq, short_attn_min, hpw1_max, float_mode, ggml_mode):
    d.fused, d.fused_max_tok, d.same_seq, d.short_attn_min = int(fused), fused_max_tok, int(same_seq), short_attn_min
    d.hpw1_max, d.float_mode, d.ggml_mode = hpw1_max, int(float_mode), int(ggml_mode)


def attention_plan(ntok, n_head=16, n_kv=8, fused=True, fused_max_tok=8, same_seq=False, short_attn_min=0, hpw1_max=0, float_mode=False,
                   ggml_mode=False):
    d = AttentionDesc()
    d.ntok, d.n_head, d.n_kv = ntok, n_head, n_kv
    _attn_flags(d, fused, fused_max_tok, same_seq, short_attn_min, hpw1_max, float_mode, ggml_mode)
    lib().q3tts_attention_plan.argtypes = [C.POINTER(AttentionDesc)]
    _chk(lib().q3tts_attention_plan(C.byref(d)))
    return ATTN_FORM_NAMES[d.form_ran]


def op_attention(qkv, q_norm, k_norm, k_cache, v_cache, n_head, n_kv, n_layer, layer, eps=1e-6, rope_base=1e6, n_ctx=4096,
                 mrope_sec=(0, 0, 0, 0), seq=None, slot=None, pos=None, uniform_pos=-1, page_table=None, form="AUTO", fused=True,
                 fused_max_tok=8, same_seq=False, short_attn_min=0, hpw1_max=0, float_mode=False, ggml_mode=False):
    qkv = np.ascontiguousarray(qkv, np.float32)
    ntok = qkv.shape[0]
    q_norm = np.ascontiguousarray(q_norm, np.float32)
    k_norm = np.ascontiguousarray(k_norm, np.float32)
    kc = np.array(k_cache, np.uint16, copy=True, order="C")
    vc = np.array(v_cache, np.uint16, copy=True, order="C")
    assert kc.shape == vc.shape and kc.size % (n_layer * n_kv * 8192) == 0
    d = AttentionDesc()
    d.n_head, d.n_kv, d.n_layer, d.layer, d.ntok = n_head, n_kv, n_layer, layer, ntok
    d.qkv, d.qkv_stride, d.q_norm, d.k_norm = _p(qkv), qkv.shape[1], _p(q_norm), _p(k_norm)
    d.eps, d.rope_base, d.n_ctx = eps, rope_base, n_ctx
    for i in range(4):
        d.mrope_sec[i] = int(mrope_sec[i])
    keep = []
    if uniform_pos < 0:
        seq = np.ascontiguousarray(seq, np.int32)
        slot = np.ascontiguousarray(slot, np.int32)
        pos = np.ascontiguousarray(pos, np.int32).reshape(ntok, 4)
        keep += [seq, slot, pos]
        d.seq, d.slot, d.pos = _p(seq), _p(slot), _p(pos)
    d.uniform_pos = uniform_pos
    if page_table is not None:
        page_table = np.ascontiguousarray(page_table, np.int32)
        keep.append(page_table)
        d.page_table, d.n_seq, d.max_pages = _p(page_table), page_table.shape[0], page_table.shape[1]
    d.k_cache, d.v_cache, d.n_pages = _p(kc), _p(vc), kc.size // (n_layer * n_kv * 8192)
    _attn_flags(d, fused, fused_max_tok, same_seq, short_attn_min, hpw1_max, float_mode, ggml_mode)
    d.form = ATTN_FORMS[form]
    att = np.full((ntok, n_head * 128), np.nan, np.float32)
    aq = np.zeros((ntok, n_head * 128), np.int8)
    ad = np.zeros((ntok, n_head * 4), np.uint16)
    d.att, d.aq, d.ad = _p(att), _p(aq), _p(ad)
    lib().q3tts_op_attention.argtypes = [C.POINTER(AttentionDesc)]
    _chk(lib().q3tts_op_attention(C.byref(d)))
    ran = ATTN_FORM_NAMES[d.form_ran]
    return dict(att=None if ran == "FUSED" else att, aq=None if ran == "GGML" else aq, ad=None if ran == "GGML" else ad,
                k_cache=kc, v_cache=vc, form=ran)


def op_gemv_kq(parts, k, xq, xd, lpr=0):
    L = lib()
    L.q3tts_op_gemv_kq.argtypes = [C.c_void_p, C.c_void_p, C.c_void_p, C.c_int32, C.c_int32, C.c_void_p, C.c_void_p, C.c_int32, C.c_void_p, C.c_int32]
    raws = [np.ascontiguousarray(p[0]) for p in parts]
    ptrs = (C.c_void_p * len(parts))(*[r.ctypes.data for r in raws])
    types = np.asarray([p[1] for p in parts], np.int32); rows = np.asarray([p[2] for p in parts], np.int32)
    xq = np.ascontiguousarray(xq, np.int8); xd = np.ascontiguousarray(xd, np.uint16)
    ntok = xq.shape[0]
    y = np.zeros((ntok, int(rows.sum())), np.float32)
    _chk(L.q3tts_op_gemv_kq(ptrs, types.ctypes.data, rows.ctypes.data, len(parts), k, xq.ctypes.data, xd.ctypes.data, ntok, y.ctypes.data, lpr))
    return y


def op_gateup_kq(gate_raw, up_raw, qtype, ff, k, xq, xd):
    L = lib()
    L.q3tts_op_gateup_kq.argtypes = [C.c_void_p, C.c_void_p, C.c_int32, C.c_int32, C.c_int32, C.c_void_p, C.c_void_p, C.c_int32, C.c_void_p, C.c_void_p]
    g = np.ascontiguousarray(gate_raw); u = np.ascontiguousarray(up_raw)
    xq = np.ascontiguousarray(xq, np.int8); xd = np.ascontiguousarray(xd, np.uint16)
    ntok = xq.shape[0]
    aq = np.zeros((ntok, ff), np.int8); ad = np.zeros((ntok, ff // 32), np.uint16)
    _chk(L.q3tts_op_gateup_kq(g.ctypes.data, u.ctypes.data, qtype, ff, k, xq.ctypes.data, xd.ctypes.data, ntok, aq.ctypes.data, ad.ctypes.data))
    return aq, ad


def text_nfc(text):
    L = lib()
    L.q3tts_text_nfc.restype = C.c_int64
    L.q3tts_text_nfc.argtypes = [C.c_char_p, C.c_char_p, C.c_int64]
    raw = text.encode("utf-8", "surrogatepass")
    n = L.q3tts_text_nfc(raw, None, 0)
    buf = C.create_string_buffer(int(n))
    L.q3tts_text_nfc(raw, buf, n)
    return buf.raw[: n - 1].decode("utf-8", "surrogatepass")


def onnx_op_executable(op_type):
    L = lib()
    L.q3tts_onnx_op_executable.argtypes = [C.c_char_p]
    return bool(L.q3tts_onnx_op_executable(op_type.encode()))


class OnnxModel:

    def __init__(self, path):
        L = lib()
        L.q3tts_onnx_open.argtypes = [C.c_char_p, C.POINTER(C.c_void_p)]
        L.q3tts_onnx_close.argtypes = [C.c_void_p]
        L.q3tts_onnx_counts.argtypes = [C.c_void_p] + [C.POINTER(C.c_int32)] * 4
        L.q3tts_onnx_summary.restype = C.c_int64
        L.q3tts_onnx_summary.argtypes = [C.c_void_p, C.c_char_p, C.c_int64]
        L.q3tts_onnx_node.argtypes = [C.c_void_p, C.c_int32, C.POINTER(C.c_char_p), C.POINTER(C.c_char_p)] + [C.POINTER(C.c_int32)] * 3
# ... 171 lines not shown
```

Baseline: 699.7.

## Precompute predictor layer-0 QKV per codebook entry and gather rows by argmax key

At engine init, for each codebook (1..14) the predictor's layer-0 RMSNorm and QKV projection are run over every codec embedding row and stored as a table. During the frame loop, layer 0 skips the norm and QKV GEMV and instead has the attention kernels read q/k/v rows indexed by the argmax keys, using a new QkvRows accessor. This removes one weight-streaming GEMV per predictor step. The cost is extra device memory for the tables, a startup build pass, and a dependence on layer-0 input being exactly the embedding lookup. It is gated off by an environment variable and in ggml mode.

```diff
diff --git a/include/q3tts.h b/include/q3tts.h
--- a/include/q3tts.h
+++ b/include/q3tts.h
@@ -76,6 +76,7 @@
 void q3tts_engine_reset_stats(q3tts_engine* e);
 void q3tts_engine_set_instrument(q3tts_engine* e, int32_t on);
 double q3tts_engine_bytes_per_step(q3tts_engine* e, int32_t batch, double mean_ctx);
+int64_t q3tts_pred_table_bytes(q3tts_engine* e);
 
 #define Q3TTS_REQ_QUEUED 0
 #define Q3TTS_REQ_RUNNING 1
@@ -355,6 +356,7 @@
     int32_t form_ran;
 } q3tts_attention_desc;
 int q3tts_op_attention(q3tts_attention_desc* d);
+int q3tts_op_attention_keyed(q3tts_attention_desc* d, const uint64_t* keys, int32_t key_stride, int32_t qkv_rows);
 int q3tts_attention_plan(q3tts_attention_desc* d);
 
 enum { Q3TTS_LOP_GEMV = 0, Q3TTS_LOP_GATEUP = 1, Q3TTS_LOP_NORM = 2, Q3TTS_LOP_NORM_GEMV = 3, Q3TTS_LOP_NORM_ARGMAX = 4, Q3TTS_LOP_NORM_GATEUP = 5,
diff --git a/qwen3-tts-rust_amd/csrc/capi.cpp b/qwen3-tts-rust_amd/csrc/capi.cpp
--- a/qwen3-tts-rust_amd/csrc/capi.cpp
+++ b/qwen3-tts-rust_amd/csrc/capi.cpp
@@ -290,6 +290,7 @@
 void q3tts_engine_reset_stats(q3tts_engine* e) { if (e) e->e->reset_stats(); }
 void q3tts_engine_set_instrument(q3tts_engine* e, int32_t on) { if (e) e->e->set_instrument(on != 0); }
 double q3tts_engine_bytes_per_step(q3tts_engine* e, int32_t batch, double mean_ctx) { return e ? (double)e->e->bytes_per_frame_step(batch, mean_ctx) : 0.0; }
+int64_t q3tts_pred_table_bytes(q3tts_engine* e) { return e ? (int64_t)e->e->pred_table_bytes() : 0; }
 
 int q3tts_assets_open(const char* path, q3tts_assets** out) {
     Q3_API_BEGIN
diff --git a/qwen3-tts-rust_amd/csrc/capi_ops.cpp b/qwen3-tts-rust_amd/csrc/capi_ops.cpp
--- a/qwen3-tts-rust_amd/csrc/capi_ops.cpp
+++ b/qwen3-tts-rust_amd/csrc/capi_ops.cpp
@@ -49,14 +49,25 @@
     }
 }
 
-static void attention_op_run(q3tts_attention_desc* dp) {
+static void attention_op_run(q3tts_attention_desc* dp, const uint64_t* keys = nullptr, int key_stride = 0, int qkv_rows = 0) {
     Q3_CHECK(dp, "null attention descriptor");
     q3tts_attention_desc& d = *dp;
     Q3_CHECK(d.ntok >= 1 && d.n_head >= 1 && d.n_kv >= 1, "bad attention shape");
     const int form = d.form == Q3TTS_ATTN_AUTO ? attention_op_plan(d) : d.form;
     attention_op_check(d, form);
     const int nt = d.ntok, dq = d.n_head * 128, qs = d.qkv_stride;
-    DevBuf<float> qkv((size_t)nt * qs); qkv.upload(d.qkv, qkv.n);
+    DevBuf<q3_u64> dkeys;
+    if (keys) {
+        Q3_CHECK(form != ATTN_GGML, "the ggml form reads no keyed rows");
+        Q3_CHECK(key_stride >= 1 && qkv_rows >= 1, "bad key stride / table rows");
+        for (int t = 0; t < nt; t++) {
+            const int c = key_code(keys[(size_t)t * key_stride]);
+            Q3_CHECK(c >= 0 && c < qkv_rows, "a key selects a row outside the table");
+        }
+        dkeys.alloc((size_t)(nt - 1) * key_stride + 1); dkeys.upload((const q3_u64*)keys, dkeys.n);
+    }
+    DevBuf<float> qkv((size_t)(keys ? qkv_rows : nt) * qs); qkv.upload(d.qkv, qkv.n);
+    const QkvRows rows(qkv.p, qs, dkeys.p, key_stride);
     DevBuf<float> qn(128), kn(128); qn.upload(d.q_norm, 128); kn.upload(d.k_norm, 128);
     std::vector<float> hc, hs;
     build_rope_tables(d.rope_base, d.n_ctx, hc, hs);
@@ -80,14 +91,14 @@
     switch (form) {
     case ATTN_UNFUSED:
         qrot.alloc((size_t)nt * dq);
-        launch_qk_rope_append(0, qkv.p, qs, nullptr, d.n_head, d.n_kv, qn.p, kn.p, d.eps, rc.p, rs.p, d.n_ctx, sec.p, tm, kv, d.layer, qrot.p, nt);
+        launch_qk_rope_append(0, rows, nullptr, d.n_head, d.n_kv, qn.p, kn.p, d.eps, rc.p, rs.p, d.n_ctx, sec.p, tm, kv, d.layer, qrot.p, nt);
         launch_attention(0, qrot.p, d.n_head, d.n_kv, tm, kv, d.layer, att.p, aq.p, ad.p, nt);
         break;
     case ATTN_FUSED:
-        launch_attention_fused(0, qkv.p, qs, d.n_head, d.n_kv, qn.p, kn.p, d.eps, rc.p, rs.p, d.n_ctx, sec.p, tm, kv, d.layer, aq.p, ad.p, nt);
+        launch_attention_fused(0, rows, d.n_head, d.n_kv, qn.p, kn.p, d.eps, rc.p, rs.p, d.n_ctx, sec.p, tm, kv, d.layer, aq.p, ad.p, nt);
         break;
     case ATTN_SHORT1: case ATTN_SHORT2:
-        launch_attention_short(0, form == ATTN_SHORT1 ? 1 : 2, qkv.p, qs, d.n_head, d.n_kv, qn.p, kn.p, d.eps, rc.p, rs.p, d.n_ctx, sec.p, tm, kv,
+        launch_attention_short(0, form == ATTN_SHORT1 ? 1 : 2, rows, d.n_head, d.n_kv, qn.p, kn.p, d.eps, rc.p, rs.p, d.n_ctx, sec.p, tm, kv,
                                d.layer, aq.p, ad.p, nt, att.p);
         break;
     default:
@@ -101,6 +112,7 @@
     kc.download(d.k_cache, cache_halfs); vc.download(d.v_cache, cache_halfs);
     if (d.att && form != ATTN_FUSED) att.download(d.att, att.n);
     if (form != ATTN_GGML) { aq.download(d.aq, aq.n); ad.download(d.ad, ad.n); }
+    if (keys) qkv.download(const_cast<float*>(d.qkv), qkv.n);
     d.form_ran = form;
 }
 
@@ -341,6 +353,15 @@
     Q3_API_BEGIN
     require_gpu();
     attention_op_run(d);
+    return Q3TTS_OK;
+    Q3_API_END(Q3TTS_ERR)
+}
+
+int q3tts_op_attention_keyed(q3tts_attention_desc* d, const uint64_t* keys, int32_t key_stride, int32_t qkv_rows) {
+    Q3_API_BEGIN
+    require_gpu();
+    Q3_CHECK(keys, "null keys");
+    attention_op_run(d, keys, key_stride, qkv_rows);
     return Q3TTS_OK;
     Q3_API_END(Q3TTS_ERR)
 }
diff --git a/qwen3-tts-rust_amd/csrc/engine.cpp b/qwen3-tts-rust_amd/csrc/engine.cpp
--- a/qwen3-tts-rust_amd/csrc/engine.cpp
+++ b/qwen3-tts-rust_amd/csrc/engine.cpp
@@ -64,6 +64,18 @@
     }
     d_tab_ptrs_.alloc(16); d_tab_ptrs_.upload(ptrs.data(), 16);
     d_tab_rows_.alloc(16); d_tab_rows_.upload(rows.data(), 16);
+    pred_l0_table_ = !predictor_->ggml_mode();
+    if (const char* e = std::getenv("Q3_PRED_L0_TABLE")) if (e[0] == '0') pred_l0_table_ = false;
+    if (pred_l0_table_) {
+        const int qs = (predictor_->hp().n_head + 2 * predictor_->hp().n_kv) * 128;
+        Transformer wide(*predictor_, 256);
+        for (int q = 1; q < 15; q++) {
+            d_qkv0_tab_[q].alloc((size_t)assets_->codec_rows[q] * qs);
+            wide.build_layer0_qkv(st_, d_proj_tab_[q].p, dP_, assets_->codec_rows[q], d_qkv0_tab_[q].p);
+            pred_table_bytes_ += d_qkv0_tab_[q].n * sizeof(float);
+        }
+        Q3_HIP(hipStreamSynchronize(st_));
+    }
     const int pages_per_seq = (p.max_prompt + p.max_steps + 1 + 63) / 64;
     kv_rows_ = (int64_t)pages_per_seq * 64;
     kv_t_.reset(new KvPool(talker_->hp().n_layer, talker_->hp().n_kv, B * pages_per_seq + 1, B + 1, pages_per_seq));
@@ -202,8 +214,9 @@
     const size_t head_t = (size_t)tl_stride_ * talker_->head_bytes_per_row();
     const size_t head_p = (size_t)15 * Q3_CODEBOOK_SIZE * predictor_->head_bytes_per_row();
     const size_t kv_per_tok = (size_t)t.n_layer * 2 * t.n_kv * 128 * 2;
+    const size_t tab_rows = pred_l0_table_ ? (size_t)batch * 14 * (size_t)(predictor_->hp().n_head + 2 * predictor_->hp().n_kv) * 128 * 4 : 0;
     return talker_->weight_bytes() + head_t + predictor_->weight_bytes() + head_p +
-           (size_t)((double)batch * mean_ctx * (double)kv_per_tok) + (size_t)batch * 17 * 8192;
+           (size_t)((double)batch * mean_ctx * (double)kv_per_tok) + (size_t)batch * 17 * 8192 + tab_rows;
 }
 
 void Engine::record_frame(FrameGraph& fg, FrameVariant v) {
@@ -239,6 +252,7 @@
         KvCache kvq = kvp;
         if (pred_identity_pages_) { tm.uniform_pos = q + 1; kvq.page_table = nullptr; }
         Transformer::Input in; in.x = d_proj_tab_[q].p; in.x_stride = dP_; in.idx_keys = d_keys_.p + q; in.idx_stride = 16;
+        if (pred_l0_table_) { in.qkv0 = d_qkv0_tab_[q].p; in.qkv0_stride = (predictor_->hp().n_head + 2 * predictor_->hp().n_kv) * 128; }
         predictor_->forward(st_, in, B, tm, kvq, nullptr);
         if (v.pred || v.lp) {
             float* pl = v.lp ? d_plp_.p + (size_t)q * B_ * Q3_CODEBOOK_SIZE : d_plogits_.p;
diff --git a/qwen3-tts-rust_amd/csrc/engine.h b/qwen3-tts-rust_amd/csrc/engine.h
--- a/qwen3-tts-rust_amd/csrc/engine.h
+++ b/qwen3-tts-rust_amd/csrc/engine.h
@@ -80,6 +80,7 @@
     EngineStats stats; void reset_stats() { stats = EngineStats(); }
     void set_instrument(bool on) { instrument_ = on; }
     size_t bytes_per_frame_step(int batch, double mean_ctx) const;
+    size_t pred_table_bytes() const { return pred_table_bytes_; }
     hipStream_t stream() const { return st_; }
     int max_batch() const { return B_; }
     int device() const { return dev_; }
@@ -127,6 +128,7 @@
     std::unique_ptr<KvPool> kv_t_, kv_p_;
     std::unique_ptr<CodecDecoder> codec_;
     DevBuf<float> d_codec_tab_[16]; DevBuf<float> d_proj_tab_[16];
+    DevBuf<float> d_qkv0_tab_[16]; bool pred_l0_table_ = false; size_t pred_table_bytes_ = 0;
     DevBuf<float> d_proj_wt_, d_proj_wblk_, d_proj_b_, d_tts_pad_;
     DevBuf<const float*> d_tab_ptrs_; DevBuf<int64_t> d_tab_rows_;
     int dP_ = 0;
diff --git a/qwen3-tts-rust_amd/csrc/kernels.h b/qwen3-tts-rust_amd/csrc/kernels.h
--- a/qwen3-tts-rust_amd/csrc/kernels.h
+++ b/qwen3-tts-rust_amd/csrc/kernels.h
@@ -56,7 +56,18 @@
 };
 void launch_rmsnorm_quant(hipStream_t st, const NormArgs& a, int ntok);
 
-void launch_qk_rope_append(hipStream_t st, const float* qkv, int qkv_stride, const float* parts_unused, int n_head, int n_kv,
+struct QkvRows {
+    const float* base = nullptr;
+    const unsigned long long* keys = nullptr;
+    int stride = 0, key_stride = 0;
+    QkvRows() = default;
+    QkvRows(const float* b, int s, const unsigned long long* k = nullptr, int ks = 0) : base(b), keys(k), stride(s), key_stride(ks) {}
+    __device__ __forceinline__ const float* row(int tok) const {
+        return base + (size_t)(keys ? (int)(~(uint32_t)keys[(size_t)tok * key_stride]) : tok) * stride;
+    }
+};
+
+void launch_qk_rope_append(hipStream_t st, const QkvRows& qkv, const float* parts_unused, int n_head, int n_kv,
                            const float* q_norm_w, const float* k_norm_w, float eps, const float* rope_cos,
                            const float* rope_sin, int n_ctx, const int32_t* mrope_sec , const TokMeta& tm,
                            const KvCache& kv, int layer, float* qrot, int ntok);
@@ -108,11 +119,11 @@
     return NormArgs{p.h_in, p.h_stride, idx, p.idx_stride, p.idx_keys, p.parts, p.nparts, p.parts_stride, p.h_out, p.g, p.eps, d, xq, xd, p.xn_out};
 }
 void launch_gateup_swiglu(hipStream_t st, const Q8Mat& wgu, int ff, const NormPro& a, int8_t* aq, uint16_t* ad, int ntok);
-void launch_attention_fused(hipStream_t st, const float* qkv, int qkv_stride, int n_head, int n_kv, const float* q_norm_w,
+void launch_attention_fused(hipStream_t st, const QkvRows& qkv, int n_head, int n_kv, const float* q_norm_w,
                             const float* k_norm_w, float eps, const float* rope_cos, const float* rope_sin, int n_ctx,
                             const int32_t* mrope_sec, const TokMeta& tm, const KvCache& kv, int layer, int8_t* aq, uint16_t* ad,
                             int ntok);
-void launch_attention_short(hipStream_t st, int hpw, const float* qkv, int qkv_stride, int n_head, int n_kv, const float* q_norm_w,
+void launch_attention_short(hipStream_t st, int hpw, const QkvRows& qkv, int n_head, int n_kv, const float* q_norm_w,
                             const float* k_norm_w, float eps, const float* rope_cos, const float* rope_sin, int n_ctx,
                             const int32_t* mrope_sec, const TokMeta& tm, const KvCache& kv, int layer, int8_t* aq, uint16_t* ad, int ntok,
                             float* att = nullptr );
diff --git a/qwen3-tts-rust_amd/csrc/kernels.hip b/qwen3-tts-rust_amd/csrc/kernels.hip
--- a/qwen3-tts-rust_amd/csrc/kernels.hip
+++ b/qwen3-tts-rust_amd/csrc/kernels.hip
@@ -834,14 +834,14 @@
     hipLaunchKernelGGL(k_rmsnorm_quant, dim3(ntok), dim3(64), 0, st, a);
 }
 
-__global__ void __launch_bounds__(64) k_qk_rope_append(const float* __restrict__ qkv, int qkv_stride, int n_head, int n_kv,
+__global__ void __launch_bounds__(64) k_qk_rope_append(QkvRows qkv, int n_head, int n_kv,
                                                        const float* __restrict__ q_norm_w, const float* __restrict__ k_norm_w,
                                                        float eps, const float* __restrict__ rope_cos,
                                                        const float* __restrict__ rope_sin, int n_ctx,
                                                        const int32_t* __restrict__ mrope_sec, TokMeta tm, KvCache kv,
                                                        int layer, float* __restrict__ qrot) {
     const int hv = blockIdx.x, tok = blockIdx.y, lane = threadIdx.x;
-    const float* vec = qkv + (size_t)tok * qkv_stride + (size_t)hv * 128;
+    const float* vec = qkv.row(tok) + (size_t)hv * 128;
     float x1 = vec[lane], x2 = vec[lane + 64];
     const int seq = tm.seq_of(tok), slot = tm.slot_of(tok);
     const int page = kv.page_of(seq, slot >> 6);
@@ -876,11 +876,11 @@
         Vb[ps * 128 + lane + 64] = f2h(x2);
     }
 }
-void launch_qk_rope_append(hipStream_t st, const float* qkv, int qkv_stride, const float*, int n_head, int n_kv,
+void launch_qk_rope_append(hipStream_t st, const QkvRows& qkv, const float*, int n_head, int n_kv,
                            const float* q_norm_w, const float* k_norm_w, float eps, const float* rope_cos,
                            const float* rope_sin, int n_ctx, const int32_t* mrope_sec, const TokMeta& tm,
                            const KvCache& kv, int layer, float* qrot, int ntok) {
-    hipLaunchKernelGGL(k_qk_rope_append, dim3(n_head + 2 * n_kv, ntok), dim3(64), 0, st, qkv, qkv_stride, n_head, n_kv,
+    hipLaunchKernelGGL(k_qk_rope_append, dim3(n_head + 2 * n_kv, ntok), dim3(64), 0, st, qkv, n_head, n_kv,
                        q_norm_w, k_norm_w, eps, rope_cos, rope_sin, n_ctx, mrope_sec, tm, kv, layer, qrot);
 }
 
diff --git a/qwen3-tts-rust_amd/csrc/kernels_fused.hip b/qwen3-tts-rust_amd/csrc/kernels_fused.hip
--- a/qwen3-tts-rust_amd/csrc/kernels_fused.hip
+++ b/qwen3-tts-rust_amd/csrc/kernels_fused.hip
@@ -328,7 +328,7 @@
     run_gateup_swiglu(st, plan_linear(in), w, ff, a, aq, ad, ntok);
 }
 
-__global__ void __launch_bounds__(256) k_attention_fused(const float* __restrict__ qkv, int qkv_stride, int n_head, int n_kv,
+__global__ void __launch_bounds__(256) k_attention_fused(QkvRows qkv, int n_head, int n_kv,
                                                          const float* __restrict__ q_norm_w, const float* __restrict__ k_norm_w,
                                                          float eps, const float* __restrict__ rope_cos,
                                                          const float* __restrict__ rope_sin, int n_ctx,
@@ -365,7 +365,7 @@
         }
     }
     if (wave < 3) {
-        const float* vec = qkv + (size_t)tok * qkv_stride + (wave == 0 ? (size_t)h * 128 : wave == 1 ? (size_t)(n_head + kvh) * 128 : (size_t)(n_head + n_kv + kvh) * 128);
+        const float* vec = qkv.row(tok) + (wave == 0 ? (size_t)h * 128 : wave == 1 ? (size_t)(n_head + kvh) * 128 : (size_t)(n_head + n_kv + kvh) * 128);
         const float x1 = vec[lane], x2 = vec[lane + 64];
         const int page = kv.page_of(seq, slot >> 6), ps = slot & 63;
         if (wave < 2) {
@@ -523,16 +523,16 @@
         }
     }
 }
-void launch_attention_fused(hipStream_t st, const float* qkv, int qkv_stride, int n_head, int n_kv, const float* q_norm_w,
+void launch_attention_fused(hipStream_t st, const QkvRows& qkv, int n_head, int n_kv, const float* q_norm_w,
                             const float* k_norm_w, float eps, const float* rope_cos, const float* rope_sin, int n_ctx,
                             const int32_t* mrope_sec, const TokMeta& tm, const KvCache& kv, int layer, int8_t* aq, uint16_t* ad,
                             int ntok) {
-    hipLaunchKernelGGL(k_attention_fused, dim3(n_head, ntok), dim3(256), 0, st, qkv, qkv_stride, n_head, n_kv, q_norm_w, k_norm_w,
+    hipLaunchKernelGGL(k_attention_fused, dim3(n_head, ntok), dim3(256), 0, st, qkv, n_head, n_kv, q_norm_w, k_norm_w,
                        eps, rope_cos, rope_sin, n_ctx, mrope_sec, tm, kv, layer, aq, ad);
 }
 
 template <int HPW>
-__global__ void __launch_bounds__(64) k_attention_short(const float* __restrict__ qkv, int qkv_stride, int n_head, int n_kv,
+__global__ void __launch_bounds__(64) k_attention_short(QkvRows qkv, int n_head, int n_kv,
                                                         const float* __restrict__ q_norm_w, const float* __restrict__ k_norm_w, float eps,
                                                         const float* __restrict__ rope_cos, const float* __restrict__ rope_sin, int n_ctx,
                                                         const int32_t* __restrict__ mrope_sec, TokMeta tm, KvCache kv, int layer,
@@ -546,6 +546,7 @@
     Q3_STAMP(0);
     const bool writer = HPW == 2 || (blockIdx.x & 1) == 0;
     const int tok = blockIdx.y, lane = threadIdx.x;
+    const float* tv = qkv.row(tok);
     const float scale = 0.08838834764831845f;
     const int jj = lane >> 4, dc = lane & 15;
     const int seq = tm.seq_of(tok), slot = tm.slot_of(tok), n = slot + 1;
@@ -568,7 +569,6 @@
     if (pp < 0) pp = 0;
     if (pp > n_ctx - 1) pp = n_ctx - 1;
     const float cs = rope_cos[(size_t)pp * 64 + lane], sn = rope_sin[(size_t)pp * 64 + lane];
-    const float* tv = qkv + (size_t)tok * qkv_stride;
 #pragma unroll
     for (int which = 0; which < HPW + 1; which++) {
         const float* vec = tv + (which < HPW ? (size_t)(h0 + which) * 128 : (size_t)(n_head + kvh) * 128);
@@ -693,14 +693,14 @@
     static const int v = [] { const char* e = std::getenv("Q3_SHORT_ATTN_HPW1_MAX"); return e ? atoi(e) : 128; }();
     return v;
 }
-void launch_attention_short(hipStream_t st, int hpw, const float* qkv, int qkv_stride, int n_head, int n_kv, const float* q_norm_w,
+void launch_attention_short(hipStream_t st, int hpw, const QkvRows& qkv, int n_head, int n_kv, const float* q_norm_w,
                             const float* k_norm_w, float eps, const float* rope_cos, const float* rope_sin, int n_ctx,
                             const int32_t* mrope_sec, const TokMeta& tm, const KvCache& kv, int layer, int8_t* aq, uint16_t* ad, int ntok, float* att) {
     if (hpw == 1)
-        hipLaunchKernelGGL(k_attention_short<1>, dim3(n_head, ntok), dim3(64), 0, st, qkv, qkv_stride, n_head, n_kv, q_norm_w, k_norm_w, eps, rope_cos,
+        hipLaunchKernelGGL(k_attention_short<1>, dim3(n_head, ntok), dim3(64), 0, st, qkv, n_head, n_kv, q_norm_w, k_norm_w, eps, rope_cos,
                            rope_sin, n_ctx, mrope_sec, tm, kv, layer, aq, ad, att);
     else
-        hipLaunchKernelGGL(k_attention_short<2>, dim3(n_kv, ntok), dim3(64), 0, st, qkv, qkv_stride, n_head, n_kv, q_norm_w, k_norm_w, eps, rope_cos,
+        hipLaunchKernelGGL(k_attention_short<2>, dim3(n_kv, ntok), dim3(64), 0, st, qkv, n_head, n_kv, q_norm_w, k_norm_w, eps, rope_cos,
                            rope_sin, n_ctx, mrope_sec, tm, kv, layer, aq, ad, att);
 }
 
diff --git a/qwen3-tts-rust_amd/csrc/transformer.cpp b/qwen3-tts-rust_amd/csrc/transformer.cpp
--- a/qwen3-tts-rust_amd/csrc/transformer.cpp
+++ b/qwen3-tts-rust_amd/csrc/transformer.cpp
@@ -1,6 +1,7 @@
 #include "transformer.h"
 #include <cstdlib>
 #include <cmath>
+#include <algorithm>
 
 namespace q3 {
 
@@ -378,17 +379,16 @@
     timed(timer, s.st, (double)L.wqkv.bytes(), [&] { launch_gemv_q8_norm(s.st, L.wqkv, 0, L.wqkv.N, a, qkv_.p, L.wqkv.N, s.ntok, nullptr); });
 }
 
-void Transformer::attention(const Pass& s, const Layer& L, int l) {
-    const int qs = (hp_.n_head + 2 * hp_.n_kv) * 128;
+void Transformer::attention(const Pass& s, const Layer& L, int l, const QkvRows& rows) {
     float* att = float_mode_ ? attf_.p : nullptr;
     if (s.af == ATTN_SHORT1 || s.af == ATTN_SHORT2)
-        launch_attention_short(s.st, s.af == ATTN_SHORT1 ? 1 : 2, qkv_.p, qs, hp_.n_head, hp_.n_kv, L.q_norm, L.k_norm, hp_.eps, rope_cos_.p, rope_sin_.p,
+        launch_attention_short(s.st, s.af == ATTN_SHORT1 ? 1 : 2, rows, hp_.n_head, hp_.n_kv, L.q_norm, L.k_norm, hp_.eps, rope_cos_.p, rope_sin_.p,
                                n_ctx_, d_mrope_.p, s.tm, s.kv, l, aq_.p, ad_.p, s.ntok, att);
     else if (s.af == ATTN_FUSED)
-        launch_attention_fused(s.st, qkv_.p, qs, hp_.n_head, hp_.n_kv, L.q_norm, L.k_norm, hp_.eps, rope_cos_.p, rope_sin_.p, n_ctx_, d_mrope_.p, s.tm,
+        launch_attention_fused(s.st, rows, hp_.n_head, hp_.n_kv, L.q_norm, L.k_norm, hp_.eps, rope_cos_.p, rope_sin_.p, n_ctx_, d_mrope_.p, s.tm,
                                s.kv, l, aq_.p, ad_.p, s.ntok);
     else {
-        launch_qk_rope_append(s.st, qkv_.p, qs, nullptr, hp_.n_head, hp_.n_kv, L.q_norm, L.k_norm, hp_.eps, rope_cos_.p, rope_sin_.p, n_ctx_, d_mrope_.p,
+        launch_qk_rope_append(s.st, rows, nullptr, hp_.n_head, hp_.n_kv, L.q_norm, L.k_norm, hp_.eps, rope_cos_.p, rope_sin_.p, n_ctx_, d_mrope_.p,
                               s.tm, s.kv, l, qrot_.p, s.ntok);
         launch_attention(s.st, qrot_.p, hp_.n_head, hp_.n_kv, s.tm, s.kv, l, att, aq_.p, ad_.p, s.ntok);
     }
@@ -419,7 +419,8 @@
 
 void Transformer::forward(hipStream_t st, const Input& in, int ntok, const TokMeta& tm, const KvCache& kv, float* hidden_out) {
     Q3_CHECK(ntok >= 1 && ntok <= max_tok_, "ntok out of range");
-    const int d = hp_.n_embd;
+    Q3_CHECK(!in.qkv0 || (in.idx_keys && !ggml_mode_), "layer-0 q/k/v rows need the argmax keys that select them (and are not for the ggml mode)");
+    const int d = hp_.n_embd, qs = (hp_.n_head + 2 * hp_.n_kv) * 128;
     Pass s{st, ntok, tm, kv, attention_form(ntok), false, false};
     last_fused_ = false; last_ntok_ = ntok;
     if (s.af == ATTN_GGML) { forward_ggml(st, in, ntok, tm, kv, hidden_out); return; }
@@ -440,16 +441,38 @@
         const Layer& L = layers_[l];
         NormPro a = pro(hb, parts_d_.p, npd, h_.p, L.attn_norm, xn);
         if (l == 0) { a.h_in = in.x; a.h_stride = in.x_stride; a.idx_keys = in.idx_keys; a.idx_stride = in.idx_stride; a.parts = nullptr; a.nparts = 0; }
-        qkv(s, L, a);
-        attention(s, L, l);
+        NormPro b = pro(h_.p, parts_o_.p, 1, hb, L.ffn_norm, xn);
+        const bool tab0 = l == 0 && in.qkv0;
+        if (tab0) { b.h_in = in.x; b.h_stride = in.x_stride; b.idx_keys = in.idx_keys; b.idx_stride = in.idx_stride; }
+        else qkv(s, L, a);
+        attention(s, L, l, tab0 ? QkvRows(in.qkv0, in.qkv0_stride, in.idx_keys, in.idx_stride) : QkvRows(qkv_.p, qs));
         linear(s, L.wo, L.fo, attf_.p, aq_.p, ad_.p, parts_o_.p);
-        gate_up(s, L, pro(h_.p, parts_o_.p, 1, hb, L.ffn_norm, xn));
+        gate_up(s, L, b);
         linear(s, L.wdown, L.fdown, actf_.p, fq_.p, fd_.p, parts_d_.p);
     }
     if (s.fused) { if (hidden_out) head(st, 0, ntok, 0, 0, nullptr, 0, nullptr, -1, hidden_out); }
     else {
         norm(s, pro(h_.p, parts_d_.p, npd, nullptr, output_norm_, hidden_out ? hidden_out : hid_.p));
         if (float_mode_ && hidden_out) launch_copy_f32(st, hidden_out, hid_.p, (size_t)ntok * d);
+    }
+    Q3_LAUNCH_CHECK();
+}
+
+void Transformer::build_layer0_qkv(hipStream_t st, const float* x, int x_stride, int64_t rows, float* out) {
+    Q3_CHECK(!ggml_mode_, "the ggml mode takes no layer-0 q/k/v rows");
+    const int d = hp_.n_embd, qs = (hp_.n_head + 2 * hp_.n_kv) * 128;
+    const Layer& L = layers_[0];
+    const TokMeta tm{nullptr, nullptr, nullptr}; const KvCache kv{};
+    for (int64_t r0 = 0; r0 < rows; r0 += max_tok_) {
+        const int n = (int)std::min<int64_t>(max_tok_, rows - r0);
+        Pass s{st, n, tm, kv, ATTN_UNFUSED, false, false};
+        LinearPlanIn npi; npi.op = LOP_NORM; npi.ntok = n;
+        s.wgnorm = plan_linear(npi).form == LIN_NORM_WG;
+        NormPro a{};
+        a.h_in = x + (size_t)r0 * x_stride; a.h_stride = x_stride; a.parts_stride = d; a.g = L.attn_norm; a.eps = hp_.eps;
+        a.xn_out = float_mode_ ? xnf_.p : nullptr;
+        norm(s, a);
+        linear(s, L.wqkv, L.fqkv, xnf_.p, xq_.p, xd_.p, out + (size_t)r0 * qs);
     }
     Q3_LAUNCH_CHECK();
 }
diff --git a/qwen3-tts-rust_amd/csrc/transformer.h b/qwen3-tts-rust_amd/csrc/transformer.h
--- a/qwen3-tts-rust_amd/csrc/transformer.h
+++ b/qwen3-tts-rust_amd/csrc/transformer.h
@@ -41,11 +41,13 @@
     struct Input {
         const float* x = nullptr; int x_stride = 0;
         const q3_u64* idx_keys = nullptr; int idx_stride = 0;
+        const float* qkv0 = nullptr; int qkv0_stride = 0;
     };
     bool fused = true;
     void forward(hipStream_t st, const Input& in, int ntok, const TokMeta& tm, const KvCache& kv, float* hidden_out);
     void head(hipStream_t st, int tok0, int tok_count, int row0, int nrows, float* logits, int logits_stride,
               const ArgmaxEpi* am = nullptr, int nrows_valid = -1, float* hidden_out = nullptr);
+    void build_layer0_qkv(hipStream_t st, const float* x, int x_stride, int64_t rows, float* out);
     void set_same_seq_tokens(bool v) { same_seq_ = v; }
     void set_short_attention(int min_tok, int max_positions) {
         Q3_CHECK(min_tok <= 0 || (max_positions >= 1 && max_positions <= 64), "the short attention form serves at most 64 positions per sequence");
@@ -70,7 +72,7 @@
     void norm(const Pass& s, const NormPro& a);
     void linear(const Pass& s, const Q8Mat& w, const FMat& fw, const float* xf, const int8_t* xq, const uint16_t* xd, float* out);
     void qkv(const Pass& s, const Layer& L, const NormPro& a);
-    void attention(const Pass& s, const Layer& L, int l);
+    void attention(const Pass& s, const Layer& L, int l, const QkvRows& rows);
     void gate_up(const Pass& s, const Layer& L, const NormPro& b);
     bool float_mode_ = false; FMat foutput_; DevBuf<float> xnf_, attf_, actf_;
     float* scratch_logits(int) { return scratch_.p; }
diff --git a/qwen3-tts-rust_amd/python/q3tts/__init__.py b/qwen3-tts-rust_amd/python/q3tts/__init__.py
--- a/qwen3-tts-rust_amd/python/q3tts/__init__.py
+++ b/qwen3-tts-rust_amd/python/q3tts/__init__.py
@@ -87,6 +87,7 @@
     "q3tts_cancel", "q3tts_group_cancel",
     "q3tts_submit_resume", "q3tts_group_submit_resume", "q3tts_op_feedback_rows", "q3tts_engine_prefill_width",
     "q3tts_engine_set_logprobs", "q3tts_fetch_logprobs", "q3tts_group_set_logprobs", "q3tts_group_fetch_logprobs", "q3tts_op_logprob_rows",
+    "q3tts_pred_table_bytes", "q3tts_op_attention_keyed",
 ]
 
 LOGPROB_COLS = 17
@@ -592,6 +593,12 @@
     def bytes_per_step(self, batch, mean_ctx):
         return lib().q3tts_engine_bytes_per_step(self.h, batch, mean_ctx)
 
+    def pred_table_bytes(self):
+        L = lib()
+        L.q3tts_pred_table_bytes.restype = C.c_int64
+        L.q3tts_pred_table_bytes.argtypes = [C.c_void_p]
+        return int(L.q3tts_pred_table_bytes(self.h))
+
 
 class TfContext:
     def __init__(self, path, n_ctx=4096, max_tok=64):
@@ -1013,9 +1020,15 @@
 
 def op_attention(qkv, q_norm, k_norm, k_cache, v_cache, n_head, n_kv, n_layer, layer, eps=1e-6, rope_base=1e6, n_ctx=4096,
                  mrope_sec=(0, 0, 0, 0), seq=None, slot=None, pos=None, uniform_pos=-1, page_table=None, form="AUTO", fused=True,
-                 fused_max_tok=8, same_seq=False, short_attn_min=0, hpw1_max=0, float_mode=False, ggml_mode=False):
-    qkv = np.ascontiguousarray(qkv, np.float32)
-    ntok = qkv.shape[0]
+                 fused_max_tok=8, same_seq=False, short_attn_min=0, hpw1_max=0, float_mode=False, ggml_mode=False, keys=None):
+    if keys is not None:
+        keys = np.ascontiguousarray(keys, np.uint64)
+        keys = keys.reshape(keys.shape[0], -1)
+        qkv = np.array(qkv, np.float32, copy=True, order="C")
+        ntok = keys.shape[0]
+    else:
+        qkv = np.ascontiguousarray(qkv, np.float32)
+        ntok = qkv.shape[0]
     q_norm = np.ascontiguousarray(q_norm, np.float32)
     k_norm = np.ascontiguousarray(k_norm, np.float32)
     kc = np.array(k_cache, np.uint16, copy=True, order="C")
@@ -1046,11 +1059,18 @@
     aq = np.zeros((ntok, n_head * 128), np.int8)
     ad = np.zeros((ntok, n_head * 4), np.uint16)
     d.att, d.aq, d.ad = _p(att), _p(aq), _p(ad)
-    lib().q3tts_op_attention.argtypes = [C.POINTER(AttentionDesc)]
-    _chk(lib().q3tts_op_attention(C.byref(d)))
+    if keys is not None:
+        lib().q3tts_op_attention_keyed.argtypes = [C.POINTER(AttentionDesc), C.c_void_p, C.c_int32, C.c_int32]
+        _chk(lib().q3tts_op_attention_keyed(C.byref(d), _p(keys), keys.shape[1], qkv.shape[0]))
+    else:
+        lib().q3tts_op_attention.argtypes = [C.POINTER(AttentionDesc)]
+        _chk(lib().q3tts_op_attention(C.byref(d)))
     ran = ATTN_FORM_NAMES[d.form_ran]
-    return dict(att=None if ran == "FUSED" else att, aq=None if ran == "GGML" else aq, ad=None if ran == "GGML" else ad,
-                k_cache=kc, v_cache=vc, form=ran)
+    r = dict(att=None if ran == "FUSED" else att, aq=None if ran == "GGML" else aq, ad=None if ran == "GGML" else ad,
+             k_cache=kc, v_cache=vc, form=ran)
+    if keys is not None:
+        r["qkv"] = qkv
+    return r
 
 
 def op_gemv_kq(parts, k, xq, xd, lpr=0):
```

New measurement: 713.2 (median of 6 runs). 1.02x the previous value.
